# PytorchConnectomics/pytorch_connectomics

Hardware: AMD Instinct MI355X
Metric: voxels/s (train + sliding-window infer), MedNeXt-S 112^3 bf16 (higher is better)
Workload: dtype bf16; 1 GPU; Lucchi++ sliding-window inference (configs[1]): MedNeXt-S k3, 165x1024x768 volume, roi 112^3, overlap 0.5, bump blending, sw_batch_size 8, random-init weights; step = one whole-volume EagerSlidingWindowEngine call (TTA off); value = window-voxels/s; sw_batch_size=8, window_pipeline_streams=3

## Files before the change

include/pytc_hip.h:

```cpp
#ifndef PYTC_HIP_H
#define PYTC_HIP_H

#include <stdint.h>

#ifdef __cplusplus
extern "C" {
#endif

#define PYTC_ABI_VERSION 5

#define PYTC_OK 0
#define PYTC_ERR_INVALID 1
#define PYTC_ERR_HIP 2
#define PYTC_ERR_UNSUPPORTED 3

#define PYTC_F32 0
#define PYTC_BF16 1

#define PYTC_VIEW_FLIP_Z 1
#define PYTC_VIEW_FLIP_Y 2
#define PYTC_VIEW_FLIP_X 4
#define PYTC_VIEW_SWAP_YX 8
#define PYTC_VIEW_SWAP_ZY 16
#define PYTC_VIEW_SWAP_ZX 32

#define PYTC_PAD_CONSTANT 0
#define PYTC_PAD_REFLECT 1
#define PYTC_PAD_REPLICATE 2
#define PYTC_PAD_CIRCULAR 3

#define PYTC_BLEND_PRODUCT 0
#define PYTC_BLEND_MIN 1

#define PYTC_ACT_NONE 0
#define PYTC_ACT_SIGMOID 1
#define PYTC_ACT_TANH 2
#define PYTC_ACT_GELU 3

#define PYTC_RES_NONE 0
#define PYTC_RES_ADD 1
#define PYTC_RES_UPSAMPLE 2
#define PYTC_RES_GELU_BWD 3
#define PYTC_RES_NORM_BWD 4

int pytc_abi_version(void);
const char* pytc_last_error(void);
int pytc_device_info(int device, int* cu_count, int* lds_bytes_per_cu, char* arch, int arch_len);
int pytc_set_tuning(const char* key, int value);


int pytc_gather_windows(const float* vol, int C, int Z, int Y, int X, const int32_t* starts, int B,
                        int rz, int ry, int rx, int view, int pad_mode, float cval, void* out,
                        int out_dtype, void* stream);

int pytc_blend_accumulate(const void* pred, int pred_dtype, int B, const int32_t* starts, int rz,
                          int ry, int rx, int C, int view, const float* wz, const float* wy,
                          const float* wx, int combine, float floor_w, const int32_t* border ,
                          float* value, float* weight, int Z, int Y, int X, void* stream);

int pytc_blend_accumulate_mapped(const void* pred, int pred_dtype, int B, const int32_t* starts, int rz, int ry,
                                 int rx, int C, int view, const float* wz, const float* wy, const float* wx,
                                 int combine, float floor_w, const int32_t* border, const int32_t* chan_src,
                                 const int32_t* chan_shift, float* value, float* weight, int Z, int Y, int X,
                                 void* stream);
int pytc_blend_weight_shifted(int B, const int32_t* starts, int rz, int ry, int rx, const float* wz, const float* wy,
                              const float* wx, int combine, float floor_w, const int32_t* border,
                              const int32_t* shift, float* weight, int Z, int Y, int X, void* stream);
int pytc_normalize_covered(float* value, const float* weight, int64_t n, void* stream);
int pytc_ensemble_update_masked(float* stat, float* count, const float* x, const float* cover, int64_t n, int mode,
                                void* stream);
int pytc_ensemble_finalize_masked(const float* stat, const float* count, float* out, int64_t n, int mode, void* stream);

int pytc_blend_finalize(float* value, const float* weight, int C, int64_t nvox, float clamp,
                        int act, void* stream);

#define PYTC_ACT_SOFTMAX 4
int pytc_channel_activation(float* value, int C, int64_t nvox, int channels_last, int c0, int c1, int act,
                            float scale, void* stream);

int pytc_ensemble_update(float* acc, const float* x, int64_t n, int mode, int count, void* stream);

#define PYTC_ST_U8 0
#define PYTC_ST_I8 1
#define PYTC_ST_U16 2
#define PYTC_ST_I16 3
#define PYTC_ST_I32 4
#define PYTC_ST_F16 5
#define PYTC_ST_F32 6
int pytc_scale_cast(const float* x, void* y, int64_t n, float scale, int target, void* stream);


#define PYTC_RAW_U8 0
// ... 11 lines not shown
#define PYTC_NORM_ZSCORE 1
#define PYTC_NORM_MINMAX 2
#define PYTC_NORM_DIVIDE 3
int64_t pytc_window_normalize_ws_elems(int B, int64_t n);
int pytc_window_normalize(float* x, int B, int64_t n, int mode, int binarize, float threshold, float divide, const float* clip,
                          double* workspace, void* stream);


int pytc_dwconv3d_stat_slots(int N, int D, int H, int W, int C, int K, int stride, int dtype,
                             int transposed);

int pytc_dwconv3d_kernel_variant(int N, int D, int H, int W, int C, int K, int stride, int dtype, int transposed);

int pytc_dwconv3d_fwd(const void* x, void* y, const float* w, const float* bias, float* stats,
                      int N, int D, int H, int W, int C, int K, int stride, int dtype,
                      void* stream);

int pytc_dwconv3d_fwd_wide(const void* x, void* y, const float* w, const float* bias, float* stats, int N, int D, int H,
                           int W, int C, int K, int stride, int dtype, void* stream);

int pytc_dwconv3d_res_supported(int D, int H, int W, int C, int K, int stride, int dtype);

int pytc_dwmix_supported(int D, int H, int W, int C, int C_hid, int C_out, int dtype);
int pytc_dwmix_fwd(const void* x, const float* taps, const float* dw_bias, const void* w2n, const float* b2n, const void* w3_f16,
                   const float* b3, int residual, void* y, const void* head_w, const float* head_b, float* head_y, int n_head, int N,
                   int D, int H, int W, int C, int C_hid, int C_out, int dtype, void* stream);
int pytc_dwconv3d_fwd_res(const void* x, const void* res, void* y, const float* w, const float* bias, int N, int D, int H,
                          int W, int C, int K, int stride, int dtype, void* stream);

int pytc_dwconvT3d_fwd(const void* x, void* y, const float* w, const float* bias, float* stats,
                       int N, int D, int H, int W, int C, int K, int dtype, void* stream);

int pytc_groupnorm_finalize(const float* stats, int slots, float count, const float* gamma,
                            const float* beta, float eps, float* ab, int N, int C, void* stream);


int64_t pytc_pw_packed_elems(int C_out, int C_in, int dtype);
int pytc_pw_pack_weight(const float* w, int C_out, int C_in, int transposed, void* packed,
                        int dtype, void* stream);

typedef struct {
  const void* x;
  const void* w_packed;
  const float* bias;
  const float* ab;
  const void* res;
  void* y;
  int N;
  int64_t rows_per_sample;
  int C_in, C_out;
  int in_dtype, out_dtype, w_dtype;
  int act;
  int res_mode;
  int gather;
  int Di, Hi, Wi;
  const void* res_low;
  const float* res_bias;
  int pre_act;
  int w_paired;
} pytc_pw_args;

int pytc_pw_conv_fwd(const pytc_pw_args* a, void* stream);
int pytc_pw_conv_paired_supported(const pytc_pw_args* a);
int pytc_pw_conv_rowmajor_supported(const pytc_pw_args* a);

typedef struct {
  const void* t;
  const float* ab;
  const void* w2_packed;
  const float* b2;
  const void* w3_packed;
  const float* b3;
  const void* res;
  const void* res_low;
  const float* res_bias;
  void* y;
  int N;
  int64_t rows_per_sample;
  int C_in, C_hid, C_out;
  int res_mode;
  int Di, Hi, Wi;
  int w3_format;
  int per_sample;
} pytc_mlp_args;
#define PYTC_W3_BF16 0
#define PYTC_W3_F16 1

int pytc_pw_gemm_supported(int C_in, int C_out);
int pytc_pw_gemm_fwd(const void* x, const void* w, const float* bias, const float* ab, void* y, int N, int64_t rows_per_sample,
                     int C_in, int C_out, int in_f16, int gelu_out, const void* res, const void* res_low, const float* res_bias,
                     int res_mode, int Di, int Hi, int Wi, void* stream);
int pytc_pw_mlp_supported(int C_in, int C_hid, int C_out);
int pytc_pw_pack_weight_paired(const float* w, int C_out, int C_in, int transposed, void* packed_bf16,
                               void* stream);
int pytc_pack_multi(const int64_t* table_dev, int n_items, int64_t total_elems, void* stream);
int pytc_pw_pack_weight_paired_f16(const float* w, int C_out, int C_in, int transposed, void* packed_f16,
                                   void* stream);
int pytc_pw_mlp_fwd(const pytc_mlp_args* a, void* stream);

int pytc_pw_mlp_lds_supported(int C_in, int C_hid, int C_out);
int pytc_pw_mlp_lds_fwd(const pytc_mlp_args* a, void* stream);
int pytc_pw_mlp_dma_applies(const pytc_mlp_args* a, int ignore_res_mode);
int pytc_pw_mlp_proj_supported(int C_in, int C_hid, int C_out, int C_proj);
int pytc_pw_mlp_proj_fwd(const pytc_mlp_args* a, const void* proj_w, const float* proj_b, void* z, int store_y, void* stream);
int pytc_pw_mlp_chunk_supported(int C_in, int C_hid, int C_out);
int pytc_pw_mlp_chunk_fwd(const pytc_mlp_args* a, void* stream);
int pytc_groupnorm_fold_mlp(const float* stats, int slots, float count, const float* gamma, const float* beta, float eps,
                            const float* w2, const float* b2, void* w2n, float* b2n, float* ab_out, int N, int C, int C_hid,
                            void* stream);
int pytc_pw_mlp_train_fwd(const pytc_mlp_args* a, void* hidden_pre, void* stream);
int pytc_pw_mlp_train_fwd_nostore(const pytc_mlp_args* a, void* stream);
int pytc_pw_mlp_bwd(const pytc_mlp_args* a, const void* hidden_pre, void* d_hidden, void* stream);
int pytc_pw_mlp_up_supported(int C_in, int C_hid, int C_out);
int pytc_pw_mlp_up_fwd(const pytc_mlp_args* a, const float* taps, const float* dw_bias, void* stream);
int pytc_pw_mlp_head_supported(int C_in, int C_hid, int C_out);
int pytc_pw_mlp_stemres_fwd(const pytc_mlp_args* a, const float* stem_x, const float* stem_w, const float* stem_b,
                            void* stream);
int pytc_stem_dwconv3d_stat_slots(int D, int H, int W);
int pytc_stem_dwconv3d_supported(int C_in, int C, int K);
int pytc_stem_dwconv3d_mfma_image_bytes(void);
int pytc_stem_dwconv3d_pack_mfma(const float* wx, const float* wb, const float* cst, void* image, void* stream);
int pytc_stem_dwconv3d_fwd(const float* x, const float* wx, const float* wb, const float* cst, const void* mfma_image, void* y,
                           float* stats, int N, int D, int H, int W, int C, void* stream);
int pytc_pw_mlp_head_fwd(const pytc_mlp_args* a, const void* head_w, const float* head_b, float* head_y, int n_head,
                         int store_y, void* stream);


#define PYTC_ACT_RELU 5
#define PYTC_ACT_LEAKY 6
#define PYTC_ACT_ELU 7

typedef struct {
  const void* x;
  const void* w_packed;
  const float* bias;
  const float* ab;
  const void* res;
  void* y;
  int N, D, H, W, C_in, C_out;
  int kd, kh, kw;
  int act_in;
  float act_param;
  int res_mode;
  int dtype;
} pytc_conv3d_args;

int64_t pytc_conv3d_packed_elems(int C_out, int C_in, int kd, int kh, int kw, int dtype);
int pytc_conv3d_pack_weight(const float* w, int C_out, int C_in, int kd, int kh, int kw, void* packed, int dtype,
                            void* stream);
int pytc_conv3d_fwd(const pytc_conv3d_args* a, void* stream);

int pytc_channel_stats_slots(int64_t rows);
int pytc_channel_stats(const void* x, float* stats, int N, int64_t rows, int C, int dtype, void* stream);
int pytc_norm_finalize_groups(const float* stats, int slots, float count, const float* gamma, const float* beta,
                              float eps, int groups, float* ab, int N, int C, void* stream);
int pytc_affine_act(const void* x, void* y, const float* ab, int N, int64_t rows, int C, int act, float prm,
                    int dtype, void* stream);
int pytc_maxpool3d_fwd(const void* x, void* y, int N, int D, int H, int W, int C, int fz, int fy, int fx, int dtype,
                       void* stream);
int pytc_dwconvT3d_generic_fwd(const void* x, void* y, const float* w, int N, int D, int H, int W, int C,
                               const int32_t* kernel, const int32_t* stride, const int32_t* pad, int dtype,
                               void* stream);


int pytc_groupnorm_finalize_mr(const float* stats, int slots, float count, const float* gamma, const float* beta,
                               float eps, float* ab, float* mean_rstd, int N, int C, void* stream);
int pytc_gelu(const void* x, const void* dy, void* out, int64_t n, int dtype, void* stream);
int pytc_add_inplace(void* y, const void* x, int64_t n, int dtype, void* stream);
int pytc_pw_wgrad_slots(int64_t rows_total);
int pytc_pw_wgrad(const void* x, const float* ab, const void* dy, float* dW, float* db, float* workspace, int N,
                  int64_t rows_per_sample, int C_in, int C_out, int dtype, int x_act , void* stream);
int pytc_dw_wgrad_slots(int N, const int32_t* gdims, const int32_t* xdims, int C, int K, int stride, int dtype);
int pytc_dw_wgrad(const void* g, const void* x, float* dW, float* db, float* workspace, int N, const int32_t* gdims,
                  const int32_t* xdims, int C, int K, int stride, int dtype, void* stream);

int pytc_pw_wgrad_partial(const void* x, const float* ab, const void* dy, float* workspace, int want_db, int N,
                          int64_t rows_per_sample, int C_in, int C_out, int dtype, int x_act, int* slots_out, void* stream);
int pytc_pw_wgrad_dgrad_supported(int C_in, int C_out, int dtype);
int pytc_pw_wgrad_dgrad_partial(const void* x, const void* dy, const void* w_t_paired, void* dx, float* workspace, int want_db, int N,
                                int64_t rows_per_sample, int C_in, int C_out, int dtype, int* slots_out, void* stream);
int pytc_mixer_bwd_rc_supported(int C, int C_hid, int C_out, int dtype);
// ... 175 lines not shown
```

pytorch_connectomics_amd/_native.py:

```python
from __future__ import annotations

import ctypes as C
import os
from pathlib import Path

LIB_PATH = Path(__file__).resolve().parent / "lib" / "libpytc_hip.so"
ABI_VERSION = 5

F32, BF16 = 0, 1
OK = 0

VIEW_FLIP_Z, VIEW_FLIP_Y, VIEW_FLIP_X, VIEW_SWAP_YX, VIEW_SWAP_ZY, VIEW_SWAP_ZX = 1, 2, 4, 8, 16, 32
VIEW_SWAPS = {VIEW_SWAP_YX: (1, 2), VIEW_SWAP_ZY: (0, 1), VIEW_SWAP_ZX: (0, 2)}
PAD_MODES = {"constant": 0, "reflect": 1, "replicate": 2, "circular": 3}
BLEND_PRODUCT, BLEND_MIN = 0, 1
ACT_NONE, ACT_SIGMOID, ACT_TANH, ACT_GELU, ACT_SOFTMAX, ACT_RELU, ACT_LEAKY, ACT_ELU = 0, 1, 2, 3, 4, 5, 6, 7
RES_NONE, RES_ADD, RES_UPSAMPLE, RES_GELU_BWD, RES_NORM_BWD = 0, 1, 2, 3, 4


class PwArgs(C.Structure):
    _fields_ = [
        ("x", C.c_void_p), ("w_packed", C.c_void_p), ("bias", C.c_void_p), ("ab", C.c_void_p),
        ("res", C.c_void_p), ("y", C.c_void_p),
        ("N", C.c_int), ("rows_per_sample", C.c_int64),
        ("C_in", C.c_int), ("C_out", C.c_int),
        ("in_dtype", C.c_int), ("out_dtype", C.c_int), ("w_dtype", C.c_int),
        ("act", C.c_int), ("res_mode", C.c_int), ("gather", C.c_int),
        ("Di", C.c_int), ("Hi", C.c_int), ("Wi", C.c_int),
        ("res_low", C.c_void_p), ("res_bias", C.c_void_p), ("pre_act", C.c_int), ("w_paired", C.c_int),
    ]


class MlpArgs(C.Structure):
    _fields_ = [
        ("t", C.c_void_p), ("ab", C.c_void_p), ("w2_packed", C.c_void_p), ("b2", C.c_void_p),
        ("w3_packed", C.c_void_p), ("b3", C.c_void_p), ("res", C.c_void_p), ("res_low", C.c_void_p),
        ("res_bias", C.c_void_p), ("y", C.c_void_p),
        ("N", C.c_int), ("rows_per_sample", C.c_int64),
        ("C_in", C.c_int), ("C_hid", C.c_int), ("C_out", C.c_int), ("res_mode", C.c_int),
        ("Di", C.c_int), ("Hi", C.c_int), ("Wi", C.c_int), ("w3_format", C.c_int), ("per_sample", C.c_int),
    ]


W3_BF16, W3_F16 = 0, 1
NORM_NONE, NORM_ZSCORE, NORM_MINMAX, NORM_DIVIDE = 0, 1, 2, 3
RAW_DTYPES = {"uint8": 0, "int8": 1, "uint16": 2, "int16": 3, "uint32": 4, "int32": 5, "float32": 6, "float64": 7}


class ReduceItem(C.Structure):
    _fields_ = [("part", C.c_void_p), ("out", C.c_void_p), ("n", C.c_int64), ("slots", C.c_int32), ("out_t", C.c_int32)]


class Conv3dArgs(C.Structure):
    _fields_ = [
        ("x", C.c_void_p), ("w_packed", C.c_void_p), ("bias", C.c_void_p), ("ab", C.c_void_p), ("res", C.c_void_p),
        ("y", C.c_void_p),
        ("N", C.c_int), ("D", C.c_int), ("H", C.c_int), ("W", C.c_int), ("C_in", C.c_int), ("C_out", C.c_int),
        ("kd", C.c_int), ("kh", C.c_int), ("kw", C.c_int),
        ("act_in", C.c_int), ("act_param", C.c_float), ("res_mode", C.c_int), ("dtype", C.c_int),
    ]


_SIGS = {
    "pytc_abi_version": (C.c_int, []),
    "pytc_last_error": (C.c_char_p, []),
    "pytc_device_info": (C.c_int, [C.c_int, C.POINTER(C.c_int), C.POINTER(C.c_int), C.c_char_p, C.c_int]),
    "pytc_set_tuning": (C.c_int, [C.c_char_p, C.c_int]),
    "pytc_gather_windows": (C.c_int, [C.c_void_p, C.c_int, C.c_int, C.c_int, C.c_int, C.POINTER(C.c_int32),
                                      C.c_int, C.c_int, C.c_int, C.c_int, C.c_int, C.c_int, C.c_float,
                                      C.c_void_p, C.c_int, C.c_void_p]),
    "pytc_blend_accumulate": (C.c_int, [C.c_void_p, C.c_int, C.c_int, C.POINTER(C.c_int32), C.c_int, C.c_int,
                                        C.c_int, C.c_int, C.c_int, C.c_void_p, C.c_void_p, C.c_void_p, C.c_int,
                                        C.c_float, C.POINTER(C.c_int32), C.c_void_p, C.c_void_p, C.c_int, C.c_int,
                                        C.c_int, C.c_void_p]),
    "pytc_blend_finalize": (C.c_int, [C.c_void_p, C.c_void_p, C.c_int, C.c_int64, C.c_float, C.c_int, C.c_void_p]),
    "pytc_channel_activation": (C.c_int, [C.c_void_p, C.c_int, C.c_int64, C.c_int, C.c_int, C.c_int, C.c_int,
                                          C.c_float, C.c_void_p]),
    "pytc_ensemble_update": (C.c_int, [C.c_void_p, C.c_void_p, C.c_int64, C.c_int, C.c_int, C.c_void_p]),
    "pytc_dwconv3d_stat_slots": (C.c_int, [C.c_int] * 9),
    "pytc_dwconv3d_kernel_variant": (C.c_int, [C.c_int] * 9),
    "pytc_dwconv3d_fwd": (C.c_int, [C.c_void_p, C.c_void_p, C.c_void_p, C.c_void_p, C.c_void_p] + [C.c_int] * 8
                          + [C.c_void_p]),
    "pytc_dwconv3d_fwd_wide": (C.c_int, [C.c_void_p, C.c_void_p, C.c_void_p, C.c_void_p, C.c_void_p] + [C.c_int] * 8
                               + [C.c_void_p]),
    "pytc_dwconv3d_res_supported": (C.c_int, [C.c_int] * 7),
    "pytc_dwmix_supported": (C.c_int, [C.c_int] * 7),
    "pytc_dwmix_fwd": (C.c_int, [C.c_void_p] * 7 + [C.c_int] + [C.c_void_p] * 4 + [C.c_int] * 9 + [C.c_void_p]),
    "pytc_dwconv3d_fwd_res": (C.c_int, [C.c_void_p, C.c_void_p, C.c_void_p, C.c_void_p, C.c_void_p] + [C.c_int] * 8
                              + [C.c_void_p]),
    "pytc_dwconvT3d_fwd": (C.c_int, [C.c_void_p, C.c_void_p, C.c_void_p, C.c_void_p, C.c_void_p] + [C.c_int] * 7
                           + [C.c_void_p]),
    "pytc_groupnorm_finalize": (C.c_int, [C.c_void_p, C.c_int, C.c_float, C.c_void_p, C.c_void_p, C.c_float,
                                          C.c_void_p, C.c_int, C.c_int, C.c_void_p]),
    "pytc_groupnorm_fold_mlp": (C.c_int, [C.c_void_p, C.c_int, C.c_float, C.c_void_p, C.c_void_p, C.c_float, C.c_void_p,
                                          C.c_void_p, C.c_void_p, C.c_void_p, C.c_void_p, C.c_int, C.c_int, C.c_int, C.c_void_p]),
    "pytc_pw_gemm_supported": (C.c_int, [C.c_int, C.c_int]),
    "pytc_pw_gemm_fwd": (C.c_int, [C.c_void_p, C.c_void_p, C.c_void_p, C.c_void_p, C.c_void_p, C.c_int, C.c_int64, C.c_int, C.c_int,
                                   C.c_int, C.c_int, C.c_void_p, C.c_void_p, C.c_void_p, C.c_int, C.c_int, C.c_int, C.c_int,
                                   C.c_void_p]),
    "pytc_pw_packed_elems": (C.c_int64, [C.c_int, C.c_int, C.c_int]),
    "pytc_pw_pack_weight": (C.c_int, [C.c_void_p, C.c_int, C.c_int, C.c_int, C.c_void_p, C.c_int, C.c_void_p]),
    "pytc_blend_accumulate_mapped": (C.c_int, [C.c_void_p, C.c_int, C.c_int, C.POINTER(C.c_int32), C.c_int, C.c_int, C.c_int,
                                               C.c_int, C.c_int, C.c_void_p, C.c_void_p, C.c_void_p, C.c_int, C.c_float,
                                               C.POINTER(C.c_int32), C.POINTER(C.c_int32), C.POINTER(C.c_int32), C.c_void_p,
                                               C.c_void_p, C.c_int, C.c_int, C.c_int, C.c_void_p]),
    "pytc_blend_weight_shifted": (C.c_int, [C.c_int, C.POINTER(C.c_int32), C.c_int, C.c_int, C.c_int, C.c_void_p, C.c_void_p,
                                            C.c_void_p, C.c_int, C.c_float, C.POINTER(C.c_int32), C.POINTER(C.c_int32),
                                            C.c_void_p, C.c_int, C.c_int, C.c_int, C.c_void_p]),
    "pytc_normalize_covered": (C.c_int, [C.c_void_p, C.c_void_p, C.c_int64, C.c_void_p]),
    "pytc_ensemble_update_masked": (C.c_int, [C.c_void_p, C.c_void_p, C.c_void_p, C.c_void_p, C.c_int64, C.c_int, C.c_void_p]),
    "pytc_ensemble_finalize_masked": (C.c_int, [C.c_void_p, C.c_void_p, C.c_void_p, C.c_int64, C.c_int, C.c_void_p]),
    "pytc_scale_cast": (C.c_int, [C.c_void_p, C.c_void_p, C.c_int64, C.c_float, C.c_int, C.c_void_p]),
    "pytc_resample_region": (C.c_int, [C.c_void_p, C.c_int, C.POINTER(C.c_int64), C.c_int, C.c_void_p, C.c_void_p, C.c_void_p,
                                       C.POINTER(C.c_int32), C.c_void_p, C.c_void_p]),
    "pytc_window_normalize_ws_elems": (C.c_int64, [C.c_int, C.c_int64]),
    "pytc_window_normalize": (C.c_int, [C.c_void_p, C.c_int, C.c_int64, C.c_int, C.c_int, C.c_float, C.c_float, C.c_void_p,
                                        C.c_void_p, C.c_void_p]),
    "pytc_pw_conv_fwd": (C.c_int, [C.POINTER(PwArgs), C.c_void_p]),
    "pytc_pw_conv_paired_supported": (C.c_int, [C.POINTER(PwArgs)]),
    "pytc_pw_conv_rowmajor_supported": (C.c_int, [C.POINTER(PwArgs)]),
    "pytc_conv3d_packed_elems": (C.c_int64, [C.c_int] * 6),
    "pytc_conv3d_pack_weight": (C.c_int, [C.c_void_p, C.c_int, C.c_int, C.c_int, C.c_int, C.c_int, C.c_void_p, C.c_int,
                                          C.c_void_p]),
    "pytc_conv3d_fwd": (C.c_int, [C.POINTER(Conv3dArgs), C.c_void_p]),
    "pytc_channel_stats_slots": (C.c_int, [C.c_int64]),
    "pytc_channel_stats": (C.c_int, [C.c_void_p, C.c_void_p, C.c_int, C.c_int64, C.c_int, C.c_int, C.c_void_p]),
    "pytc_norm_finalize_groups": (C.c_int, [C.c_void_p, C.c_int, C.c_float, C.c_void_p, C.c_void_p, C.c_float, C.c_int,
# ... 33 lines not shown
    "pytc_pw_wgrad_groupnorm_supported": (C.c_int, [C.c_int, C.c_int, C.c_int]),
    "pytc_pw_wgrad_groupnorm_sps": (C.c_int, [C.c_int, C.c_int64, C.c_int, C.c_int]),
    "pytc_pw_wgrad_groupnorm_ws_elems": (C.c_int64, [C.c_int, C.c_int64, C.c_int, C.c_int]),
    "pytc_pw_wgrad_groupnorm": (C.c_int, [C.c_void_p] * 6 + [C.c_float] + [C.c_void_p] * 3 + [C.c_int, C.c_int64, C.c_int, C.c_int, C.c_int,
                                           C.c_void_p]),
    "pytc_norm_bwd_apply": (C.c_int, [C.c_void_p] * 5 + [C.c_int, C.c_void_p, C.c_int, C.c_int64, C.c_int, C.c_float, C.c_int,
                                      C.c_void_p, C.c_void_p]),
    "pytc_norm_bwd_ws_elems": (C.c_int, [C.c_int, C.c_int64, C.c_int]),
    "pytc_norm_bwd": (C.c_int, [C.c_void_p, C.c_void_p, C.c_void_p, C.c_void_p, C.c_void_p, C.c_void_p, C.c_void_p,
                                C.c_int, C.c_int64, C.c_float, C.c_int, C.c_int, C.c_void_p]),
    "pytc_dwconv3d_bwd_data": (C.c_int, [C.c_void_p, C.c_void_p, C.c_void_p, C.c_int, C.POINTER(C.c_int32),
                                         C.POINTER(C.c_int32), C.c_int, C.c_int, C.c_int, C.c_int, C.c_void_p]),
    "pytc_dwconv3d_bwd_data_add": (C.c_int, [C.c_void_p, C.c_void_p, C.c_void_p, C.c_void_p, C.c_int, C.POINTER(C.c_int32),
                                             C.POINTER(C.c_int32), C.c_int, C.c_int, C.c_int, C.c_int, C.c_void_p]),
    "pytc_conv3d_wgrad_ws_elems": (C.c_int64, [C.c_int, C.c_int, C.c_int, C.c_int, C.c_int, C.c_int, C.POINTER(C.c_int32), C.c_int]),
    "pytc_conv3d_wgrad": (C.c_int, [C.c_void_p, C.c_void_p, C.c_void_p, C.c_void_p, C.c_int, C.c_int, C.c_int, C.c_int, C.c_int,
                                    C.c_int, C.POINTER(C.c_int32), C.c_int, C.c_void_p]),
    "pytc_act_bwd": (C.c_int, [C.c_void_p, C.c_void_p, C.c_void_p, C.c_void_p, C.c_void_p, C.c_int, C.c_int64, C.c_int,
                               C.c_int, C.c_float, C.c_int, C.c_void_p]),
    "pytc_norm_finalize_groups_mr": (C.c_int, [C.c_void_p, C.c_int, C.c_float, C.c_void_p, C.c_void_p, C.c_float, C.c_int,
                                               C.c_void_p, C.c_void_p, C.c_int, C.c_int, C.c_void_p]),
    "pytc_norm_bwd_stats": (C.c_int, [C.c_void_p, C.c_void_p, C.c_void_p, C.c_void_p, C.c_void_p, C.c_int, C.c_int64, C.c_int,
                                      C.c_int, C.c_void_p]),
    "pytc_act_norm_bwd_stats": (C.c_int, [C.c_void_p] * 8 + [C.c_int, C.c_int64, C.c_int, C.c_int, C.c_float, C.c_int, C.c_void_p]),
    "pytc_act_norm_bwd_apply": (C.c_int, [C.c_void_p] * 7 + [C.c_int, C.c_int64, C.c_int, C.c_int, C.c_float, C.c_int, C.c_void_p]),
    "pytc_act_norm_bwd_apply_cg": (C.c_int, [C.c_void_p] * 5 + [C.c_int] + [C.c_void_p] * 2 + [C.c_int, C.c_int64, C.c_int, C.c_int, C.c_float, C.c_int, C.c_void_p]),
    "pytc_norm_bwd_apply_general": (C.c_int, [C.c_void_p, C.c_void_p, C.c_void_p, C.c_void_p, C.c_void_p, C.c_void_p, C.c_int,
                                              C.c_int64, C.c_int, C.c_int, C.c_void_p]),
    "pytc_maxpool3d_bwd": (C.c_int, [C.c_void_p, C.c_void_p, C.c_void_p, C.c_int, C.c_int, C.c_int, C.c_int, C.c_int, C.c_int,
                                     C.c_int, C.c_int, C.c_int, C.c_void_p]),
    "pytc_dwconv3d_generic_fwd": (C.c_int, [C.c_void_p, C.c_void_p, C.c_void_p, C.c_int, C.c_int, C.c_int, C.c_int, C.c_int,
                                            C.POINTER(C.c_int32), C.POINTER(C.c_int32), C.POINTER(C.c_int32),
                                            C.POINTER(C.c_int32), C.c_int, C.c_void_p]),
    "pytc_conv3d_direct_packed_elems": (C.c_int64, [C.c_int] * 6),
    "pytc_conv3d_pack_weight_direct": (C.c_int, [C.c_void_p, C.c_int, C.c_int, C.c_int, C.c_int, C.c_int, C.c_int64, C.c_int64,
                                                 C.c_int, C.c_void_p, C.c_int, C.c_void_p]),
    "pytc_conv3d_strided_fwd": (C.c_int, [C.POINTER(Conv3dArgs), C.POINTER(C.c_int32), C.POINTER(C.c_int32),
                                          C.POINTER(C.c_int32), C.c_int, C.c_void_p]),
    "pytc_convT3d_c1_fwd": (C.c_int, [C.c_void_p, C.c_void_p, C.c_void_p, C.c_void_p, C.c_void_p, C.c_int, C.POINTER(C.c_int32), C.c_int,
                                      C.c_int, C.c_void_p]),
    "pytc_convT3d_phase_plan": (C.c_int, [C.c_int, C.c_int, C.c_int, C.c_void_p]),
    "pytc_convT3d_phase_supported": (C.c_int, [C.c_int, C.c_int, C.c_int]),
    "pytc_convT3d_phase_fwd": (C.c_int, [C.POINTER(Conv3dArgs), C.POINTER(C.c_int32), C.c_void_p]),
    "pytc_conv3d_wgrad_strided_ws_elems": (C.c_int64, [C.c_int, C.POINTER(C.c_int32), C.c_int, C.c_int, C.POINTER(C.c_int32)]),
    "pytc_conv3d_wgrad_strided": (C.c_int, [C.c_void_p, C.c_void_p, C.c_void_p, C.c_void_p, C.c_int, C.POINTER(C.c_int32),
                                            C.POINTER(C.c_int32), C.c_int, C.c_int, C.POINTER(C.c_int32), C.POINTER(C.c_int32),
                                            C.POINTER(C.c_int32), C.c_int, C.c_void_p]),
    "pytc_conv3d_pack_plan": (C.c_int, [C.c_int] * 7 + [C.c_void_p]),
    "pytc_conv3d_pack_multi": (C.c_int, [C.c_void_p, C.c_int, C.c_int64, C.c_void_p]),
    "pytc_conv3d_pack_weight_dgrad": (C.c_int, [C.c_void_p, C.c_int, C.c_int, C.c_int, C.c_int, C.c_int, C.c_void_p, C.c_int, C.c_void_p]),
    "pytc_norm_bwd_means": (C.c_int, [C.c_void_p, C.c_void_p, C.c_void_p, C.c_void_p, C.c_void_p, C.c_int, C.c_int, C.c_int,
                                      C.c_float, C.c_void_p]),
    "pytc_norm_bwd_means_cpg": (C.c_int, [C.c_void_p, C.c_void_p, C.c_void_p, C.c_void_p, C.c_void_p, C.c_int, C.c_int, C.c_int,
                                          C.c_int, C.c_float, C.c_void_p]),
    "pytc_norm_finalize_groups_cpg": (C.c_int, [C.c_void_p, C.c_int, C.c_float, C.c_void_p, C.c_void_p, C.c_float, C.c_int, C.c_int,
                                                C.c_void_p, C.c_void_p, C.c_int, C.c_int, C.c_void_p]),
    "pytc_bn_train_finalize": (C.c_int, [C.c_void_p, C.c_int, C.c_float, C.c_void_p, C.c_void_p, C.c_float, C.c_float, C.c_void_p,
                                         C.c_void_p, C.c_void_p, C.c_void_p, C.c_void_p, C.c_int, C.c_int, C.c_void_p]),
    "pytc_bn_train_finalize_cpad": (C.c_int, [C.c_void_p, C.c_int, C.c_float, C.c_void_p, C.c_void_p, C.c_float, C.c_float, C.c_void_p,
                                              C.c_void_p, C.c_void_p, C.c_void_p, C.c_void_p, C.c_int, C.c_int, C.c_int, C.c_void_p]),
    "pytc_bn_update_running": (C.c_int, [C.c_void_p, C.c_void_p, C.c_void_p, C.c_int, C.c_float, C.c_float, C.c_float, C.c_void_p]),
    "pytc_layernorm_rows": (C.c_int, [C.c_void_p, C.c_void_p, C.c_void_p, C.c_void_p, C.c_int64, C.c_int, C.c_float, C.c_int, C.c_void_p]),
    "pytc_layernorm_rows_bwd_slots": (C.c_int, [C.c_int64, C.c_int, C.c_int]),
    "pytc_layernorm_rows_bwd": (C.c_int, [C.c_void_p, C.c_void_p, C.c_void_p, C.c_void_p, C.c_void_p, C.c_int64, C.c_int, C.c_float,
                                          C.c_int, C.c_void_p]),
    "pytc_grn_bwd_apply": (C.c_int, [C.c_void_p, C.c_void_p, C.c_void_p, C.c_void_p, C.c_void_p, C.c_int, C.c_int64, C.c_int, C.c_int,
                                     C.c_void_p]),
    "pytc_bce_dice_ws_elems": (C.c_int64, [C.c_int, C.c_int, C.c_int64]),
    "pytc_bce_dice_fwd": (C.c_int, [C.c_void_p, C.c_void_p, C.c_void_p, C.c_int, C.c_int, C.c_int64, C.POINTER(C.c_int64),
                                    C.POINTER(C.c_int64), C.POINTER(C.c_int64), C.c_float, C.c_float, C.c_float, C.c_float,
                                    C.c_float, C.c_void_p, C.c_void_p, C.c_void_p, C.c_void_p]),
    "pytc_bce_dice_bwd": (C.c_int, [C.c_void_p, C.c_void_p, C.c_void_p, C.c_void_p, C.c_void_p, C.c_void_p, C.c_void_p,
                                    C.c_int, C.c_int, C.c_int64, C.POINTER(C.c_int64), C.POINTER(C.c_int64),
                                    C.POINTER(C.c_int64), C.POINTER(C.c_int64), C.c_float, C.c_float, C.c_float, C.c_float,
                                    C.c_float, C.c_void_p]),
    "pytc_opt_chunk_elems": (C.c_int, []),
    "pytc_grad_norm_multi": (C.c_int, [C.c_void_p, C.c_void_p, C.c_int, C.c_float, C.c_void_p, C.c_void_p, C.c_void_p]),
    "pytc_adamw_multi": (C.c_int, [C.c_void_p, C.c_void_p, C.c_int, C.POINTER(C.c_float), C.c_int, C.c_void_p, C.c_void_p]),
    "pytc_pw_mlp_supported": (C.c_int, [C.c_int, C.c_int, C.c_int]),
    "pytc_pw_pack_weight_paired": (C.c_int, [C.c_void_p, C.c_int, C.c_int, C.c_int, C.c_void_p, C.c_void_p]),
    "pytc_pack_multi": (C.c_int, [C.c_void_p, C.c_int, C.c_int64, C.c_void_p]),
    "pytc_pw_pack_weight_paired_f16": (C.c_int, [C.c_void_p, C.c_int, C.c_int, C.c_int, C.c_void_p, C.c_void_p]),
    "pytc_pw_mlp_fwd": (C.c_int, [C.POINTER(MlpArgs), C.c_void_p]),
    "pytc_pw_mlp_lds_supported": (C.c_int, [C.c_int, C.c_int, C.c_int]),
    "pytc_pw_mlp_lds_fwd": (C.c_int, [C.POINTER(MlpArgs), C.c_void_p]),
    "pytc_pw_mlp_dma_applies": (C.c_int, [C.POINTER(MlpArgs), C.c_int]),
    "pytc_pw_mlp_proj_supported": (C.c_int, [C.c_int, C.c_int, C.c_int, C.c_int]),
    "pytc_pw_mlp_proj_fwd": (C.c_int, [C.POINTER(MlpArgs), C.c_void_p, C.c_void_p, C.c_void_p, C.c_int, C.c_void_p]),
    "pytc_pw_mlp_chunk_supported": (C.c_int, [C.c_int, C.c_int, C.c_int]),
    "pytc_pw_mlp_chunk_fwd": (C.c_int, [C.POINTER(MlpArgs), C.c_void_p]),
    "pytc_pw_mlp_stemres_fwd": (C.c_int, [C.POINTER(MlpArgs), C.c_void_p, C.c_void_p, C.c_void_p, C.c_void_p]),
    "pytc_stem_dwconv3d_stat_slots": (C.c_int, [C.c_int, C.c_int, C.c_int]),
    "pytc_stem_dwconv3d_supported": (C.c_int, [C.c_int, C.c_int, C.c_int]),
    "pytc_convT3d_thin_supported": (C.c_int, [C.c_int, C.c_int]),
    "pytc_convT3d_thin_fwd": (C.c_int, [C.c_void_p, C.c_void_p, C.c_void_p, C.c_void_p, C.c_int, C.POINTER(C.c_int32), C.c_int, C.c_int,
                                        C.c_int, C.c_void_p]),
    "pytc_stem_dwconv3d_mfma_image_bytes": (C.c_int, []),
    "pytc_stem_dwconv3d_pack_mfma": (C.c_int, [C.c_void_p, C.c_void_p, C.c_void_p, C.c_void_p, C.c_void_p]),
    "pytc_stem_dwconv3d_fwd": (C.c_int, [C.c_void_p, C.c_void_p, C.c_void_p, C.c_void_p, C.c_void_p, C.c_void_p, C.c_void_p,
                                         C.c_int, C.c_int, C.c_int, C.c_int, C.c_int, C.c_void_p]),
    "pytc_pw_mlp_train_fwd": (C.c_int, [C.POINTER(MlpArgs), C.c_void_p, C.c_void_p]),
    "pytc_pw_mlp_train_fwd_nostore": (C.c_int, [C.POINTER(MlpArgs), C.c_void_p]),
    "pytc_pw_mlp_bwd": (C.c_int, [C.POINTER(MlpArgs), C.c_void_p, C.c_void_p, C.c_void_p]),
    "pytc_pw_mlp_up_supported": (C.c_int, [C.c_int, C.c_int, C.c_int]),
    "pytc_pw_mlp_up_fwd": (C.c_int, [C.POINTER(MlpArgs), C.c_void_p, C.c_void_p, C.c_void_p]),
    "pytc_pw_mlp_head_supported": (C.c_int, [C.c_int, C.c_int, C.c_int]),
    "pytc_pw_mlp_head_fwd": (C.c_int, [C.POINTER(MlpArgs), C.c_void_p, C.c_void_p, C.c_void_p, C.c_int, C.c_int, C.c_void_p]),
    "pytc_upcat_deconv2_fwd": (C.c_int, [C.c_void_p, C.c_void_p, C.c_void_p, C.c_void_p, C.c_void_p] + [C.c_int] * 11 + [C.c_void_p]),
    "pytc_upcat_deconv2_bwd_data": (C.c_int, [C.c_void_p, C.c_void_p, C.c_void_p, C.c_void_p] + [C.c_int] * 11 + [C.c_void_p]),
    "pytc_upcat_deconv2_wgrad_ws_elems": (C.c_int64, [C.c_int] * 4),
    "pytc_upcat_deconv2_wgrad": (C.c_int, [C.c_void_p] * 5 + [C.c_int] * 11 + [C.c_void_p]),
    "pytc_linear_fwd": (C.c_int, [C.c_void_p] * 4 + [C.c_int] + [C.c_void_p] * 2 + [C.c_int] * 5 + [C.c_void_p]),
    "pytc_linear_bwd_data": (C.c_int, [C.c_void_p] * 4 + [C.c_int] * 4 + [C.c_void_p]),
    "pytc_linear_wgrad": (C.c_int, [C.c_void_p] * 5 + [C.c_int] * 6 + [C.c_void_p]),
    "pytc_layernorm_wide": (C.c_int, [C.c_void_p] * 4 + [C.c_int64, C.c_int, C.c_float, C.c_int, C.c_void_p]),
    "pytc_layernorm_wide_bwd_slots": (C.c_int, [C.c_int64]),
    "pytc_layernorm_wide_bwd": (C.c_int, [C.c_void_p] * 7 + [C.c_int64, C.c_int, C.c_float, C.c_int, C.c_void_p]),
    "pytc_patch_gather16": (C.c_int, [C.c_void_p] * 2 + [C.c_int] * 7 + [C.c_void_p]),
    "pytc_attention_supported": (C.c_int, [C.c_int]),
    "pytc_attention_fwd": (C.c_int, [C.c_void_p] * 3 + [C.c_int] * 4 + [C.c_float, C.c_int, C.c_void_p]),
    "pytc_attention_bwd": (C.c_int, [C.c_void_p] * 6 + [C.c_int] * 4 + [C.c_float, C.c_int, C.c_void_p]),
    "pytc_deconv2_upfirst_fwd": (C.c_int, [C.c_void_p] * 5 + [C.c_int] * 8 + [C.c_void_p]),
    "pytc_deconv2_upfirst_bwd_data": (C.c_int, [C.c_void_p] * 4 + [C.c_int] * 8 + [C.c_void_p]),
    "pytc_deconv2_upfirst_wgrad": (C.c_int, [C.c_void_p] * 5 + [C.c_int] * 8 + [C.c_void_p]),
    "pytc_window_attention_supported": (C.c_int, [C.c_int]),
    "pytc_window_attention_bias_groups": (C.c_int, [C.c_int] * 3),
    "pytc_window_attention_fwd": (C.c_int, [C.c_void_p] * 2 + [C.POINTER(C.c_int32)] + [C.c_void_p] * 2 + [C.c_int] * 4
                                  + [C.c_float, C.c_int, C.c_void_p]),
    "pytc_window_attention_bwd": (C.c_int, [C.c_void_p] * 2 + [C.POINTER(C.c_int32)] + [C.c_void_p] * 7 + [C.c_int] * 4
                                  + [C.c_float, C.c_int, C.c_void_p]),
    "pytc_window_partition": (C.c_int, [C.c_void_p] * 3 + [C.POINTER(C.c_int32)] + [C.c_int] * 4 + [C.c_void_p]),
    "pytc_space_to_depth2": (C.c_int, [C.c_void_p] * 2 + [C.c_int] * 8 + [C.c_void_p]),
    "pytc_layernorm_any": (C.c_int, [C.c_void_p] * 4 + [C.c_int64, C.c_int, C.c_float, C.c_int, C.c_void_p]),
    "pytc_layernorm_any_bwd_slots": (C.c_int, [C.c_int64]),
    "pytc_layernorm_any_bwd": (C.c_int, [C.c_void_p] * 8 + [C.c_int64, C.c_int, C.c_float, C.c_int, C.c_void_p]),
    "pytc_cldice_tiles": (C.c_int, [C.c_int64]),
    "pytc_cldice_erode": (C.c_int, [C.c_void_p] * 2 + [C.c_int] * 5 + [C.c_void_p]),
    "pytc_cldice_skeleton": (C.c_int, [C.c_void_p] * 7 + [C.c_int] * 6 + [C.c_void_p]),
    "pytc_cldice_chain_bwd": (C.c_int, [C.c_void_p] * 7 + [C.c_int] * 6 + [C.c_void_p]),
    "pytc_cldice_sweep_bwd": (C.c_int, [C.c_void_p] * 9 + [C.c_int] * 7 + [C.c_void_p]),
}

_lib = None


def exported_symbols():
    return sorted(_SIGS)


def lib():
    global _lib
    if _lib is not None:
        return _lib
    if not LIB_PATH.exists():
        raise RuntimeError(
            f"pytorch_connectomics_amd: HIP library {LIB_PATH} is missing. Build it with "
            "`python -m pytorch_connectomics_amd.csrc.build` (needs hipcc). There is no CPU fallback.")
    import torch
    handle = C.CDLL(str(LIB_PATH))
    for name, (res, args) in _SIGS.items():
        try:
            fn = getattr(handle, name)
        except AttributeError as e:
            raise RuntimeError(f"{LIB_PATH} does not export {name}; rebuild the library") from e
        fn.restype = res
        fn.argtypes = args
# ... 19 lines not shown
```

pytorch_connectomics_amd/csrc/pw_common.h:

```cpp
#pragma once
#include "pytc_common.h"

namespace pytc {

template <typename TW>
struct Mma;

template <>
struct Mma<bf16_t> {
  static constexpr int EPL = 8;
  static constexpr int KSTEP = 32;
  typedef bf16x8_t frag_t;
  static __device__ __forceinline__ f32x4_t mma(frag_t a, frag_t b, f32x4_t c) {
    return __builtin_amdgcn_mfma_f32_16x16x32_bf16(a, b, c, 0, 0, 0);
  }
  static __device__ __forceinline__ frag_t from_floats(const float (&v)[8]) {
    f32x8_t f;
#pragma unroll
    for (int i = 0; i < 8; ++i) f[i] = v[i];
    return __builtin_convertvector(f, frag_t);
  }
};

template <>
struct Mma<float> {
  static constexpr int EPL = 4;
  static constexpr int KSTEP = 16;
  typedef f32x4_t frag_t;
  static __device__ __forceinline__ f32x4_t mma(frag_t a, frag_t b, f32x4_t c) {
#pragma unroll
    for (int s = 0; s < 4; ++s) c = __builtin_amdgcn_mfma_f32_16x16x4f32(a[s], b[s], c, 0, 0, 0);
    return c;
  }
  static __device__ __forceinline__ frag_t from_floats(const float (&v)[4]) {
    frag_t f;
#pragma unroll
    for (int i = 0; i < 4; ++i) f[i] = v[i];
    return f;
  }
};

__host__ __device__ __forceinline__ int paired_row(int T, int m) {
  return (T >> 1) * 32 + (m >> 2) * 8 + (T & 1) * 4 + (m & 3);
}

struct EpiParams {
  const void* res;
  const void* res_low;
  const float* res_bias;
  void* y;
  long rps_out;
  int C_out;
  int res_mode;
  int Go_d, Go_h, Go_w;
  int Gl_d, Gl_h, Gl_w;
  int nt;
};

typedef unsigned int pytc_u32x4_t __attribute__((ext_vector_type(4)));
template <typename V>
__device__ __forceinline__ V ld_stream(const V* ptr, int nt) {
  static_assert(sizeof(V) == 16, "16-byte row pieces");
  if (nt) return __builtin_bit_cast(V, __builtin_nontemporal_load(reinterpret_cast<const pytc_u32x4_t*>(ptr)));
  return *ptr;
}

static inline int stream_nt_policy(long bytes_largest_tensor) {
  (void)bytes_largest_tensor;
  return tuning_get("stream_nt", 0) > 0 ? 1 : 0;
}

template <typename TO, int NCH, bool GELU_BWD = false, int COUT = 0>
__device__ __forceinline__ void finish_and_store(float (&v)[NCH], const EpiParams& e, int n, long orow, int o0,
                                                 const float* pre = nullptr, const int* pos = nullptr) {
  const int C_out = COUT > 0 ? COUT : e.C_out;
  TO* yn = reinterpret_cast<TO*>(e.y) + (long)n * e.rps_out * C_out;
  const TO* resn = e.res ? reinterpret_cast<const TO*>(e.res) + (long)n * e.rps_out * C_out : nullptr;
  const long off = orow * C_out + o0;
  const bool full = (C_out % NCH) == 0 && (o0 + NCH <= C_out);
  if (e.res_mode == PYTC_RES_ADD) {
    float rv[NCH];
    if (pre) {
#pragma unroll
      for (int i = 0; i < NCH; ++i) rv[i] = pre[i];
    } else if (full) VecIO<TO, NCH>::load(resn + off, rv);
    else {
#pragma unroll
      for (int i = 0; i < NCH; ++i) rv[i] = (o0 + i < C_out) ? to_f32<TO>(resn[off + i]) : 0.f;
    }
#pragma unroll
    for (int i = 0; i < NCH; ++i) v[i] += rv[i];
  } else if (GELU_BWD && e.res_mode == PYTC_RES_GELU_BWD) {
    float rv[NCH];
    if (pre) {
#pragma unroll
      for (int i = 0; i < NCH; ++i) rv[i] = pre[i];
    } else if (full) VecIO<TO, NCH>::load(resn + off, rv);
    else {
#pragma unroll
      for (int i = 0; i < NCH; ++i) rv[i] = (o0 + i < C_out) ? to_f32<TO>(resn[off + i]) : 0.f;
    }
#pragma unroll
    for (int i = 0; i < NCH; ++i) v[i] *= gelu_erf_grad(rv[i]);
  } else if (GELU_BWD && e.res_mode == PYTC_RES_NORM_BWD) {
    float rv[NCH];
    if (pre) {
#pragma unroll
      for (int i = 0; i < NCH; ++i) rv[i] = pre[i];
    } else if (full) VecIO<TO, NCH>::load(resn + off, rv);
    else {
#pragma unroll
      for (int i = 0; i < NCH; ++i) rv[i] = (o0 + i < C_out) ? to_f32<TO>(resn[off + i]) : 0.f;
    }
    const float* cf = e.res_bias + (long)n * 3 * C_out + o0;
#pragma unroll
    for (int i = 0; i < NCH; ++i)
      if (o0 + i < C_out) v[i] = fmaf(cf[i], v[i], fmaf(cf[C_out + i], rv[i], cf[2 * C_out + i]));
    if (e.Go_w > 0) {
      const unsigned ur = (unsigned)orow, gw = (unsigned)e.Go_w, gh = (unsigned)e.Go_h;
      const unsigned tq = ur / gw;
      const int px = (int)(ur - tq * gw), pz = (int)(tq / gh), py = (int)(tq - (unsigned)pz * gh);
      if (px == 0 || py == 0 || pz == 0) return;
      const long crow = ((long)(pz - 1) * (e.Go_h - 1) + (py - 1)) * (e.Go_w - 1) + (px - 1);
      TO* yc = reinterpret_cast<TO*>(e.y) + ((long)n * (e.Go_d - 1) * (e.Go_h - 1) * (e.Go_w - 1) + crow) * C_out + o0;
      if (full) VecIO<TO, NCH>::store(yc, v);
      else {
#pragma unroll
        for (int i = 0; i < NCH; ++i)
          if (o0 + i < C_out) yc[i] = from_f32<TO>(v[i]);
      }
      return;
    }
  } else if (e.res_mode == PYTC_RES_UPSAMPLE) {
    int px, py, pz;
    if (pos) { pz = pos[0]; py = pos[1]; px = pos[2]; }
    else {
      const unsigned ur = (unsigned)orow, gw = (unsigned)e.Go_w, gh = (unsigned)e.Go_h;
      const unsigned t = ur / gw;
      px = (int)(ur - t * gw);
      pz = (int)(t / gh);
      py = (int)(t - (unsigned)pz * gh);
    }
    float sk[NCH];
    if (pre) {
#pragma unroll
      for (int i = 0; i < NCH; ++i) sk[i] = pre[i];
    } else if (full) VecIO<TO, NCH>::load(resn + off, sk);
    else {
#pragma unroll
      for (int i = 0; i < NCH; ++i) sk[i] = (o0 + i < C_out) ? to_f32<TO>(resn[off + i]) : 0.f;
    }
    if (px == 0 || py == 0 || pz == 0) {
#pragma unroll
      for (int i = 0; i < NCH; ++i) v[i] = sk[i];
    } else {
      const int oz = pz - 1, oy = py - 1, ox = px - 1;
      float rl[NCH];
      if (e.res_low && !((oz | oy | ox) & 1)) {
        const TO* rp = reinterpret_cast<const TO*>(e.res_low) +
                       ((((long)n * e.Gl_d + (oz >> 1)) * e.Gl_h + (oy >> 1)) * e.Gl_w + (ox >> 1)) * C_out + o0;
        if (full) VecIO<TO, NCH>::load(rp, rl);
        else {
#pragma unroll
          for (int i = 0; i < NCH; ++i) rl[i] = (o0 + i < C_out) ? to_f32<TO>(rp[i]) : 0.f;
        }
      } else {
#pragma unroll
        for (int i = 0; i < NCH; ++i) rl[i] = (e.res_bias && o0 + i < C_out) ? e.res_bias[o0 + i] : 0.f;
      }
#pragma unroll
      for (int i = 0; i < NCH; ++i) v[i] = v[i] + rl[i] + sk[i];
    }
  }
  if (full) {
    if constexpr (sizeof(TO) == 2 && NCH == 8) {
      if (e.nt) {
        f32x8_t f;
#pragma unroll
        for (int i = 0; i < 8; ++i) f[i] = v[i];
        __builtin_nontemporal_store(__builtin_convertvector(f, bf16x8_t), reinterpret_cast<bf16x8_t*>(yn + off));
        return;
      }
    }
    VecIO<TO, NCH>::store(yn + off, v);
  } else {
#pragma unroll
    for (int i = 0; i < NCH; ++i)
      if (o0 + i < C_out) yn[off + i] = from_f32<TO>(v[i]);
  }
}

template <typename TI, int EPL>
__device__ __forceinline__ void load_row_frag(const TI* __restrict__ row, int k0, int C_in, bool vec_ok,
                                              float (&v)[EPL]) {
  if (vec_ok && k0 + EPL <= C_in) {
    if constexpr (sizeof(TI) == 4 && EPL == 8) {
      float t0[4], t1[4];
      VecIO<float, 4>::load(reinterpret_cast<const float*>(row) + k0, t0);
      VecIO<float, 4>::load(reinterpret_cast<const float*>(row) + k0 + 4, t1);
#pragma unroll
      for (int i = 0; i < 4; ++i) { v[i] = t0[i]; v[4 + i] = t1[i]; }
    } else {
      VecIO<TI, EPL>::load(row + k0, v);
    }
  } else {
#pragma unroll
    for (int j = 0; j < EPL; ++j) v[j] = (k0 + j < C_in) ? to_f32<TI>(row[k0 + j]) : 0.f;
  }
}

template <int PER>
struct WarmRegs { unsigned int r[2 * PER]; };
template <int PER>
__device__ __forceinline__ void warm_l2(const void* base, long bytes, WarmRegs<PER>& w, int first) {
  const long lines = (bytes + 127) >> 7;
  const long lin = (long)blockIdx.z * gridDim.y * gridDim.x + (long)blockIdx.y * gridDim.x + blockIdx.x;
  const long total = (long)gridDim.x * gridDim.y * gridDim.z;
  const long per_xcd = (total + 7) >> 3;
  const long stride = per_xcd * blockDim.x;
  long l = (lin >> 3) * blockDim.x + threadIdx.x;
#pragma unroll
  for (int it = 0; it < PER; ++it, l += stride) {
    const long lc = l < lines ? l : lines - 1;
    const char* ptr = reinterpret_cast<const char*>(base) + (lc << 7);
    asm volatile("global_load_dword %0, %1, off" : "=v"(w.r[first + it]) : "v"(ptr) : "memory");
  }
}
template <int PER>
__device__ __forceinline__ void warm_l2_done(WarmRegs<PER>& w) {
  asm volatile("s_waitcnt vmcnt(0)" : : : "memory");
#pragma unroll
  for (int i = 0; i < 2 * PER; ++i) asm volatile("" : : "v"(w.r[i]) : "memory");
}

__device__ __forceinline__ float apply_act(float t, int act) {
  if (act == PYTC_ACT_GELU) return gelu_erf(t);
  if (act == PYTC_ACT_SIGMOID) return 1.f / (1.f + __expf(-t));
  if (act == PYTC_ACT_TANH) return tanhf(t);
  return t;
}

}
```

pytorch_connectomics_amd/csrc/pw_mlp_chunk_kernels.hip:

```cpp
#include "pw_common.h"

namespace pytc {

struct MlpChunkParams {
  const bf16_t* t;
  const float* ab;
  const bf16x8_t* w2;
  const float* b2;
  const h8_t* w3;
  const float* b3;
  EpiParams e;
  long rps;
  int N, C_in, C_hid, C_out, HC;
  long w2_stride;
};

__device__ __forceinline__ void chunk_glds16(const void* gsrc, unsigned lds_dst) {
  unsigned keep;
  asm volatile("s_mov_b32 %0, m0\n\ts_mov_b32 m0, %2\n\ts_nop 0\n\tglobal_load_lds_dwordx4 %1, off\n\ts_mov_b32 m0, %0"
               : "=&s"(keep) : "v"(gsrc), "s"(lds_dst) : "memory");
}

template <int KS_IN, int MO, int NW, int WPS>
__global__ void __launch_bounds__(NW * 64, WPS)
pw_mlp_chunk_kernel(MlpChunkParams p) {
  constexpr int NT = 2, CIN = KS_IN * 32, COUT = MO * 16;
  constexpr int PIECES = 2 * KS_IN + MO;
  constexpr int MINE = (PIECES + NW - 1) / NW;
  constexpr int NBUF = 3;
  extern __shared__ __attribute__((aligned(16))) unsigned char chunk_lds[];
  uint4* ring = reinterpret_cast<uint4*>(chunk_lds);
  float* lb2 = reinterpret_cast<float*>(chunk_lds + (size_t)NBUF * PIECES * 1024);
  float* lb3 = lb2 + p.C_hid;
  const int tid = threadIdx.x, lane = tid & 63;
  const int wave = __builtin_amdgcn_readfirstlane(tid >> 6);
  const int r = lane & 15, kb = lane >> 4;
  const int n = blockIdx.y;
  const bool folded = p.ab == nullptr;
  const long row0 = ((long)blockIdx.x * NW + wave) * (NT * 16);
  const bool with_res = p.e.res_mode != PYTC_RES_NONE;
  const bool ups = p.e.res_mode == PYTC_RES_UPSAMPLE;

  const unsigned char* w2img = reinterpret_cast<const unsigned char*>(p.w2 + (folded ? (long)n * p.w2_stride : 0L));
  const unsigned char* w3img = reinterpret_cast<const unsigned char*>(p.w3);
  const unsigned lbase = __builtin_amdgcn_readfirstlane((unsigned)(size_t)(__attribute__((address_space(3))) void*)ring);
  int mine = 0;
#pragma unroll
  for (int i = 0; i < MINE; ++i) mine += (wave + i * NW < PIECES) ? 1 : 0;
  auto request = [&](int hc) {
    const unsigned buf = lbase + (unsigned)((hc % NBUF) * PIECES) * 1024u;
#pragma unroll
    for (int i = 0; i < MINE; ++i) {
      const int pc = wave + i * NW;
      if (pc < PIECES) {
        const unsigned char* src = pc < 2 * KS_IN ? w2img + ((long)hc * (2 * KS_IN) + pc) * 1024
                                                  : w3img + ((long)(pc - 2 * KS_IN) * p.HC + hc) * 1024;
        chunk_glds16(src + lane * 16, buf + (unsigned)pc * 1024u);
      }
    }
  };

  long orow[NT];
#pragma unroll
  for (int nt = 0; nt < NT; ++nt) orow[nt] = row0 + nt * 16 + r;
  bf16x8_t bact[KS_IN][NT];
  const bf16_t* tn = p.t + (long)n * p.rps * CIN;
  uint4 raw[KS_IN][NT];
#pragma unroll
  for (int nt = 0; nt < NT; ++nt) {
    const long rr = orow[nt] < p.rps ? orow[nt] : p.rps - 1;
#pragma unroll
    for (int ks = 0; ks < KS_IN; ++ks) raw[ks][nt] = ld_stream(reinterpret_cast<const uint4*>(tn + rr * CIN + ks * 32 + kb * 8), p.e.nt);
  }
  {
    const float* b2 = p.b2 + (folded ? (long)n * p.C_hid : 0L);
    for (int i = tid; i < p.C_hid; i += NW * 64) lb2[i] = b2[i];
    if (tid < COUT) lb3[tid] = p.b3[tid];
  }
  request(0);
  if (p.HC > 1) request(1);
  const float* an = folded ? nullptr : p.ab + (long)n * 2 * CIN;
#pragma unroll
  for (int ks = 0; ks < KS_IN; ++ks) {
    if (folded) {
#pragma unroll
      for (int nt = 0; nt < NT; ++nt) bact[ks][nt] = __builtin_bit_cast(bf16x8_t, raw[ks][nt]);
    } else {
      const int k0 = ks * 32 + kb * 8;
      float av[8], bv[8];
      VecIO<float, 4>::load(an + k0, reinterpret_cast<float(&)[4]>(av[0]));
      VecIO<float, 4>::load(an + k0 + 4, reinterpret_cast<float(&)[4]>(av[4]));
      VecIO<float, 4>::load(an + CIN + k0, reinterpret_cast<float(&)[4]>(bv[0]));
      VecIO<float, 4>::load(an + CIN + k0 + 4, reinterpret_cast<float(&)[4]>(bv[4]));
#pragma unroll
      for (int nt = 0; nt < NT; ++nt) {
        float v[8];
        VecIO<bf16_t, 8>::load(reinterpret_cast<const bf16_t*>(&raw[ks][nt]), v);
#pragma unroll
        for (int j = 0; j < 8; ++j) v[j] = fmaf(v[j], av[j], bv[j]);
        bact[ks][nt] = Mma<bf16_t>::from_floats(v);
      }
    }
  }
#pragma unroll
  for (int ks = 0; ks < KS_IN; ++ks)
#pragma unroll
    for (int nt = 0; nt < NT; ++nt) asm volatile("" : "+v"(bact[ks][nt]));
  __syncthreads();
  f32x4_t acc2[MO][NT];
#pragma unroll
  for (int pr = 0; pr < MO / 2; ++pr) {
    const f32x4_t lo = *reinterpret_cast<const f32x4_t*>(lb3 + pr * 32 + kb * 8), hi = *reinterpret_cast<const f32x4_t*>(lb3 + pr * 32 + kb * 8 + 4);
#pragma unroll
    for (int nt = 0; nt < NT; ++nt) { acc2[2 * pr][nt] = lo; acc2[2 * pr + 1][nt] = hi; }
  }

  for (int hc = 0; hc < p.HC; ++hc) {
    if (hc + 1 < p.HC) {
      if (mine == 2) asm volatile("s_waitcnt vmcnt(2)" ::: "memory");
      else if (mine == 1) asm volatile("s_waitcnt vmcnt(1)" ::: "memory");
      else if (mine == 3) asm volatile("s_waitcnt vmcnt(3)" ::: "memory");
      else asm volatile("s_waitcnt vmcnt(0)" ::: "memory");
    } else {
      asm volatile("s_waitcnt vmcnt(0)" ::: "memory");
    }
    __syncthreads();
    if (hc + 2 < p.HC) request(hc + 2);
    const uint4* cb = ring + (size_t)(hc % NBUF) * PIECES * 64;
    const f32x4_t b2lo = *reinterpret_cast<const f32x4_t*>(lb2 + hc * 32 + kb * 8);
    const f32x4_t b2hi = *reinterpret_cast<const f32x4_t*>(lb2 + hc * 32 + kb * 8 + 4);
    f32x4_t acc1[2][NT];
#pragma unroll
    for (int nt = 0; nt < NT; ++nt) { acc1[0][nt] = b2lo; acc1[1][nt] = b2hi; }
#pragma unroll
    for (int mt = 0; mt < 2; ++mt) {
#pragma unroll
      for (int ks = 0; ks < KS_IN; ++ks) {
        const bf16x8_t a = __builtin_bit_cast(bf16x8_t, cb[(mt * KS_IN + ks) * 64 + lane]);
#pragma unroll
        for (int nt = 0; nt < NT; ++nt) acc1[mt][nt] = Mma<bf16_t>::mma(a, bact[ks][nt], acc1[mt][nt]);
      }
    }
    h8_t bhh[NT];
#pragma unroll
    for (int nt = 0; nt < NT; ++nt) {
      float gg[8];
#pragma unroll
      for (int j = 0; j < 4; ++j) { gg[j] = acc1[0][nt][j]; gg[4 + j] = acc1[1][nt][j]; }
      bhh[nt] = gelu_h8_from_f32(gg);
    }
#pragma unroll
    for (int mo = 0; mo < MO; ++mo) {
      const h8_t a = __builtin_bit_cast(h8_t, cb[(2 * KS_IN + mo) * 64 + lane]);
#pragma unroll
      for (int nt = 0; nt < NT; ++nt) acc2[mo][nt] = __builtin_amdgcn_mfma_f32_16x16x32_f16(a, bhh[nt], acc2[mo][nt], 0, 0, 0);
    }
  }

  if (row0 >= p.rps) return;
  int upos[NT][3];
  if (ups) {
    const unsigned ur = (unsigned)row0, gw = (unsigned)p.e.Go_w, gh = (unsigned)p.e.Go_h;
    const unsigned t0 = ur / gw;
    const int bx = (int)(ur - t0 * gw);
    const int bz = (int)(t0 / gh);
    const int by = (int)(t0 - (unsigned)bz * gh);
#pragma unroll
    for (int nt = 0; nt < NT; ++nt) {
      int px = bx + nt * 16 + r, py = by, pz = bz;
      while (px >= p.e.Go_w) { px -= p.e.Go_w; ++py; }
      while (py >= p.e.Go_h) { py -= p.e.Go_h; ++pz; }
      upos[nt][0] = pz; upos[nt][1] = py; upos[nt][2] = px;
    }
  }
#pragma unroll
  for (int pr = 0; pr < MO / 2; ++pr) {
#pragma unroll
    for (int nt = 0; nt < NT; ++nt) {
      if (orow[nt] >= p.rps) continue;
      float v[8];
#pragma unroll
      for (int j = 0; j < 4; ++j) { v[j] = acc2[2 * pr][nt][j]; v[4 + j] = acc2[2 * pr + 1][nt][j]; }
      finish_and_store<bf16_t, 8, false, COUT>(v, p.e, n, orow[nt], pr * 32 + kb * 8, nullptr, (with_res && ups) ? upos[nt] : nullptr);
    }
  }
}

template <int KS_IN, int MO, int NW, int WPS>
static void launch_mlp_chunk_v(const MlpChunkParams& p, hipStream_t s) {
  auto kern = &pw_mlp_chunk_kernel<KS_IN, MO, NW, WPS>;
  const size_t lds = (size_t)3 * (2 * KS_IN + MO) * 1024 + (size_t)(p.C_hid + MO * 16) * 4;
  if (!ensure_dynamic_lds(reinterpret_cast<const void*>(kern), 160 * 1024, "pw_mlp_chunk")) return;
  const long wg_rows = (long)NW * 32;
  dim3 grid((unsigned)((p.rps + wg_rows - 1) / wg_rows), (unsigned)p.N), block(NW * 64);
  hipLaunchKernelGGL(kern, grid, block, lds, s, p);
}

template <int KS_IN, int MO>
static void launch_mlp_chunk(const MlpChunkParams& p, int variant, hipStream_t s) {
  if (variant == 0) variant = (KS_IN == 8) ? 1 : 3;
  switch (variant) {
    case 2: launch_mlp_chunk_v<KS_IN, MO, 12, 3>(p, s); break;
    case 3: launch_mlp_chunk_v<KS_IN, MO, 8, 4>(p, s); break;
    case 4: launch_mlp_chunk_v<KS_IN, MO, 16, 4>(p, s); break;
    default: launch_mlp_chunk_v<KS_IN, MO, 8, 2>(p, s); break;
  }
}

}

using namespace pytc;

extern "C" int pytc_pw_mlp_chunk_supported(int C_in, int C_hid, int C_out) {
  if (C_in % 32 || C_hid % 32 || C_out % 32) return 0;
  const int ks = C_in / 32, mo = C_out / 16;
  const bool shape = (ks == 2 && (mo == 2 || mo == 4 || mo == 8)) || (ks == 4 && mo == 4) || (ks == 4 && mo == 8) || (ks == 8 && mo == 8);
  return (shape && C_hid >= 64 && C_hid <= 8192) ? 1 : 0;
}

extern "C" int pytc_pw_mlp_chunk_fwd(const pytc_mlp_args* a, void* stream) {
  PYTC_REQUIRE(a && a->t && (a->ab || a->per_sample) && a->w2_packed && a->w3_packed && a->b2 && a->b3 && a->y, "pw_mlp_chunk: null pointer");
  PYTC_REQUIRE(!(a->ab && a->per_sample), "pw_mlp_chunk: per-sample (norm-folded) expand operands come without an affine");
  PYTC_REQUIRE(a->w3_format == PYTC_W3_F16, "pw_mlp_chunk: the projection image must be fp16 (pytc_pw_pack_weight_paired_f16)");
  PYTC_REQUIRE(a->N >= 1 && a->rows_per_sample >= 1, "pw_mlp_chunk: bad shape");
  if (!pytc_pw_mlp_chunk_supported(a->C_in, a->C_hid, a->C_out)) {
    set_error("pw_mlp_chunk: no chunk-streamed kernel for C_in=%d C_hid=%d C_out=%d", a->C_in, a->C_hid, a->C_out);
    return PYTC_ERR_UNSUPPORTED;
  }
  PYTC_REQUIRE(a->res_mode == PYTC_RES_NONE || a->res, "pw_mlp_chunk: residual mode without residual pointer");
  PYTC_REQUIRE(a->res_mode == PYTC_RES_NONE || a->res_mode == PYTC_RES_ADD || a->res_mode == PYTC_RES_UPSAMPLE, "pw_mlp_chunk: residual mode");
  MlpChunkParams p{};
  p.t = (const bf16_t*)a->t; p.ab = a->ab; p.w2 = (const bf16x8_t*)a->w2_packed; p.b2 = a->b2;
  p.w3 = (const h8_t*)a->w3_packed; p.b3 = a->b3;
  p.rps = a->rows_per_sample; p.N = a->N; p.C_in = a->C_in; p.C_hid = a->C_hid; p.C_out = a->C_out; p.HC = a->C_hid / 32;
  p.w2_stride = (long)(a->C_hid / 16) * (a->C_in / 32) * 64;
  p.e.res = a->res; p.e.res_low = a->res_low; p.e.res_bias = a->res_bias; p.e.y = a->y;
  p.e.rps_out = a->rows_per_sample; p.e.C_out = a->C_out; p.e.res_mode = a->res_mode;
  p.e.nt = stream_nt_policy((long)a->N * a->rows_per_sample * (a->C_in > a->C_out ? a->C_in : a->C_out) * 2);
  p.e.Go_d = p.e.Go_h = p.e.Go_w = p.e.Gl_d = p.e.Gl_h = p.e.Gl_w = 0;
  if (a->res_mode == PYTC_RES_UPSAMPLE) {
    PYTC_REQUIRE((long)a->Di * a->Hi * a->Wi == a->rows_per_sample && !(a->Di & 1) && !(a->Hi & 1) && !(a->Wi & 1) &&
                 a->rows_per_sample < (1L << 31), "pw_mlp_chunk: RES_UPSAMPLE needs the (even) output grid");
    p.e.Go_d = a->Di; p.e.Go_h = a->Hi; p.e.Go_w = a->Wi;
    p.e.Gl_d = a->Di / 2; p.e.Gl_h = a->Hi / 2; p.e.Gl_w = a->Wi / 2;
  }
  hipStream_t s = (hipStream_t)stream;
  const int ks = a->C_in / 32, mo = a->C_out / 16;
  const int variant = tuning_get("mlp_chunk_variant", 0);
  if (ks == 2 && mo == 2) launch_mlp_chunk<2, 2>(p, variant, s);
  else if (ks == 2 && mo == 4) launch_mlp_chunk<2, 4>(p, variant, s);
  else if (ks == 2 && mo == 8) launch_mlp_chunk<2, 8>(p, variant, s);
  else if (ks == 4 && mo == 4) launch_mlp_chunk<4, 4>(p, variant, s);
  else if (ks == 4 && mo == 8) launch_mlp_chunk<4, 8>(p, variant, s);
  else launch_mlp_chunk<8, 8>(p, variant, s);
  PYTC_LAUNCH_CHECK("pw_mlp_chunk");
  return PYTC_OK;
}
```

pytorch_connectomics_amd/csrc/pw_mlp_kernels.hip:

```cpp
#include <cmath>
#include "pw_common.h"

namespace pytc {

struct MlpParams {
  const bf16_t* t;
  const float* ab;
  const bf16x8_t* w2;
  const float* b2;
  const bf16x8_t* w3;
  const float* b3;
  EpiParams e;
  long rps;
  int C_in, C_hid, C_out, HC;
  int w3_f16;
  long w2_stride;
  const bf16x8_t* head_w;
  const float* head_b;
  float* head_y;
  int n_head, store_y;
  bf16_t* proj_y;
  const float* stem_x;
  const float* stem_w;
  const float* stem_b;
  bf16_t* hp;
  int round_h;
  const bf16_t* hp_in;
};

constexpr int GELU_LUT_N = 1024;
__device__ float2 g_gelu_lut[GELU_LUT_N];

__device__ __forceinline__ float gelu_lut(const float2* __restrict__ tab, float x) {
  const float t = fminf(fmaxf(fmaf(x, 64.0f, 512.0f), 0.0f), (float)(GELU_LUT_N - 1));
  const float2 ab = tab[(int)t];
  return fmaf(ab.y, x, ab.x);
}

constexpr int mlp_waves_per_simd(int ks, int mo, int nt) {
  if (ks >= 8 && nt == 1) return 1;
  const int regs = ks * nt * 4 + mo * nt * 4 + 2 * nt * 4;
  return regs <= 64 ? 4 : (regs <= 112 ? 3 : (regs <= 200 ? 2 : 1));
}

template <int KS_IN, int MO, int NT, int GELU_MODE, bool HEAD = false, bool STEMRES = false, bool STOREH = false, bool BWD = false>
__global__ void __launch_bounds__(256, mlp_waves_per_simd(KS_IN, MO, NT))
pw_mlp_kernel(MlpParams p) {
  constexpr int CIN = KS_IN * 32, COUT = MO * 16;
  static_assert(MO % 2 == 0, "C_out must be a multiple of 32");
  static_assert(!STEMRES || (MO == 2 && (MO / 2) * NT <= 4), "the stem-recomputing residual covers C_out = 32");
  static_assert(!HEAD || MO == 2, "the fused head covers C_out = 32");
  __shared__ __attribute__((aligned(16))) float2 lut[GELU_MODE == 2 ? GELU_LUT_N : 1];
  if constexpr (GELU_MODE == 2) {
    const uint4* src = reinterpret_cast<const uint4*>(g_gelu_lut);
    uint4* dst = reinterpret_cast<uint4*>(lut);
    dst[threadIdx.x] = src[threadIdx.x];
    dst[threadIdx.x + 256] = src[threadIdx.x + 256];
    __syncthreads();
  }
  constexpr bool PREFETCH_RES = (MO / 2) * NT <= 4;
  const int wave = threadIdx.x >> 6, lane = threadIdx.x & 63;
  const int n = blockIdx.y;
  constexpr bool WARM = KS_IN * MO >= 32;
  constexpr int WPER = KS_IN * MO >= 512 ? 6 : 2;
  WarmRegs<WPER> warm;
  const bool folded = p.ab == nullptr;
  const bf16x8_t* w2 = p.w2 + (folded ? (long)n * p.w2_stride : 0L);
  const float* b2 = p.b2 + (folded ? (long)n * p.C_hid : 0L);
  if (WARM) {
    warm_l2(w2, (long)p.C_hid * CIN * 2, warm, 0);
    warm_l2(p.w3, (long)COUT * p.C_hid * 2, warm, WPER);
  }
  const long row0 = ((long)blockIdx.x * 4 + wave) * (NT * 16);
  if (row0 >= p.rps) {
    if (WARM) asm volatile("s_waitcnt vmcnt(0)" : : : "memory");
    return;
  }
  const int r = lane & 15, kb = lane >> 4;

  long orow[NT];
#pragma unroll
  for (int nt = 0; nt < NT; ++nt) orow[nt] = row0 + nt * 16 + r;

  bf16x8_t bact[KS_IN][NT];
  const bf16_t* tn = p.t + (long)n * p.rps * CIN;
  if (folded) {
#pragma unroll
    for (int ks = 0; ks < KS_IN; ++ks)
#pragma unroll
      for (int nt = 0; nt < NT; ++nt) {
        const long rr = orow[nt] < p.rps ? orow[nt] : p.rps - 1;
        bact[ks][nt] = ld_stream(reinterpret_cast<const bf16x8_t*>(tn + rr * CIN + ks * 32 + kb * 8), p.e.nt);
      }
  }
  const float* an = p.ab + (long)n * 2 * CIN;
#pragma unroll
  for (int ks = 0; ks < KS_IN; ++ks) {
    if (folded) break;
    const int k0 = ks * 32 + kb * 8;
    float av[8], bv[8];
    VecIO<float, 4>::load(an + k0, reinterpret_cast<float(&)[4]>(av[0]));
    VecIO<float, 4>::load(an + k0 + 4, reinterpret_cast<float(&)[4]>(av[4]));
    VecIO<float, 4>::load(an + CIN + k0, reinterpret_cast<float(&)[4]>(bv[0]));
    VecIO<float, 4>::load(an + CIN + k0 + 4, reinterpret_cast<float(&)[4]>(bv[4]));
#pragma unroll
    for (int nt = 0; nt < NT; ++nt) {
      const long rr = orow[nt] < p.rps ? orow[nt] : p.rps - 1;
      float v[8];
      VecIO<bf16_t, 8>::load(tn + rr * CIN + k0, v);
#pragma unroll
      for (int j = 0; j < 8; ++j) v[j] = fmaf(v[j], av[j], bv[j]);
      bact[ks][nt] = Mma<bf16_t>::from_floats(v);
    }
  }

  if (WARM) warm_l2_done(warm);

  uint4 rpre[PREFETCH_RES ? MO / 2 : 1][PREFETCH_RES ? NT : 1];
  const bool use_pre = PREFETCH_RES && p.e.res_mode != PYTC_RES_NONE;
  if constexpr (STEMRES) {
    const float* sx = p.stem_x + (long)n * p.rps;
    float sw[8], sb[8];
    VecIO<float, 4>::load(p.stem_w + kb * 8, reinterpret_cast<float(&)[4]>(sw[0]));
    VecIO<float, 4>::load(p.stem_w + kb * 8 + 4, reinterpret_cast<float(&)[4]>(sw[4]));
    VecIO<float, 4>::load(p.stem_b + kb * 8, reinterpret_cast<float(&)[4]>(sb[0]));
    VecIO<float, 4>::load(p.stem_b + kb * 8 + 4, reinterpret_cast<float(&)[4]>(sb[4]));
#pragma unroll
    for (int nt = 0; nt < NT; ++nt) {
      const float xv = sx[orow[nt] < p.rps ? orow[nt] : p.rps - 1];
      float rv[8];
#pragma unroll
      for (int j = 0; j < 8; ++j) rv[j] = fmaf(sw[j], xv, sb[j]);
      rpre[0][nt] = __builtin_bit_cast(uint4, Mma<bf16_t>::from_floats(rv));
    }
  } else if (use_pre) {
    const bf16_t* resn = reinterpret_cast<const bf16_t*>(p.e.res) + (long)n * p.rps * COUT;
#pragma unroll
    for (int pr = 0; pr < (PREFETCH_RES ? MO / 2 : 1); ++pr)
#pragma unroll
      for (int nt = 0; nt < (PREFETCH_RES ? NT : 1); ++nt) {
        const long rr = orow[nt] < p.rps ? orow[nt] : p.rps - 1;
        rpre[pr][nt] = ld_stream(reinterpret_cast<const uint4*>(resn + rr * COUT + pr * 32 + kb * 8), p.e.nt);
      }
  }

  f32x4_t acc2[MO][NT];
#pragma unroll
  for (int pr = 0; pr < MO / 2; ++pr) {
    float b[8];
    VecIO<float, 4>::load(p.b3 + pr * 32 + kb * 8, reinterpret_cast<float(&)[4]>(b[0]));
    VecIO<float, 4>::load(p.b3 + pr * 32 + kb * 8 + 4, reinterpret_cast<float(&)[4]>(b[4]));
#pragma unroll
    for (int nt = 0; nt < NT; ++nt) {
      acc2[2 * pr][nt] = f32x4_t{b[0], b[1], b[2], b[3]};
      acc2[2 * pr + 1][nt] = f32x4_t{b[4], b[5], b[6], b[7]};
    }
  }

  for (int hc = 0; hc < p.HC; ++hc) {
    float b2v[8];
    VecIO<float, 4>::load(b2 + hc * 32 + kb * 8, reinterpret_cast<float(&)[4]>(b2v[0]));
    VecIO<float, 4>::load(b2 + hc * 32 + kb * 8 + 4, reinterpret_cast<float(&)[4]>(b2v[4]));
    f32x4_t acc1[2][NT];
#pragma unroll
    for (int nt = 0; nt < NT; ++nt) {
      acc1[0][nt] = f32x4_t{b2v[0], b2v[1], b2v[2], b2v[3]};
      acc1[1][nt] = f32x4_t{b2v[4], b2v[5], b2v[6], b2v[7]};
    }
#pragma unroll
    for (int mt = 0; mt < 2; ++mt) {
#pragma unroll
      for (int ks = 0; ks < KS_IN; ++ks) {
        const bf16x8_t a = w2[((long)(hc * 2 + mt) * KS_IN + ks) * 64 + lane];
#pragma unroll
        for (int nt = 0; nt < NT; ++nt) acc1[mt][nt] = Mma<bf16_t>::mma(a, bact[ks][nt], acc1[mt][nt]);
      }
    }
    bf16x8_t bh[NT];
    h8_t bhh[GELU_MODE == 3 ? NT : 1];
#pragma unroll
    for (int nt = 0; nt < NT; ++nt) {
      float g[8];
      if constexpr (BWD) {
        const long rr = orow[nt] < p.rps ? orow[nt] : p.rps - 1;
        float hv[8];
        VecIO<bf16_t, 8>::load(p.hp_in + ((long)n * p.rps + rr) * p.C_hid + hc * 32 + kb * 8, hv);
#pragma unroll
        for (int j = 0; j < 4; ++j) {
          g[j] = acc1[0][nt][j] * gelu_erf_grad(hv[j]);
          g[4 + j] = acc1[1][nt][j] * gelu_erf_grad(hv[4 + j]);
        }
        bh[nt] = Mma<bf16_t>::from_floats(g);
        if (orow[nt] < p.rps)
          *reinterpret_cast<bf16x8_t*>(p.hp + ((long)n * p.rps + orow[nt]) * p.C_hid + hc * 32 + kb * 8) = bh[nt];
        continue;
      }
      if constexpr (STOREH) {
        float pre[8];
#pragma unroll
        for (int j = 0; j < 4; ++j) { pre[j] = acc1[0][nt][j]; pre[4 + j] = acc1[1][nt][j]; }
        const bf16x8_t hb = Mma<bf16_t>::from_floats(pre);
        if (p.hp && orow[nt] < p.rps)
          *reinterpret_cast<bf16x8_t*>(p.hp + ((long)n * p.rps + orow[nt]) * p.C_hid + hc * 32 + kb * 8) = hb;
        const f32x8_t hr = __builtin_convertvector(hb, f32x8_t);
#pragma unroll
        for (int j = 0; j < 4; ++j) { acc1[0][nt][j] = hr[j]; acc1[1][nt][j] = hr[4 + j]; }
      }
      if constexpr (GELU_MODE == 3) {
#pragma unroll
        for (int j = 0; j < 4; ++j) { g[j] = acc1[0][nt][j]; g[4 + j] = acc1[1][nt][j]; }
        bhh[nt] = gelu_h8_from_f32(g);
        continue;
      }
#pragma unroll
      for (int j = 0; j < 4; ++j) {
        g[j] = GELU_MODE == 2 ? gelu_lut(lut, acc1[0][nt][j]) : (GELU_MODE == 1 ? gelu_fast(acc1[0][nt][j]) : gelu_erf(acc1[0][nt][j]));
        g[4 + j] = GELU_MODE == 2 ? gelu_lut(lut, acc1[1][nt][j]) : (GELU_MODE == 1 ? gelu_fast(acc1[1][nt][j]) : gelu_erf(acc1[1][nt][j]));
      }
      bh[nt] = Mma<bf16_t>::from_floats(g);
    }
#pragma unroll
    for (int mo = 0; mo < MO; ++mo) {
      if constexpr (GELU_MODE == 3) {
        const h8_t a = reinterpret_cast<const h8_t*>(p.w3)[((long)mo * p.HC + hc) * 64 + lane];
#pragma unroll
        for (int nt = 0; nt < NT; ++nt) acc2[mo][nt] = __builtin_amdgcn_mfma_f32_16x16x32_f16(a, bhh[nt], acc2[mo][nt], 0, 0, 0);
      } else {
        const bf16x8_t a = p.w3[((long)mo * p.HC + hc) * 64 + lane];
#pragma unroll
        for (int nt = 0; nt < NT; ++nt) acc2[mo][nt] = Mma<bf16_t>::mma(a, bh[nt], acc2[mo][nt]);
      }
    }
  }

  if constexpr (HEAD) {
    bf16_t* yn = reinterpret_cast<bf16_t*>(p.e.y) + (long)n * p.rps * 32;
    const bf16_t* resn = p.e.res ? reinterpret_cast<const bf16_t*>(p.e.res) + (long)n * p.rps * 32 : nullptr;
    float* hy = p.head_y + (long)n * p.rps * p.n_head;
    const bf16x8_t ah = p.head_w[lane];
    float hb[4];
#pragma unroll
    for (int i = 0; i < 4; ++i) hb[i] = (p.head_b && kb * 4 + i < p.n_head) ? p.head_b[kb * 4 + i] : 0.f;
#pragma unroll
    for (int nt = 0; nt < NT; ++nt) {
      float v[8];
#pragma unroll
      for (int j = 0; j < 4; ++j) { v[j] = acc2[0][nt][j]; v[4 + j] = acc2[1][nt][j]; }
      const bool live = orow[nt] < p.rps;
      if (p.e.res_mode == PYTC_RES_ADD) {
        float rv[8];
        if (use_pre) VecIO<bf16_t, 8>::load(reinterpret_cast<const bf16_t*>(&rpre[0][PREFETCH_RES ? nt : 0]), rv);
        else VecIO<bf16_t, 8>::load(resn + (live ? orow[nt] : p.rps - 1) * 32 + kb * 8, rv);
#pragma unroll
        for (int j = 0; j < 8; ++j) v[j] += rv[j];
      }
      const bf16x8_t ob = Mma<bf16_t>::from_floats(v);
      if (p.store_y && live) *reinterpret_cast<bf16x8_t*>(yn + orow[nt] * 32 + kb * 8) = ob;
      const f32x4_t h = Mma<bf16_t>::mma(ah, ob, f32x4_t{0.f, 0.f, 0.f, 0.f});
      if (live) {
#pragma unroll
        for (int i = 0; i < 4; ++i)
          if (kb * 4 + i < p.n_head) hy[orow[nt] * p.n_head + kb * 4 + i] = h[i] + hb[i];
      }
    }
    return;
  }
  int upos[NT][3];
  const bool ups = p.e.res_mode == PYTC_RES_UPSAMPLE;
  if (ups) {
    const unsigned ur = (unsigned)row0, gw = (unsigned)p.e.Go_w, gh = (unsigned)p.e.Go_h;
    const unsigned t0 = ur / gw;
    const int bx = (int)(ur - t0 * gw);
    const int bz = (int)(t0 / gh);
    const int by = (int)(t0 - (unsigned)bz * gh);
#pragma unroll
    for (int nt = 0; nt < NT; ++nt) {
      int px = bx + nt * 16 + r, py = by, pz = bz;
      while (px >= p.e.Go_w) { px -= p.e.Go_w; ++py; }
      while (py >= p.e.Go_h) { py -= p.e.Go_h; ++pz; }
      upos[nt][0] = pz; upos[nt][1] = py; upos[nt][2] = px;
    }
  }
#pragma unroll
  for (int pr = 0; pr < MO / 2; ++pr) {
#pragma unroll
    for (int nt = 0; nt < NT; ++nt) {
      if (orow[nt] >= p.rps) continue;
      float v[8];
#pragma unroll
      for (int j = 0; j < 4; ++j) {
        v[j] = acc2[2 * pr][nt][j];
        v[4 + j] = acc2[2 * pr + 1][nt][j];
      }
      if (use_pre) {
        float pre[8];
        VecIO<bf16_t, 8>::load(reinterpret_cast<const bf16_t*>(&rpre[PREFETCH_RES ? pr : 0][PREFETCH_RES ? nt : 0]), pre);
        finish_and_store<bf16_t, 8, false, COUT>(v, p.e, n, orow[nt], pr * 32 + kb * 8, pre, ups ? upos[nt] : nullptr);
      } else {
        finish_and_store<bf16_t, 8, false, COUT>(v, p.e, n, orow[nt], pr * 32 + kb * 8, nullptr, ups ? upos[nt] : nullptr);
      }
    }
  }
}


__device__ __forceinline__ void glds16(const void* gsrc, unsigned lds_dst) {
  unsigned keep;
  asm volatile("s_mov_b32 %0, m0\n\ts_mov_b32 m0, %2\n\ts_nop 0\n\tglobal_load_lds_dwordx4 %1, off\n\ts_mov_b32 m0, %0"
               : "=&s"(keep) : "v"(gsrc), "s"(lds_dst) : "memory");
}
__device__ __forceinline__ void glds4(const void* gsrc, unsigned lds_dst) {
  unsigned keep;
  asm volatile("s_mov_b32 %0, m0\n\ts_mov_b32 m0, %2\n\ts_nop 0\n\tglobal_load_lds_dword %1, off\n\ts_mov_b32 m0, %0"
               : "=&s"(keep) : "v"(gsrc), "s"(lds_dst) : "memory");
}

template <int HCT, int KIND>
__global__ void __launch_bounds__(256, 3)
pw_mlp_dma_kernel(MlpParams p, int waves_per_sample) {
  constexpr int NT = 4, CIN = 32, COUT = 32;
  constexpr bool STEM = KIND == 1, HEAD = KIND == 2, PROJ = KIND == 3;
  __shared__ __attribute__((aligned(16))) uint4 land[4][2][NT * 64];
  __shared__ __attribute__((aligned(16))) uint4 w2s[HCT * 2 * 64], w3s[2 * HCT * 64];
  __shared__ __attribute__((aligned(16))) float b2s[HCT * 32], b3s[32];
  __shared__ __attribute__((aligned(16))) float auxa[STEM ? 32 : (HEAD ? 256 : (PROJ ? 512 : 4))], auxb[(STEM || PROJ) ? 32 : (HEAD ? 16 : 4)];
  const int wave = threadIdx.x >> 6, lane = threadIdx.x & 63;
  const int n = blockIdx.y;
  const int r = lane & 15, kb = lane >> 4;
  const long tiles = (p.rps + NT * 16 - 1) / (NT * 16);
  const bool with_res = STEM || p.e.res_mode == PYTC_RES_ADD;
  const bf16_t* tn = p.t + (long)n * p.rps * CIN;
  const bf16_t* resn = (!STEM && with_res) ? reinterpret_cast<const bf16_t*>(p.e.res) + (long)n * p.rps * COUT : nullptr;
  const float* sx = STEM ? p.stem_x + (long)n * p.rps : nullptr;
  bf16_t* yn = reinterpret_cast<bf16_t*>(p.e.y) + (long)n * p.rps * COUT;
  float* hy = HEAD ? p.head_y + (long)n * p.rps * p.n_head : nullptr;
  bf16_t* zn = PROJ ? p.proj_y + (long)n * p.rps * 32 : nullptr;
  {
    const uint4* w2 = reinterpret_cast<const uint4*>(p.w2 + (long)n * p.w2_stride);
    const uint4* w3 = reinterpret_cast<const uint4*>(p.w3);
    for (int i = threadIdx.x; i < HCT * 2 * 64; i += 256) { w2s[i] = w2[i]; w3s[i] = w3[i]; }
    if (threadIdx.x < HCT * 32) b2s[threadIdx.x] = p.b2[(long)n * p.C_hid + threadIdx.x];
    if (threadIdx.x < 32) b3s[threadIdx.x] = p.b3[threadIdx.x];
    if constexpr (STEM) {
      if (threadIdx.x < 32) { auxa[threadIdx.x] = p.stem_w[threadIdx.x]; auxb[threadIdx.x] = p.stem_b[threadIdx.x]; }
    }
    if constexpr (HEAD) {
      reinterpret_cast<float*>(auxa)[threadIdx.x] = reinterpret_cast<const float*>(p.head_w)[threadIdx.x];
      if (threadIdx.x < 16) auxb[threadIdx.x] = (p.head_b && (int)threadIdx.x < p.n_head) ? p.head_b[threadIdx.x] : 0.f;
    }
    if constexpr (PROJ) {
      auxa[threadIdx.x] = reinterpret_cast<const float*>(p.head_w)[threadIdx.x];
      auxa[threadIdx.x + 256] = reinterpret_cast<const float*>(p.head_w)[threadIdx.x + 256];
      if (threadIdx.x < 32) auxb[threadIdx.x] = p.head_b ? p.head_b[threadIdx.x] : 0.f;
    }
  }
  __syncthreads();
  asm volatile("s_waitcnt vmcnt(0)" ::: "memory");

  const unsigned lbase = __builtin_amdgcn_readfirstlane((unsigned)(size_t)(__attribute__((address_space(3))) void*)&land[wave][0][0]);
  auto request = [&](long tile) {
#pragma unroll
    for (int nt = 0; nt < NT; ++nt) {
      long row = tile * (NT * 16) + nt * 16 + r;
      row = row < p.rps ? row : p.rps - 1;
      glds16(tn + row * CIN + kb * 8, lbase + (unsigned)(nt * 64) * 16);
      if constexpr (STEM) glds4(sx + row, lbase + (unsigned)(NT * 64) * 16 + (unsigned)(nt * 64) * 4);
      else if (with_res) glds16(resn + row * COUT + kb * 8, lbase + (unsigned)((NT + nt) * 64) * 16);
    }
  };
  bf16x8_t out[NT];
  f32x4_t hout[HEAD ? NT : 1];
  bf16x8_t zout[PROJ ? NT : 1];
  auto store = [&](long tile) {
#pragma unroll
    for (int nt = 0; nt < NT; ++nt) {
      const long row = tile * (NT * 16) + nt * 16 + r;
      if (row >= p.rps) continue;
      if (!(HEAD || PROJ) || p.store_y) *reinterpret_cast<bf16x8_t*>(yn + row * COUT + kb * 8) = out[nt];
      if constexpr (PROJ) *reinterpret_cast<bf16x8_t*>(zn + row * 32 + kb * 8) = zout[nt];
      if constexpr (HEAD) {
#pragma unroll
        for (int i = 0; i < 4; ++i)
          if (kb * 4 + i < p.n_head) hy[row * p.n_head + kb * 4 + i] = hout[nt][i];
      }
    }
// ... 308 lines not shown

static bool ensure_gelu_lut() {
  static int state = 0;
  if (state == 0) {
    static float2 host[GELU_LUT_N];
    auto f = [](double x) { return 0.5 * x * (1.0 + erf(x * 0.70710678118654752440)); };
    for (int i = 0; i < GELU_LUT_N; ++i) {
      const double x0 = -8.0 + i / 64.0, x1 = x0 + 1.0 / 64.0;
      const double b = (f(x1) - f(x0)) * 64.0;
      host[i].x = (float)(f(x0) - b * x0);
      host[i].y = (float)b;
    }
    state = hipMemcpyToSymbol(HIP_SYMBOL(g_gelu_lut), host, sizeof(host)) == hipSuccess ? 1 : -1;
  }
  return state == 1;
}

template <int KS_IN, int MO, int NT>
static void launch_mlp(const MlpParams& p, int N, hipStream_t s) {
  long rows_per_block = 4L * NT * 16;
  dim3 grid((unsigned)((p.rps + rows_per_block - 1) / rows_per_block), (unsigned)N), block(256);
  if (p.hp_in) {
    hipLaunchKernelGGL((pw_mlp_kernel<KS_IN, MO, NT, 1, false, false, false, true>), grid, block, 0, s, p);
    return;
  }
  if (p.hp || p.round_h) {
    if (p.w3_f16) hipLaunchKernelGGL((pw_mlp_kernel<KS_IN, MO, NT, 3, false, false, true>), grid, block, 0, s, p);
    else hipLaunchKernelGGL((pw_mlp_kernel<KS_IN, MO, NT, 1, false, false, true>), grid, block, 0, s, p);
    return;
  }
  if (p.w3_f16) {
    hipLaunchKernelGGL((pw_mlp_kernel<KS_IN, MO, NT, 3>), grid, block, 0, s, p);
    return;
  }
  if (tuning_get("mlp_exact_gelu", 0))
    hipLaunchKernelGGL((pw_mlp_kernel<KS_IN, MO, NT, 0>), grid, block, 0, s, p);
  else if (tuning_get("mlp_gelu_lut", 0) && ensure_gelu_lut())
    hipLaunchKernelGGL((pw_mlp_kernel<KS_IN, MO, NT, 2>), grid, block, 0, s, p);
  else
    hipLaunchKernelGGL((pw_mlp_kernel<KS_IN, MO, NT, 1>), grid, block, 0, s, p);
}

static bool dispatch_mlp(const MlpParams& p, int N, hipStream_t s) {
  const int ks = p.C_in / 32, mo = p.C_out / 16;
  const int variant = tuning_get("mlp_variant", 0);
#define PYTC_MLP_CASE(KS, MOO, NTT) \
  if (ks == KS && mo == MOO) { launch_mlp<KS, MOO, NTT>(p, N, s); return true; }
  if (!(variant & 1)) { PYTC_MLP_CASE(2, 4, 2) }
  if (variant & 2) { PYTC_MLP_CASE(1, 2, 2) PYTC_MLP_CASE(2, 2, 2) }
  if (variant & 4) { PYTC_MLP_CASE(1, 4, 2) }
  PYTC_MLP_CASE(1, 2, 4)
  PYTC_MLP_CASE(1, 4, 4)
  PYTC_MLP_CASE(2, 2, 4)
  PYTC_MLP_CASE(2, 4, 4)
  PYTC_MLP_CASE(2, 8, 2)
  PYTC_MLP_CASE(4, 4, 2)
  PYTC_MLP_CASE(4, 8, 2)
  PYTC_MLP_CASE(4, 16, 1)
  PYTC_MLP_CASE(8, 8, 2)
  PYTC_MLP_CASE(8, 16, 1)
  PYTC_MLP_CASE(8, 32, 1)
  PYTC_MLP_CASE(16, 16, 1)
  PYTC_MLP_CASE(16, 32, 1)
#undef PYTC_MLP_CASE
  return false;
}

static bool mlp_shape_ok(int C_in, int C_hid, int C_out) {
  if (C_in % 32 || C_hid % 32 || C_out % 32 || C_in < 32 || C_out < 32 || C_hid < 32) return false;
  const int ks = C_in / 32, mo = C_out / 16;
  static const int ok[][2] = {{1, 2}, {1, 4}, {2, 2}, {2, 4}, {2, 8}, {4, 4}, {4, 8}, {4, 16}, {8, 8},
                              {8, 16}, {8, 32}, {16, 16}, {16, 32}};
  for (auto& c : ok)
    if (c[0] == ks && c[1] == mo) return true;
  return false;
}

}

using namespace pytc;

extern "C" int pytc_pw_mlp_supported(int C_in, int C_hid, int C_out) { return mlp_shape_ok(C_in, C_hid, C_out) ? 1 : 0; }

extern "C" int pytc_groupnorm_fold_mlp(const float* stats, int slots, float count, const float* gamma, const float* beta,
                                       float eps, const float* w2, const float* b2, void* w2n, float* b2n, float* ab_out, int N,
                                       int C, int C_hid, void* stream) {
  PYTC_REQUIRE(stats && w2 && w2n && b2n && slots >= 1 && count > 0 && N >= 1, "groupnorm_fold_mlp: bad arguments");
  PYTC_REQUIRE(C == 32 || C == 64 || C == 128, "groupnorm_fold_mlp: C=%d (32, 64 or 128)", C);
  PYTC_REQUIRE(C_hid % 32 == 0 && C_hid >= 32 && C_hid <= 512, "groupnorm_fold_mlp: C_hid=%d", C_hid);
  hipLaunchKernelGGL(groupnorm_fold_mlp_kernel, dim3(N), dim3(1024), 0, (hipStream_t)stream, stats, slots, count, gamma, beta,
                     eps, w2, b2, (bf16_t*)w2n, b2n, ab_out, C, C_hid);
  PYTC_LAUNCH_CHECK("groupnorm_fold_mlp");
  return PYTC_OK;
}

extern "C" int pytc_pw_mlp_head_supported(int C_in, int C_hid, int C_out) {
  return (C_out == 32 && (C_in == 32 || C_in == 64) && C_hid % 32 == 0 && C_hid >= 32) ? 1 : 0;
}

extern "C" int pytc_pw_pack_weight_paired(const float* w, int C_out, int C_in, int transposed, void* packed,
                                          void* stream) {
  PYTC_REQUIRE(w && packed && C_out >= 1 && C_in >= 1, "pw_pack_weight_paired: bad arguments");
  PYTC_REQUIRE(C_out % 32 == 0, "pw_pack_weight_paired: C_out=%d must be a multiple of 32", C_out);
  long total = pytc_pw_packed_elems(C_out, C_in, PYTC_BF16);
  int KG = (C_in + 31) / 32;
  hipLaunchKernelGGL(pw_pack_paired_kernel<bf16_t>, dim3(ceil_div(total, 256)), dim3(256), 0, (hipStream_t)stream, w, C_out,
                     C_in, transposed, (bf16_t*)packed, KG, total);
  PYTC_LAUNCH_CHECK("pw_pack_weight_paired");
  return PYTC_OK;
}

extern "C" int pytc_pw_pack_weight_paired_f16(const float* w, int C_out, int C_in, int transposed, void* packed,
                                              void* stream) {
  PYTC_REQUIRE(w && packed && C_out >= 1 && C_in >= 1, "pw_pack_weight_paired_f16: bad arguments");
  PYTC_REQUIRE(C_out % 32 == 0, "pw_pack_weight_paired_f16: C_out=%d must be a multiple of 32", C_out);
  long total = pytc_pw_packed_elems(C_out, C_in, PYTC_BF16);
  int KG = (C_in + 31) / 32;
  hipLaunchKernelGGL(pw_pack_paired_kernel<_Float16>, dim3(ceil_div(total, 256)), dim3(256), 0, (hipStream_t)stream, w,
                     C_out, C_in, transposed, (_Float16*)packed, KG, total);
  PYTC_LAUNCH_CHECK("pw_pack_weight_paired_f16");
  return PYTC_OK;
}

extern "C" int pytc_pack_multi(const int64_t* table_dev, int n_items, int64_t total_elems, void* stream) {
  PYTC_REQUIRE(table_dev && n_items >= 1 && total_elems >= 1, "pack_multi: bad arguments");
  hipLaunchKernelGGL(pack_multi_kernel, dim3(ceil_div(total_elems, 256)), dim3(256), 0, (hipStream_t)stream,
                     reinterpret_cast<const long*>(table_dev), n_items, (long)total_elems);
  PYTC_LAUNCH_CHECK("pack_multi");
  return PYTC_OK;
}

extern "C" int pytc_pw_mlp_head_fwd(const pytc_mlp_args* a, const void* head_w, const float* head_b, float* head_y,
                                    int n_head, int store_y, void* stream) {
  PYTC_REQUIRE(a && a->t && (a->ab || a->per_sample) && a->w2_packed && a->w3_packed && a->b2 && a->b3 && head_w && head_y, "pw_mlp_head: null pointer");
  PYTC_REQUIRE(!(a->ab && a->per_sample), "pw_mlp_head: per-sample (norm-folded) expand operands come without an affine");
  PYTC_REQUIRE(!store_y || a->y, "pw_mlp_head: store_y without an output buffer");
  PYTC_REQUIRE(a->N >= 1 && a->rows_per_sample >= 1 && n_head >= 1 && n_head <= 16, "pw_mlp_head: bad shape");
  if (!pytc_pw_mlp_head_supported(a->C_in, a->C_hid, a->C_out)) {
    set_error("pw_mlp_head: no fused kernel for C_in=%d C_hid=%d C_out=%d", a->C_in, a->C_hid, a->C_out);
    return PYTC_ERR_UNSUPPORTED;
  }
  PYTC_REQUIRE(a->res_mode == PYTC_RES_NONE || (a->res_mode == PYTC_RES_ADD && a->res), "pw_mlp_head: residual add or none");
  MlpParams p;
  p.t = (const bf16_t*)a->t; p.ab = a->ab; p.w2 = (const bf16x8_t*)a->w2_packed; p.b2 = a->b2;
  p.w3 = (const bf16x8_t*)a->w3_packed; p.b3 = a->b3;
  p.rps = a->rows_per_sample; p.C_in = a->C_in; p.C_hid = a->C_hid; p.C_out = a->C_out; p.HC = a->C_hid / 32;
  p.w2_stride = (long)(a->C_hid / 16) * (a->C_in / 32) * 64;
  p.e.res = a->res; p.e.res_low = nullptr; p.e.res_bias = nullptr; p.e.y = a->y;
  p.e.rps_out = a->rows_per_sample; p.e.C_out = a->C_out; p.e.res_mode = a->res_mode;
  p.e.nt = stream_nt_policy((long)a->N * a->rows_per_sample * (a->C_in > a->C_out ? a->C_in : a->C_out) * 2);
  p.e.Go_d = p.e.Go_h = p.e.Go_w = p.e.Gl_d = p.e.Gl_h = p.e.Gl_w = 0;
  p.head_w = (const bf16x8_t*)head_w; p.head_b = head_b; p.head_y = head_y; p.n_head = n_head; p.store_y = store_y;
  p.w3_f16 = a->w3_format == PYTC_W3_F16 ? 1 : 0;
  dim3 grid((unsigned)((p.rps + 4L * 4 * 16 - 1) / (4L * 4 * 16)), (unsigned)a->N), block(256);
  hipStream_t s = (hipStream_t)stream;
  const bool exact = tuning_get("mlp_exact_gelu", 0) != 0;
  if (mlp_dma_applies(a, p)) {
    mlp_dma_launch<2>(a, p, s);
    PYTC_LAUNCH_CHECK("pw_mlp_head_dma");
    return PYTC_OK;
  }
  if (p.w3_f16) {
    if (a->C_in == 32) hipLaunchKernelGGL((pw_mlp_kernel<1, 2, 4, 3, true>), grid, block, 0, s, p);
    else hipLaunchKernelGGL((pw_mlp_kernel<2, 2, 4, 3, true>), grid, block, 0, s, p);
  } else if (a->C_in == 32) {
    if (exact) hipLaunchKernelGGL((pw_mlp_kernel<1, 2, 4, 0, true>), grid, block, 0, s, p);
// ... 28 lines not shown
  p.stem_x = stem_x; p.stem_w = stem_w; p.stem_b = stem_b;
  p.w3_f16 = a->w3_format == PYTC_W3_F16 ? 1 : 0;
  dim3 grid((unsigned)((p.rps + 4L * 4 * 16 - 1) / (4L * 4 * 16)), (unsigned)a->N), block(256);
  hipStream_t s = (hipStream_t)stream;
  pytc_mlp_args shape = *a;
  shape.res_mode = PYTC_RES_NONE;
  if (mlp_dma_applies(&shape, p)) {
    mlp_dma_launch<1>(a, p, s);
    PYTC_LAUNCH_CHECK("pw_mlp_stemres_dma");
    return PYTC_OK;
  }
  if (p.w3_f16) hipLaunchKernelGGL((pw_mlp_kernel<1, 2, 4, 3, false, true>), grid, block, 0, s, p);
  else if (tuning_get("mlp_exact_gelu", 0) != 0) hipLaunchKernelGGL((pw_mlp_kernel<1, 2, 4, 0, false, true>), grid, block, 0, s, p);
  else hipLaunchKernelGGL((pw_mlp_kernel<1, 2, 4, 1, false, true>), grid, block, 0, s, p);
  PYTC_LAUNCH_CHECK("pw_mlp_stemres");
  return PYTC_OK;
}

extern "C" int pytc_pw_mlp_dma_applies(const pytc_mlp_args* a, int ignore_res_mode) {
  if (!a) return 0;
  MlpParams p{};
  p.HC = a->C_hid / 32;
  p.w3_f16 = a->w3_format == PYTC_W3_F16 ? 1 : 0;
  pytc_mlp_args shape = *a;
  if (ignore_res_mode) shape.res_mode = PYTC_RES_NONE;
  return mlp_dma_applies(&shape, p) ? 1 : 0;
}

extern "C" int pytc_pw_mlp_proj_supported(int C_in, int C_hid, int C_out, int C_proj) {
  return (C_in == 32 && C_out == 32 && C_proj == 32 && (C_hid == 64 || C_hid == 96 || C_hid == 128)) ? 1 : 0;
}
extern "C" int pytc_pw_mlp_proj_fwd(const pytc_mlp_args* a, const void* proj_w, const float* proj_b, void* z, int store_y, void* stream) {
  PYTC_REQUIRE(a && a->t && a->w2_packed && a->w3_packed && a->b2 && a->b3 && proj_w && z, "pw_mlp_proj: null pointer");
  PYTC_REQUIRE(a->per_sample && !a->ab, "pw_mlp_proj: takes the per-sample (norm-folded) expand operands");
  PYTC_REQUIRE(a->w3_format == PYTC_W3_F16, "pw_mlp_proj: the mixer's projection image must be fp16 (pytc_pw_pack_weight_paired_f16)");
  PYTC_REQUIRE(!store_y || a->y, "pw_mlp_proj: store_y without an output buffer");
  PYTC_REQUIRE(a->N >= 1 && a->rows_per_sample >= 1, "pw_mlp_proj: bad shape");
  if (!pytc_pw_mlp_proj_supported(a->C_in, a->C_hid, a->C_out, 32)) {
    set_error("pw_mlp_proj: no fused kernel for C_in=%d C_hid=%d C_out=%d", a->C_in, a->C_hid, a->C_out);
    return PYTC_ERR_UNSUPPORTED;
  }
  PYTC_REQUIRE(a->res_mode == PYTC_RES_NONE || (a->res_mode == PYTC_RES_ADD && a->res), "pw_mlp_proj: residual add or none");
  MlpParams p{};
  p.t = (const bf16_t*)a->t; p.ab = nullptr; p.w2 = (const bf16x8_t*)a->w2_packed; p.b2 = a->b2;
  p.w3 = (const bf16x8_t*)a->w3_packed; p.b3 = a->b3;
  p.rps = a->rows_per_sample; p.C_in = a->C_in; p.C_hid = a->C_hid; p.C_out = a->C_out; p.HC = a->C_hid / 32;
  p.w2_stride = (long)(a->C_hid / 16) * (a->C_in / 32) * 64;
  p.e.res = a->res; p.e.y = a->y; p.e.rps_out = a->rows_per_sample; p.e.C_out = a->C_out; p.e.res_mode = a->res_mode;
  p.head_w = (const bf16x8_t*)proj_w; p.head_b = proj_b; p.proj_y = (bf16_t*)z; p.store_y = store_y;
  p.w3_f16 = 1;
  mlp_dma_launch<3>(a, p, (hipStream_t)stream);
  PYTC_LAUNCH_CHECK("pw_mlp_proj");
  return PYTC_OK;
}

static int mlp_fwd_impl(const pytc_mlp_args* a, void* hp, void* stream, const void* hp_in = nullptr, bool round_h = false);

extern "C" int pytc_pw_mlp_bwd(const pytc_mlp_args* a, const void* hidden_pre, void* d_hidden, void* stream) {
  PYTC_REQUIRE(hidden_pre && d_hidden, "pw_mlp_bwd: null hidden buffers");
  PYTC_REQUIRE(a && a->res_mode == PYTC_RES_NONE, "pw_mlp_bwd: no residual in the backward mixer");
  return mlp_fwd_impl(a, d_hidden, stream, hidden_pre);
}

extern "C" int pytc_pw_mlp_train_fwd(const pytc_mlp_args* a, void* hidden_pre, void* stream) {
  PYTC_REQUIRE(hidden_pre, "pw_mlp_train: null hidden buffer");
  return mlp_fwd_impl(a, hidden_pre, stream);
}

extern "C" int pytc_pw_mlp_train_fwd_nostore(const pytc_mlp_args* a, void* stream) {
  return mlp_fwd_impl(a, nullptr, stream, nullptr, true);
}

extern "C" int pytc_pw_mlp_fwd(const pytc_mlp_args* a, void* stream) { return mlp_fwd_impl(a, nullptr, stream); }

static int mlp_fwd_impl(const pytc_mlp_args* a, void* hp, void* stream, const void* hp_in, bool round_h) {
  PYTC_REQUIRE(a && a->t && (a->ab || a->per_sample) && a->w2_packed && a->w3_packed && a->b2 && a->b3 && a->y, "pw_mlp: null pointer");
  PYTC_REQUIRE(!(a->ab && a->per_sample), "pw_mlp: per-sample (norm-folded) expand operands come without an affine");
  PYTC_REQUIRE(!(a->per_sample && (hp || hp_in || round_h)), "pw_mlp: the training kernels take the shared expand image and the affine");
  PYTC_REQUIRE(a->N >= 1 && a->rows_per_sample >= 1, "pw_mlp: bad shape");
  if (!mlp_shape_ok(a->C_in, a->C_hid, a->C_out)) {
    set_error("pw_mlp: no fused kernel for C_in=%d C_hid=%d C_out=%d", a->C_in, a->C_hid, a->C_out);
    return PYTC_ERR_UNSUPPORTED;
  }
  PYTC_REQUIRE(a->res_mode == PYTC_RES_NONE || a->res, "pw_mlp: residual mode without residual pointer");
  PYTC_REQUIRE(a->res_mode == PYTC_RES_NONE || a->res_mode == PYTC_RES_ADD || a->res_mode == PYTC_RES_UPSAMPLE,
               "pw_mlp: unsupported res_mode %d", a->res_mode);
  MlpParams p{};
  p.t = (const bf16_t*)a->t; p.ab = a->ab; p.w2 = (const bf16x8_t*)a->w2_packed; p.b2 = a->b2;
  p.w3 = (const bf16x8_t*)a->w3_packed; p.b3 = a->b3;
  p.rps = a->rows_per_sample; p.C_in = a->C_in; p.C_hid = a->C_hid; p.C_out = a->C_out; p.HC = a->C_hid / 32;
  p.w2_stride = (long)(a->C_hid / 16) * (a->C_in / 32) * 64;
  p.e.res = a->res; p.e.res_low = a->res_low; p.e.res_bias = a->res_bias; p.e.y = a->y;
  p.e.rps_out = a->rows_per_sample; p.e.C_out = a->C_out; p.e.res_mode = a->res_mode;
  p.e.nt = stream_nt_policy((long)a->N * a->rows_per_sample * (a->C_in > a->C_out ? a->C_in : a->C_out) * 2);
  p.e.Go_d = p.e.Go_h = p.e.Go_w = p.e.Gl_d = p.e.Gl_h = p.e.Gl_w = 0;
  p.hp = (bf16_t*)hp;
  p.hp_in = (const bf16_t*)hp_in;
  p.round_h = round_h ? 1 : 0;
  p.w3_f16 = a->w3_format == PYTC_W3_F16 ? 1 : 0;
  PYTC_REQUIRE(!(p.w3_f16 && hp_in), "pw_mlp_bwd: the backward mixer takes bf16 weight images");
  if (a->res_mode == PYTC_RES_UPSAMPLE) {
    PYTC_REQUIRE((long)a->Di * a->Hi * a->Wi == a->rows_per_sample && !(a->Di & 1) && !(a->Hi & 1) && !(a->Wi & 1),
                 "pw_mlp: RES_UPSAMPLE needs the (even) output grid");
    PYTC_REQUIRE(a->rows_per_sample < (1L << 31), "pw_mlp: RES_UPSAMPLE positions are 32-bit (rows per sample < 2^31)");
    p.e.Go_d = a->Di; p.e.Go_h = a->Hi; p.e.Go_w = a->Wi;
    p.e.Gl_d = a->Di / 2; p.e.Gl_h = a->Hi / 2; p.e.Gl_w = a->Wi / 2;
  }
  if (!hp && !hp_in && !round_h && mlp_dma_applies(a, p)) {
    mlp_dma_launch<0>(a, p, (hipStream_t)stream);
    PYTC_LAUNCH_CHECK("pw_mlp_dma");
    return PYTC_OK;
  }
  if (!dispatch_mlp(p, a->N, (hipStream_t)stream)) {
    set_error("pw_mlp: dispatch failed");
    return PYTC_ERR_UNSUPPORTED;
  }
  PYTC_LAUNCH_CHECK("pw_mlp");
  return PYTC_OK;
}
```

pytorch_connectomics_amd/csrc/pw_mlp_lds_kernels.hip:

```cpp
#include <mutex>

#include "pw_common.h"

namespace pytc {

struct MlpLdsParams {
  const bf16_t* t;
  const float* ab;
  const bf16x8_t* w2;
  const float* b2;
  const h8_t* w3;
  const float* b3;
  EpiParams e;
  long rps;
  int N, C_in, C_hid, C_out, HC;
  long w2_stride;
};

template <int KS_IN, int MO, int NT>
struct LdsTile {
  uint4 raw[KS_IN][NT];
  uint4 res[MO / 2][NT];
};

template <int KS_IN, int MO, int NT>
__device__ __forceinline__ void lds_tile_load(LdsTile<KS_IN, MO, NT>& T, const MlpLdsParams& p, int n, long row0, int r, int kb,
                                              bool with_res) {
  const bf16_t* tn = p.t + (long)n * p.rps * (KS_IN * 32);
#pragma unroll
  for (int nt = 0; nt < NT; ++nt) {
    const long o = row0 + nt * 16 + r;
    const long rr = o < p.rps ? o : p.rps - 1;
#pragma unroll
    for (int ks = 0; ks < KS_IN; ++ks) T.raw[ks][nt] = ld_stream(reinterpret_cast<const uint4*>(tn + rr * (KS_IN * 32) + ks * 32 + kb * 8), p.e.nt);
  }
  if (with_res) {
    const bf16_t* resn = reinterpret_cast<const bf16_t*>(p.e.res) + (long)n * p.rps * (MO * 16);
#pragma unroll
    for (int nt = 0; nt < NT; ++nt) {
      const long o = row0 + nt * 16 + r;
      const long rr = o < p.rps ? o : p.rps - 1;
#pragma unroll
      for (int pr = 0; pr < MO / 2; ++pr) T.res[pr][nt] = ld_stream(reinterpret_cast<const uint4*>(resn + rr * (MO * 16) + pr * 32 + kb * 8), p.e.nt);
    }
  }
}

template <int KS_IN, int MO, int NT, int NWAVES, int WPS>
__global__ void __launch_bounds__(NWAVES * 64, WPS)
pw_mlp_lds_kernel(MlpLdsParams p) {
  constexpr int CIN = KS_IN * 32, COUT = MO * 16;
  extern __shared__ __attribute__((aligned(16))) unsigned char lds_raw[];
  bf16x8_t* lw2 = reinterpret_cast<bf16x8_t*>(lds_raw);
  h8_t* lw3 = reinterpret_cast<h8_t*>(lds_raw + (size_t)p.C_hid * CIN * 2);
  float* lb2 = reinterpret_cast<float*>(lds_raw + (size_t)p.C_hid * (CIN + COUT) * 2);
  const int tid = threadIdx.x, wave = tid >> 6, lane = tid & 63;
  const int r = lane & 15, kb = lane >> 4;
  const bool folded = p.ab == nullptr;
  const int n_w2 = p.C_hid * CIN / 8, n_w3 = COUT * p.C_hid / 8;
  for (int i = tid; i < n_w3; i += NWAVES * 64) lw3[i] = p.w3[i];
  const long Ts = (p.rps + NT * 16 - 1) / (NT * 16);
  const long G = Ts * p.N;
  const long g_end = G * (blockIdx.x + 1) / gridDim.x;
  long g = G * blockIdx.x / gridDim.x;
  const bool with_res = p.e.res_mode != PYTC_RES_NONE;
  const bool ups = p.e.res_mode == PYTC_RES_UPSAMPLE;
  int staged = -1;

  while (g < g_end) {
    const int n = (int)(g / Ts);
    const long seg_end = min(g_end, (long)(n + 1) * Ts);
    if (staged < 0 || folded) {
      __syncthreads();
      const bf16x8_t* src = p.w2 + (folded ? (long)n * p.w2_stride : 0L);
      for (int i = tid; i < n_w2; i += NWAVES * 64) lw2[i] = src[i];
      const float* b2 = p.b2 + (folded ? (long)n * p.C_hid : 0L);
      for (int i = tid; i < p.C_hid; i += NWAVES * 64) lb2[i] = b2[i];
      staged = n;
      __syncthreads();
    }
    const float* an = folded ? nullptr : p.ab + (long)n * 2 * CIN;
    const long t_base = (long)n * Ts;

    for (long gt = g + wave; gt < seg_end; gt += NWAVES) {
      const long row0 = (gt - t_base) * (NT * 16);
      LdsTile<KS_IN, MO, NT> cur;
      lds_tile_load(cur, p, n, row0, r, kb, with_res);
      long orow[NT];
#pragma unroll
      for (int nt = 0; nt < NT; ++nt) orow[nt] = row0 + nt * 16 + r;

      bf16x8_t bact[KS_IN][NT];
#pragma unroll
      for (int ks = 0; ks < KS_IN; ++ks) {
        if (folded) {
#pragma unroll
          for (int nt = 0; nt < NT; ++nt) bact[ks][nt] = __builtin_bit_cast(bf16x8_t, cur.raw[ks][nt]);
        } else {
          const int k0 = ks * 32 + kb * 8;
          float av[8], bv[8];
          VecIO<float, 4>::load(an + k0, reinterpret_cast<float(&)[4]>(av[0]));
          VecIO<float, 4>::load(an + k0 + 4, reinterpret_cast<float(&)[4]>(av[4]));
          VecIO<float, 4>::load(an + CIN + k0, reinterpret_cast<float(&)[4]>(bv[0]));
          VecIO<float, 4>::load(an + CIN + k0 + 4, reinterpret_cast<float(&)[4]>(bv[4]));
#pragma unroll
          for (int nt = 0; nt < NT; ++nt) {
            float v[8];
            VecIO<bf16_t, 8>::load(reinterpret_cast<const bf16_t*>(&cur.raw[ks][nt]), v);
#pragma unroll
            for (int j = 0; j < 8; ++j) v[j] = fmaf(v[j], av[j], bv[j]);
            bact[ks][nt] = Mma<bf16_t>::from_floats(v);
          }
        }
      }
      f32x4_t acc2[MO][NT];
#pragma unroll
      for (int pr = 0; pr < MO / 2; ++pr) {
        float b[8];
        VecIO<float, 4>::load(p.b3 + pr * 32 + kb * 8, reinterpret_cast<float(&)[4]>(b[0]));
        VecIO<float, 4>::load(p.b3 + pr * 32 + kb * 8 + 4, reinterpret_cast<float(&)[4]>(b[4]));
#pragma unroll
        for (int nt = 0; nt < NT; ++nt) {
          acc2[2 * pr][nt] = f32x4_t{b[0], b[1], b[2], b[3]};
          acc2[2 * pr + 1][nt] = f32x4_t{b[4], b[5], b[6], b[7]};
        }
      }
      for (int hc = 0; hc < p.HC; ++hc) {
        const f32x4_t b2lo = *reinterpret_cast<const f32x4_t*>(lb2 + hc * 32 + kb * 8);
        const f32x4_t b2hi = *reinterpret_cast<const f32x4_t*>(lb2 + hc * 32 + kb * 8 + 4);
        f32x4_t acc1[2][NT];
#pragma unroll
        for (int nt = 0; nt < NT; ++nt) { acc1[0][nt] = b2lo; acc1[1][nt] = b2hi; }
#pragma unroll
        for (int mt = 0; mt < 2; ++mt) {
#pragma unroll
          for (int ks = 0; ks < KS_IN; ++ks) {
            const bf16x8_t a = lw2[((hc * 2 + mt) * KS_IN + ks) * 64 + lane];
#pragma unroll
            for (int nt = 0; nt < NT; ++nt) acc1[mt][nt] = Mma<bf16_t>::mma(a, bact[ks][nt], acc1[mt][nt]);
          }
        }
        h8_t bhh[NT];
#pragma unroll
        for (int nt = 0; nt < NT; ++nt) {
          float gg[8];
#pragma unroll
          for (int j = 0; j < 4; ++j) { gg[j] = acc1[0][nt][j]; gg[4 + j] = acc1[1][nt][j]; }
          bhh[nt] = gelu_h8_from_f32(gg);
        }
#pragma unroll
        for (int mo = 0; mo < MO; ++mo) {
          const h8_t a = lw3[(mo * p.HC + hc) * 64 + lane];
#pragma unroll
          for (int nt = 0; nt < NT; ++nt) acc2[mo][nt] = __builtin_amdgcn_mfma_f32_16x16x32_f16(a, bhh[nt], acc2[mo][nt], 0, 0, 0);
        }
      }
      int upos[NT][3];
      if (ups) {
        const unsigned ur = (unsigned)row0, gw = (unsigned)p.e.Go_w, gh = (unsigned)p.e.Go_h;
        const unsigned t0 = ur / gw;
        const int bx = (int)(ur - t0 * gw);
        const int bz = (int)(t0 / gh);
        const int by = (int)(t0 - (unsigned)bz * gh);
#pragma unroll
        for (int nt = 0; nt < NT; ++nt) {
          int px = bx + nt * 16 + r, py = by, pz = bz;
          while (px >= p.e.Go_w) { px -= p.e.Go_w; ++py; }
          while (py >= p.e.Go_h) { py -= p.e.Go_h; ++pz; }
          upos[nt][0] = pz; upos[nt][1] = py; upos[nt][2] = px;
        }
      }
#pragma unroll
      for (int pr = 0; pr < MO / 2; ++pr) {
#pragma unroll
        for (int nt = 0; nt < NT; ++nt) {
          if (orow[nt] >= p.rps) continue;
          float v[8];
#pragma unroll
          for (int j = 0; j < 4; ++j) { v[j] = acc2[2 * pr][nt][j]; v[4 + j] = acc2[2 * pr + 1][nt][j]; }
          if (with_res) {
            float pre[8];
            VecIO<bf16_t, 8>::load(reinterpret_cast<const bf16_t*>(&cur.res[pr][nt]), pre);
            finish_and_store<bf16_t, 8, false, COUT>(v, p.e, n, orow[nt], pr * 32 + kb * 8, pre, ups ? upos[nt] : nullptr);
          } else {
            finish_and_store<bf16_t, 8, false, COUT>(v, p.e, n, orow[nt], pr * 32 + kb * 8, nullptr, nullptr);
          }
        }
      }
    }
    g = seg_end;
  }
}

template <int KS_IN, int MO, int NT, int NWAVES, int WPS>
static void launch_mlp_lds_v(const MlpLdsParams& p, size_t lds, hipStream_t s) {
  auto kern = &pw_mlp_lds_kernel<KS_IN, MO, NT, NWAVES, WPS>;
  if (!ensure_dynamic_lds(reinterpret_cast<const void*>(kern), 160 * 1024, "pw_mlp_lds")) return;
  const long tiles = ((p.rps + NT * 16 - 1) / (NT * 16)) * p.N;
  const int by_lds = (int)((160 * 1024) / lds), by_waves = WPS * 4 / NWAVES;
  const int per_cu = by_lds < by_waves ? (by_lds < 1 ? 1 : by_lds) : by_waves;
  long blocks = 256L * per_cu;
  const long need = (tiles + NWAVES - 1) / NWAVES;
  if (blocks > need) blocks = need;
  hipLaunchKernelGGL(kern, dim3((unsigned)blocks), dim3(NWAVES * 64), lds, s, p);
}

template <int KS_IN, int MO, int NT>
static void launch_mlp_lds(const MlpLdsParams& p, int variant, hipStream_t s) {
  const size_t lds = (size_t)p.C_hid * (p.C_in + p.C_out) * 2 + (size_t)p.C_hid * 4;
  if (variant == 0) variant = (KS_IN == 4 && MO == 8) ? 3 : (MO == 2 ? 2 : 4);
  switch (variant) {
    case 1: launch_mlp_lds_v<KS_IN, MO, NT, 8, 4>(p, lds, s); break;
    case 2: launch_mlp_lds_v<KS_IN, MO, NT, 16, 4>(p, lds, s); break;
    case 3: launch_mlp_lds_v<KS_IN, MO, NT, 8, 2>(p, lds, s); break;
    default: launch_mlp_lds_v<KS_IN, MO, NT, 12, 3>(p, lds, s); break;
  }
}

}

using namespace pytc;

extern "C" int pytc_pw_mlp_lds_supported(int C_in, int C_hid, int C_out) {
  if (C_in % 32 || C_hid % 32 || C_out % 32) return 0;
  const int ks = C_in / 32, mo = C_out / 16;
  const bool shape = (ks == 2 && mo == 2) || (ks == 2 && mo == 4) || (ks == 4 && mo == 4) || (ks == 4 && mo == 8);
  const size_t lds = (size_t)C_hid * (C_in + C_out) * 2 + (size_t)C_hid * 4;
  return (shape && lds <= 160 * 1024) ? 1 : 0;
}

extern "C" int pytc_pw_mlp_lds_fwd(const pytc_mlp_args* a, void* stream) {
  PYTC_REQUIRE(a && a->t && (a->ab || a->per_sample) && a->w2_packed && a->w3_packed && a->b2 && a->b3 && a->y, "pw_mlp_lds: null pointer");
  PYTC_REQUIRE(!(a->ab && a->per_sample), "pw_mlp_lds: per-sample (norm-folded) expand operands come without an affine");
  PYTC_REQUIRE(a->w3_format == PYTC_W3_F16, "pw_mlp_lds: the projection image must be fp16 (pytc_pw_pack_weight_paired_f16)");
  PYTC_REQUIRE(a->N >= 1 && a->rows_per_sample >= 1, "pw_mlp_lds: bad shape");
  if (!pytc_pw_mlp_lds_supported(a->C_in, a->C_hid, a->C_out)) {
    set_error("pw_mlp_lds: no LDS-resident kernel for C_in=%d C_hid=%d C_out=%d", a->C_in, a->C_hid, a->C_out);
    return PYTC_ERR_UNSUPPORTED;
  }
  PYTC_REQUIRE(a->res_mode == PYTC_RES_NONE || a->res, "pw_mlp_lds: residual mode without residual pointer");
  MlpLdsParams p{};
  p.t = (const bf16_t*)a->t; p.ab = a->ab; p.w2 = (const bf16x8_t*)a->w2_packed; p.b2 = a->b2;
  p.w3 = (const h8_t*)a->w3_packed; p.b3 = a->b3;
  p.rps = a->rows_per_sample; p.N = a->N; p.C_in = a->C_in; p.C_hid = a->C_hid; p.C_out = a->C_out; p.HC = a->C_hid / 32;
  p.w2_stride = (long)(a->C_hid / 16) * (a->C_in / 32) * 64;
  p.e.res = a->res; p.e.res_low = a->res_low; p.e.res_bias = a->res_bias; p.e.y = a->y;
  p.e.rps_out = a->rows_per_sample; p.e.C_out = a->C_out; p.e.res_mode = a->res_mode;
  p.e.nt = stream_nt_policy((long)a->N * a->rows_per_sample * (a->C_in > a->C_out ? a->C_in : a->C_out) * 2);
  p.e.Go_d = p.e.Go_h = p.e.Go_w = p.e.Gl_d = p.e.Gl_h = p.e.Gl_w = 0;
  if (a->res_mode == PYTC_RES_UPSAMPLE) {
    PYTC_REQUIRE((long)a->Di * a->Hi * a->Wi == a->rows_per_sample && !(a->Di & 1) && !(a->Hi & 1) && !(a->Wi & 1) &&
                 a->rows_per_sample < (1L << 31), "pw_mlp_lds: RES_UPSAMPLE needs the (even) output grid");
    p.e.Go_d = a->Di; p.e.Go_h = a->Hi; p.e.Go_w = a->Wi;
    p.e.Gl_d = a->Di / 2; p.e.Gl_h = a->Hi / 2; p.e.Gl_w = a->Wi / 2;
  }
  hipStream_t s = (hipStream_t)stream;
  const int ks = a->C_in / 32, mo = a->C_out / 16;
  const int variant = tuning_get("mlp_lds_variant", 0);
  if (ks == 2 && mo == 2) launch_mlp_lds<2, 2, 2>(p, variant, s);
  else if (ks == 2 && mo == 4) launch_mlp_lds<2, 4, 2>(p, variant, s);
  else if (ks == 4 && mo == 4) launch_mlp_lds<4, 4, 2>(p, variant, s);
  else launch_mlp_lds<4, 8, 2>(p, variant, s);
  PYTC_LAUNCH_CHECK("pw_mlp_lds");
  return PYTC_OK;
}
```

pytorch_connectomics_amd/hip_ops.py:

```python
from __future__ import annotations

import ctypes as C
from typing import Optional, Sequence

import torch

from . import _native as nat

_DT = {torch.float32: nat.F32, torch.bfloat16: nat.BF16}


def dtype_code(dt: torch.dtype) -> int:
    try:
        return _DT[dt]
    except KeyError:
        raise TypeError(f"pytorch_connectomics_amd kernels support float32/bfloat16, got {dt}") from None


def require_device(device, what: str = "this inference path") -> None:
    if torch.device(device).type != "cuda":
        raise RuntimeError(f"{what} (pytorch_connectomics_amd) needs a CUDA(HIP) device: there is no CPU path")


def _dev(t: torch.Tensor, name: str) -> torch.Tensor:
# ... 477 lines not shown
        _run("pack_multi", self.total * 6, nat.lib().pytc_pack_multi, _p(self.table), len(self.rows), self.total, _stream())
        for r in self.rows:
            r[7] = r[0]._version


def packed_paired(w_mat: torch.Tensor, *, transposed: bool = False, f16: bool = False, packs: Optional[StepPacks] = None):
    if packs is None:
        return pw_pack_weight_paired(w_mat, transposed=transposed, f16=f16)
    kind = (PACK_PAIRED_F16 if f16 else PACK_PAIRED) + (1 if transposed else 0)
    hit = packs.lookup(w_mat, kind)
    if hit is not None:
        return hit
    out = pw_pack_weight_paired(w_mat, transposed=transposed, f16=f16)
    c_out, c_in = (w_mat.shape[1], w_mat.shape[0]) if transposed else (w_mat.shape[0], w_mat.shape[1])
    packs.register(w_mat, kind, out, c_out, c_in, (c_in + 31) // 32)
    return out


def packed_rowmajor(w_mat: torch.Tensor, *, transposed: bool = False, packs: Optional[StepPacks] = None) -> torch.Tensor:
    kind = PACK_ROWMAJOR_T if transposed else PACK_ROWMAJOR
    if packs is not None:
        hit = packs.lookup(w_mat, kind)
        if hit is not None:
            return hit
    out = (w_mat.t() if transposed else w_mat).to(torch.bfloat16).contiguous()
    if packs is not None:
        c_out, c_in = (w_mat.shape[1], w_mat.shape[0]) if transposed else (w_mat.shape[0], w_mat.shape[1])
        packs.register(w_mat, kind, out, c_out, c_in, 0)
    return out


def pw_conv_rowmajor_supported(*, c_in: int, c_out: int, in_dtype: torch.dtype, out_dtype: torch.dtype, act: int = nat.ACT_NONE,
                               gather: int = 0) -> bool:
    a = nat.PwArgs()
    a.C_in, a.C_out, a.act, a.gather = int(c_in), int(c_out), int(act), int(gather)
    try:
        a.in_dtype, a.out_dtype, a.w_dtype = dtype_code(in_dtype), dtype_code(out_dtype), dtype_code(torch.bfloat16)
    except Exception:
        return False
    return bool(nat.lib().pytc_pw_conv_rowmajor_supported(C.byref(a)))


def packed_taps(w: torch.Tensor, *, flipped: bool = False, packs: Optional[StepPacks] = None) -> torch.Tensor:
    c, k3 = w.shape[0], w.shape[-1] ** 3
    src = w.detach()
    kind = PACK_TAPS_FLIPPED if flipped else PACK_TAPS
    if packs is not None and src.dtype == torch.float32 and src.is_contiguous():
        hit = packs.lookup(src, kind)
        if hit is not None:
            return hit
    out = src.float().reshape(c, k3).t().contiguous()
    if flipped:
        out = torch.flip(out, dims=[0]).contiguous()
    if packs is not None and src.dtype == torch.float32 and src.is_contiguous():
        packs.register(src, kind, out, c, 1, k3)
    return out


def _check_out(y: torch.Tensor, numel: int, dtype: torch.dtype, what: str) -> None:
    _dev(y, "y")
    if y.dtype != dtype or y.numel() != numel or not y.is_contiguous():
        raise ValueError(f"{what}: output buffer must be a contiguous {dtype} tensor of {numel} elements, got "
                         f"{tuple(y.shape)} {y.dtype} contiguous={y.is_contiguous()}")


def _w3_format(w3p: torch.Tensor) -> int:
    return nat.W3_F16 if w3p.dtype == torch.float16 else nat.W3_BF16


def _folded_operands(ab, w2p: torch.Tensor, b2: torch.Tensor, N: int, c_in: int, c_hid: int) -> int:
    if ab is not None:
        return 0
    if tuple(w2p.shape) != (N, c_hid * c_in) or tuple(b2.shape) != (N, c_hid) or w2p.dtype != torch.bfloat16:
        raise ValueError(f"norm-folded mixer operands must be w2n (N, C_hid*C_in) bf16 and b2n (N, C_hid); got {tuple(w2p.shape)} "
                         f"{w2p.dtype} / {tuple(b2.shape)}")
    return 1


def pw_mlp(t: torch.Tensor, ab: Optional[torch.Tensor], w2p: torch.Tensor, b2: torch.Tensor, w3p: torch.Tensor,
           b3: torch.Tensor, *, N: int, rows_per_sample: int, c_in: int, c_hid: int, c_out: int,
           res: Optional[torch.Tensor] = None, res_mode: int = nat.RES_NONE, grid: Sequence[int] = (0, 0, 0),
           res_low: Optional[torch.Tensor] = None, res_bias: Optional[torch.Tensor] = None,
           y: Optional[torch.Tensor] = None, hidden_pre: Optional[torch.Tensor] = None, lds: bool = False,
           chunked: bool = False, train_nostore: bool = False) -> torch.Tensor:
    _dev(t, "t")
    if t.dtype != torch.bfloat16:
        raise TypeError("pw_mlp runs on bfloat16 activations")
    if y is None:
        y = torch.empty((N, rows_per_sample, c_out), dtype=torch.bfloat16, device=t.device)
    else:
        _check_out(y, N * rows_per_sample * c_out, torch.bfloat16, "pw_mlp")
    a = nat.MlpArgs()
    a.t, a.ab, a.w2_packed, a.b2, a.w3_packed, a.b3 = (t.data_ptr(), None if ab is None else ab.data_ptr(), w2p.data_ptr(),
                                                       b2.data_ptr(), w3p.data_ptr(), b3.data_ptr())
    a.per_sample = _folded_operands(ab, w2p, b2, N, c_in, c_hid)
    a.w3_format = _w3_format(w3p)
    a.res = res.data_ptr() if res is not None else None
    a.res_low = res_low.data_ptr() if res_low is not None else None
    a.res_bias = res_bias.data_ptr() if res_bias is not None else None
    a.y = y.data_ptr()
    a.N, a.rows_per_sample, a.C_in, a.C_hid, a.C_out, a.res_mode = N, rows_per_sample, c_in, c_hid, c_out, res_mode
    a.Di, a.Hi, a.Wi = (int(v) for v in grid)
    nb = N * rows_per_sample * 2 * (c_in + c_out + (c_out if res is not None else 0))
    if hidden_pre is not None:
        _dev(hidden_pre, "hidden_pre")
        _run(f"pw_mlp_train_fwd[{c_in}->{c_hid}->{c_out}]", nb + N * rows_per_sample * 2 * c_hid, nat.lib().pytc_pw_mlp_train_fwd,
             C.byref(a), _p(hidden_pre), _stream())
        return y
    if train_nostore:
        _run(f"pw_mlp_train_fwd_nostore[{c_in}->{c_hid}->{c_out}]", nb, nat.lib().pytc_pw_mlp_train_fwd_nostore, C.byref(a), _stream(),
             symbol=f"pw_mlp_kernel<{c_in // 32}, {c_out // 16}>")
        return y
    if lds:
        _run(f"pw_mlp_fwd[{c_in}->{c_hid}->{c_out}]", nb, nat.lib().pytc_pw_mlp_lds_fwd, C.byref(a), _stream(),
             symbol=f"pw_mlp_lds_kernel<{c_in // 32}, {c_out // 16}>")
        return y
    if chunked:
        _run(f"pw_mlp_fwd[{c_in}->{c_hid}->{c_out}]", nb, nat.lib().pytc_pw_mlp_chunk_fwd, C.byref(a), _stream(),
             symbol=f"pw_mlp_chunk_kernel<{c_in // 32}, {c_out // 16}>")
        return y
    _run(f"pw_mlp_fwd[{c_in}->{c_hid}->{c_out}]", nb, nat.lib().pytc_pw_mlp_fwd, C.byref(a), _stream(),
         symbol=_mlp_symbol(a, f"pw_mlp_kernel<{c_in // 32}, {c_out // 16}>", 0))
    return y


def pw_mlp_lds_supported(c_in: int, c_hid: int, c_out: int) -> bool:
    return bool(nat.lib().pytc_pw_mlp_lds_supported(int(c_in), int(c_hid), int(c_out)))


def pw_mlp_chunk_supported(c_in: int, c_hid: int, c_out: int) -> bool:
    return bool(nat.lib().pytc_pw_mlp_chunk_supported(int(c_in), int(c_hid), int(c_out)))


def pw_gemm_supported(c_in: int, c_out: int) -> bool:
    return bool(nat.lib().pytc_pw_gemm_supported(int(c_in), int(c_out)))


def pw_gemm(x: torch.Tensor, w: torch.Tensor, bias: torch.Tensor, *, N: int, rows_per_sample: int, ab: Optional[torch.Tensor] = None,
            gelu: bool = False, res: Optional[torch.Tensor] = None, res_mode: int = nat.RES_NONE, grid: Sequence[int] = (0, 0, 0),
            res_low: Optional[torch.Tensor] = None, res_bias: Optional[torch.Tensor] = None,
            y: Optional[torch.Tensor] = None) -> torch.Tensor:
    _dev(x, "x"); _dev(w, "w")
    c_out, c_in = int(w.shape[0]), int(w.shape[1])
    if x.dtype not in (torch.bfloat16, torch.float16) or w.dtype != x.dtype or not w.is_contiguous() or int(x.shape[-1]) != c_in:
        raise TypeError(f"pw_gemm: x {tuple(x.shape)} {x.dtype} / w {tuple(w.shape)} {w.dtype}: same 16-bit type, w (C_out, C_in) contiguous")
    out_dt = torch.float16 if gelu else torch.bfloat16
    if y is None:
        y = torch.empty((N, rows_per_sample, c_out), dtype=out_dt, device=x.device)
    else:
        _check_out(y, N * rows_per_sample * c_out, out_dt, "pw_gemm")
    nb = N * rows_per_sample * 2 * (c_in + c_out + (c_out if res is not None else 0)) + 2 * c_in * c_out
    _run(f"pw_gemm[{c_in}->{c_out}]", nb, nat.lib().pytc_pw_gemm_fwd, _p(x), _p(w), _p(bias), _p(ab), _p(y), N, rows_per_sample, c_in,
         c_out, int(x.dtype == torch.float16), int(gelu), _p(res), _p(res_low), _p(res_bias), int(res_mode), *(int(v) for v in grid),
         _stream(), flops=2 * N * rows_per_sample * c_in * c_out, symbol="pw_gemm_lds_kernel")
    return y


def pw_mlp_up_supported(c_in: int, c_hid: int, c_out: int) -> bool:
    return bool(nat.lib().pytc_pw_mlp_up_supported(int(c_in), int(c_hid), int(c_out)))


def pw_mlp_up(x_low: torch.Tensor, taps: torch.Tensor, dw_bias: Optional[torch.Tensor], ab: torch.Tensor, w2p: torch.Tensor,
              b2: torch.Tensor, w3p: torch.Tensor, b3: torch.Tensor, skip: torch.Tensor, *, c_hid: int, c_out: int,
              res_low: Optional[torch.Tensor] = None, res_bias: Optional[torch.Tensor] = None) -> torch.Tensor:
    _dev(x_low, "x_low"); _dev(skip, "skip"); _dev(taps, "taps")
    if x_low.dtype != torch.bfloat16 or skip.dtype != torch.bfloat16:
        raise TypeError("pw_mlp_up runs on bfloat16 activations")
    N, D, H, W, c_in = x_low.shape
    if tuple(skip.shape) != (N, 2 * D, 2 * H, 2 * W, c_out):
        raise ValueError(f"pw_mlp_up: skip shape {tuple(skip.shape)} does not match the up-sampled grid")
    y = torch.empty((N, 2 * D, 2 * H, 2 * W, c_out), dtype=torch.bfloat16, device=x_low.device)
    a = nat.MlpArgs()
    a.t, a.ab, a.w2_packed, a.b2, a.w3_packed, a.b3 = (x_low.data_ptr(), ab.data_ptr(), w2p.data_ptr(), b2.data_ptr(),
                                                       w3p.data_ptr(), b3.data_ptr())
    if w3p.dtype != torch.bfloat16:
        raise TypeError("pw_mlp_up takes the bf16 image of the projection weights")
    a.res = skip.data_ptr()
    if dw_bias is None:
        dw_bias = torch.zeros((c_in,), dtype=torch.float32, device=x_low.device)
    if res_bias is None:
        res_bias = torch.zeros((c_out,), dtype=torch.float32, device=x_low.device)
    a.res_low = res_low.data_ptr() if res_low is not None else None
    a.res_bias = res_bias.data_ptr()
    a.y = y.data_ptr()
    a.N, a.rows_per_sample, a.C_in, a.C_hid, a.C_out, a.res_mode = N, 8 * D * H * W, c_in, c_hid, c_out, nat.RES_UPSAMPLE
    a.Di, a.Hi, a.Wi = D, H, W
    nb = _nbytes(x_low, skip, y) + (_nbytes(res_low) if res_low is not None else 0)
    _run(f"pw_mlp_up_fwd[{c_in}->{c_hid}->{c_out}]", nb, nat.lib().pytc_pw_mlp_up_fwd, C.byref(a), _p(taps), _p(dw_bias),
         _stream())
    return y


def stem_dwconv3d_supported(c_in: int, c: int, K: int) -> bool:
    return bool(nat.lib().pytc_stem_dwconv3d_supported(int(c_in), int(c), int(K)))


def stem_dwconv3d_pack(stem_w: torch.Tensor, stem_b: torch.Tensor, w_taps: torch.Tensor, bias: Optional[torch.Tensor]):
    wx = (w_taps * stem_w.view(1, -1)).contiguous()
    wb = (w_taps * stem_b.view(1, -1)).contiguous()
    cst = (wb.sum(0) + (bias if bias is not None else 0.0)).contiguous()
    image = torch.empty((nat.lib().pytc_stem_dwconv3d_mfma_image_bytes(),), dtype=torch.uint8, device=wx.device)
    _run("stem_dwconv3d_pack_mfma", 0, nat.lib().pytc_stem_dwconv3d_pack_mfma, _p(wx), _p(wb), _p(cst), _p(image), _stream())
    return wx, wb, cst, image


def stem_dwconv3d(x: torch.Tensor, packed):
# ... 1387 lines not shown
```

pytorch_connectomics_amd/models/architectures/mednext.py:

```python
from __future__ import annotations

import os
from typing import Dict, List, Optional, Sequence, Union

import torch
import torch.nn as nn

from ... import _native as nat
from ... import hip_ops as ops

SMALL_ROWS_TWO_GEMMS = int(os.environ.get("PYTC_MIXER_TWO_GEMM_ROWS", "0"))

L0_SUBBATCH = int(os.environ.get("PYTC_L0_SUBBATCH", "0"))


def _conv_nd(dim: str):
    if dim == "3d":
        return nn.Conv3d, nn.ConvTranspose3d
    if dim == "2d":
        return nn.Conv2d, nn.ConvTranspose2d
    raise ValueError(f"dim must be '2d' or '3d', got {dim!r}")


class _ChannelLayerNorm(nn.Module):
# ... 31 lines not shown
            self.grn_gamma = nn.Parameter(torch.zeros(shape))
        self.kind = "block"

    def forward(self, x, dummy_tensor=None):
        raise RuntimeError("MedNeXt blocks execute through MedNeXt.forward (HIP engine); they are parameter "
                           "holders and cannot be called directly")


class MedNeXtDownBlock(MedNeXtBlock):
    def __init__(self, in_channels, out_channels, exp_r=4, kernel_size=7, do_res=False, norm_type="group",
                 dim="3d", grn=False):
        super().__init__(in_channels, out_channels, exp_r, kernel_size, do_res=False, norm_type=norm_type,
                         dim=dim, grn=grn)
        conv, _ = _conv_nd(dim)
        self.resample_do_res = do_res
        if do_res:
            self.res_conv = conv(in_channels, out_channels, kernel_size=1, stride=2)
        self.conv1 = conv(in_channels, in_channels, kernel_size=kernel_size, stride=2,
                          padding=kernel_size // 2, groups=in_channels)
        self.kind = "down"


class MedNeXtUpBlock(MedNeXtBlock):
    def __init__(self, in_channels, out_channels, exp_r=4, kernel_size=7, do_res=False, norm_type="group",
                 dim="3d", grn=False):
        super().__init__(in_channels, out_channels, exp_r, kernel_size, do_res=False, norm_type=norm_type,
                         dim=dim, grn=grn)
        _, convt = _conv_nd(dim)
        self.resample_do_res = do_res
        if do_res:
            self.res_conv = convt(in_channels, out_channels, kernel_size=1, stride=2)
        self.conv1 = convt(in_channels, in_channels, kernel_size=kernel_size, stride=2,
                           padding=kernel_size // 2, groups=in_channels)
        self.kind = "up"


class OutBlock(nn.Module):
    def __init__(self, in_channels: int, n_classes: int, dim: str = "3d"):
        super().__init__()
        _, convt = _conv_nd(dim)
        self.conv_out = convt(in_channels, n_classes, kernel_size=1)

    def forward(self, x, dummy_tensor=None):
        raise RuntimeError("OutBlock executes through MedNeXt.forward (HIP engine)")


class _WeightCache:

    def __init__(self):
        self._store: Dict = {}

    def get(self, key, params: Sequence[torch.Tensor], make):
        sig = tuple((p.data_ptr(), p._version) for p in params)
        hit = self._store.get(key)
        if hit is not None and hit[0] == sig:
            return hit[1]
        with torch.no_grad():
            val = make()
        self._store[key] = (sig, val)
        return val

    def clear(self):
        self._store.clear()


def _f32(p: Optional[torch.Tensor]) -> Optional[torch.Tensor]:
    return None if p is None else p.detach().float().contiguous()


class HipBlockOps:

    def __init__(self):
        self.cache = _WeightCache()
        self.fused = True
        self.fuse_up = os.environ.get("PYTC_FUSE_UP", "0") == "1"
        self.fuse_up_cin = (64, 128)
        self.fold_norm = os.environ.get("PYTC_FOLD_NORM", "1") != "0"
        self.deep_gemm_rows = int(os.environ.get("PYTC_DEEP_GEMM_ROWS", "8192"))
        self.deep_gemm_cin = int(os.environ.get("PYTC_DEEP_GEMM_CIN", "0"))
        self.lds_mixer_rows = int(os.environ.get("PYTC_LDS_MIXER_ROWS", "131072"))
        self.chunk_mixer_rows = int(os.environ.get("PYTC_CHUNK_MIXER_ROWS", "16384"))
        self.chunk_mixer_hid = int(os.environ.get("PYTC_CHUNK_MIXER_HID", "512"))
        self.fuse_block = int(os.environ.get("PYTC_FUSE_BLOCK", "0"))

    def _taps(self, conv: nn.Module):
        w = conv.weight
        def make():
            c = w.shape[0]
            k = w.shape[-1]
            w3 = embed_stencil_2d(w.detach().float()) if w.dim() == 4 else w.detach().float()
            return w3.reshape(c, k ** 3).t().contiguous(), k
        return self.cache.get(("taps", id(conv)), [w], make)

    def _pw(self, conv: nn.Module, dt: torch.dtype, transposed: bool = False):
        w = conv.weight
        def make():
            w2 = w.detach().float().reshape(w.shape[0], w.shape[1]).contiguous()
            return ops.pw_pack_weight(w2, dt, transposed=transposed)
        return self.cache.get(("pw", id(conv), dt, transposed), [w], make)

    def _pw_paired(self, conv: nn.Module, transposed: bool = False, project: bool = False):
        w = conv.weight
        f16 = bool(project and ops.MLP_F16_PROJECT)
        def make():
            w2 = w.detach().float().reshape(w.shape[0], w.shape[1]).contiguous()
            return ops.pw_pack_weight_paired(w2, transposed=transposed, f16=f16)
        return self.cache.get(("pwp", id(conv), transposed, f16), [w], make)

    def _w2_matrix(self, conv: nn.Module):
        w = conv.weight
        return self.cache.get(("w2mat", id(conv)), [w], lambda: w.detach().float().reshape(w.shape[0], w.shape[1]).contiguous())

    def _fold(self, m, st, count, C: int, c_hid: int):
        gamma, beta = self._vec(m.norm, "weight", m.norm.weight), self._vec(m.norm, "bias", m.norm.bias)
        if self.fold_norm and ops.groupnorm_fold_mlp_supported(C, c_hid):
            w2n, b2n = ops.groupnorm_fold_mlp(st, count, gamma, beta, m.norm.eps, self._w2_matrix(m.conv2),
                                              self._vec(m.conv2, "bias", m.conv2.bias))
            return None, w2n, b2n
        return (ops.groupnorm_finalize(st, count, gamma, beta, m.norm.eps), self._pw_paired(m.conv2),
                self._vec(m.conv2, "bias", m.conv2.bias))

    def _head_w(self, conv: nn.Module):
        w = conv.weight
        def make():
            return ops.pack_head_fragment(w.detach().float().reshape(w.shape[0], w.shape[1]).t().contiguous())
        return self.cache.get(("headw", id(conv)), [w], make)

    def _grn(self, m, h: torch.Tensor, N: int, grid, c_hid: int, kind: str) -> torch.Tensor:
        Do, Ho, Wo = grid
        hv = h.view(N, Do, Ho, Wo, c_hid)
        core = hv[:, 1:, 1:, 1:].contiguous() if kind == "up" else hv
        sumsq = ops.channel_stats(core)[:, :, 1].sum(1)
        gx = sumsq.clamp_min(0).sqrt()
        nx = gx / (gx.mean(1, keepdim=True) + 1e-6)
        g = self._vec(m, "grn_gamma", m.grn_gamma).view(1, c_hid)
        b = self._vec(m, "grn_beta", m.grn_beta).view(1, c_hid)
        ab = torch.stack([g * nx + 1.0, b.expand(N, c_hid)], 1).contiguous()
        return ops.affine_act(hv, ab, nat.ACT_NONE, 0.0).view(N, Do * Ho * Wo, c_hid)

    def _vec(self, owner, name: str, p: Optional[torch.Tensor]):
        if p is None:
            return None
        return self.cache.get(("vec", id(owner), name), [p], lambda: _f32(p).reshape(-1))

    def pointwise(self, x: torch.Tensor, conv: nn.Module, *, out_dtype=None, transposed=False, act=nat.ACT_NONE):
        N = x.shape[0]
        spatial = tuple(x.shape[1:-1])
        rows = 1
        for s in spatial:
            rows *= s
        c_in = x.shape[-1]
        c_out = conv.weight.shape[1] if transposed else conv.weight.shape[0]
        dt = x.dtype if x.dtype == torch.bfloat16 else torch.float32
        wdt = torch.bfloat16 if (dt == torch.bfloat16 or (out_dtype == torch.bfloat16)) else torch.float32
        wp = self._pw(conv, wdt, transposed)
        y = ops.pw_conv(x, wp, self._vec(conv, "bias", conv.bias), N=N, rows_per_sample=rows, c_in=c_in,
                        c_out=c_out, out_dtype=out_dtype or x.dtype, act=act)
        return y.view(N, *spatial, c_out)

    def block(self, m: MedNeXtBlock, x: torch.Tensor, skip: Optional[torch.Tensor] = None, head: Optional[nn.Module] = None,
              out: Optional[torch.Tensor] = None, proj: Optional[nn.Module] = None):
        if m.dim == "2d":
            if x.shape[1] != 1:
                raise ValueError(f"dim='2d' MedNeXt blocks take depth-1 volumes (N, 1, H, W, C), got {tuple(x.shape)}")
            if m.kind == "up":
                sk3 = None
# ... 104 lines not shown
                            res=res, res_mode=nat.RES_ADD if res is not None else nat.RES_NONE, **G)
        else:
            if skip is None:
                skip = torch.zeros((N, Do, Ho, Wo, c_out), dtype=dt, device=x.device)
            res_low = res_bias = None
            if m.resample_do_res:
                res_bias = self._vec(m.res_conv, "bias", m.res_conv.bias)
                res_low = ops.pw_conv(x, self._pw(m.res_conv, dt, transposed=True), res_bias, N=N,
                                      rows_per_sample=D * H * W, c_in=C, c_out=c_out, out_dtype=dt)
            y = ops.pw_conv(h, w3, b3, N=N, rows_per_sample=rows, c_in=c_hid, c_out=c_out, out_dtype=dt,
                            res=skip, res_mode=nat.RES_UPSAMPLE, grid=(Do, Ho, Wo), res_low=res_low,
                            res_bias=res_bias, **G)
        return y.view(N, Do, Ho, Wo, c_out)


def _block_dwmix(self, m, x, taps, b1, c_hid, c_out, head=None, out=None):
    N, D, H, W, C = x.shape
    _, st = ops.dwconv3d(x, taps, b1, K=3, store=False)
    w2n, b2n = ops.groupnorm_fold_mlp(st, float(D * H * W), self._vec(m.norm, "weight", m.norm.weight), self._vec(m.norm, "bias", m.norm.bias),
                                      m.norm.eps, self._w2_matrix(m.conv2), self._vec(m.conv2, "bias", m.conv2.bias))
    w3, b3 = self._pw_paired(m.conv3, project=True), self._vec(m.conv3, "bias", m.conv3.bias)
    if head is not None:
        _, logits = ops.dwmix(x, taps, b1, w2n, b2n, w3, b3, c_hid=c_hid, c_out=c_out, residual=bool(m.do_res),
                              head_w=self._head_w(head), head_b=self._vec(head, "bias", head.bias), store_y=False)
        return None, logits
    if out is not None and tuple(out.shape) != (N, D, H, W, c_out):
        raise ValueError(f"block output buffer {tuple(out.shape)} != {(N, D, H, W, c_out)}")
    return ops.dwmix(x, taps, b1, w2n, b2n, w3, b3, c_hid=c_hid, c_out=c_out, residual=bool(m.do_res), y=out)


HipBlockOps._block_dwmix = None


def _stem_block_fused(self, stem: nn.Module, m, x_cl: torch.Tensor, out: Optional[torch.Tensor] = None) -> Optional[torch.Tensor]:
    N, D, H, W, cin = x_cl.shape
    C = stem.weight.shape[0]
    K = m.conv1.weight.shape[-1]
    if (cin != 1 or x_cl.dtype != torch.float32 or stem.bias is None or m.kind != "block" or not m.do_res or m.grn
            or not isinstance(m.norm, nn.GroupNorm) or m.dim != "3d" or m.conv2.bias is None or m.conv3.bias is None
            or m.conv1.weight.shape[0] != C or W % 4 != 0 or not ops.stem_dwconv3d_supported(cin, C, K)):
        return None
    c_hid, c_out = m.conv2.weight.shape[0], m.conv3.weight.shape[0]
    if c_out != C or not ops.pw_mlp_supported(C, c_hid, c_out):
        return None
    sw = self.cache.get(("stemw", id(stem)), [stem.weight], lambda: stem.weight.detach().float().reshape(-1).bfloat16().float().contiguous())
    sb = self._vec(stem, "bias", stem.bias)
    taps, _ = self._taps(m.conv1)
    packed = self.cache.get(("stemdw", id(stem), id(m.conv1)), [stem.weight, stem.bias, m.conv1.weight, m.conv1.bias],
                            lambda: ops.stem_dwconv3d_pack(sw, sb, taps, self._vec(m.conv1, "bias", m.conv1.bias)))
    t, st = ops.stem_dwconv3d(x_cl, packed)
    rows = D * H * W
    ab, w2x, b2x = self._fold(m, st, float(rows), C, c_hid)
    y = ops.pw_mlp_stemres(t, ab, w2x, b2x,
                           self._pw_paired(m.conv3, project=True), self._vec(m.conv3, "bias", m.conv3.bias), x_cl.reshape(N, rows), sw, sb,
                           N=N, rows_per_sample=rows, c_in=C, c_hid=c_hid, c_out=c_out,
                           y=None if out is None else out.view(N, rows, c_out))
    return y.view(N, D, H, W, c_out)


HipBlockOps._stem_block_fused = None


def _block_fused(self, m, x, t, ab, skip, ishape, oshape, c_hid, c_out, out=None, w2=None, b2=None):
    N, D, H, W, C = ishape
    Do, Ho, Wo = oshape
    rows = Do * Ho * Wo
    dt = torch.bfloat16
    if w2 is None:
        w2, b2 = self._pw_paired(m.conv2), self._vec(m.conv2, "bias", m.conv2.bias)
    w3, b3 = self._pw_paired(m.conv3, project=True), self._vec(m.conv3, "bias", m.conv3.bias)
    kw = dict(N=N, rows_per_sample=rows, c_in=C, c_hid=c_hid, c_out=c_out)
    if (self.lds_mixer_rows and N * rows >= self.lds_mixer_rows and w3.dtype == torch.float16
            and ops.pw_mlp_lds_supported(C, c_hid, c_out)):
        kw["lds"] = True
    chunk_ok = (self.chunk_mixer_rows and N * rows >= self.chunk_mixer_rows and w3.dtype == torch.float16
                and ops.pw_mlp_chunk_supported(C, c_hid, c_out))
    if chunk_ok and (c_hid >= self.chunk_mixer_hid or (C, c_out) == (128, 64)):
        kw.pop("lds", None)
        kw["chunked"] = True
    if out is not None:
        if tuple(out.shape) != (N, Do, Ho, Wo, c_out):
            raise ValueError(f"block output buffer {tuple(out.shape)} != {(N, Do, Ho, Wo, c_out)}")
        kw["y"] = out.view(N, rows, c_out)
    if m.kind == "block":
        y = ops.pw_mlp(t, ab, w2, b2, w3, b3, res=x if m.do_res else None,
                       res_mode=nat.RES_ADD if m.do_res else nat.RES_NONE, **kw)
    elif m.kind == "down":
        res = None
        if m.resample_do_res:
            paired = ops.pw_conv_paired_supported(c_in=C, c_out=c_out, in_dtype=dt, out_dtype=dt, gather=2)
            wres = self._pw_paired(m.res_conv) if paired else self._pw(m.res_conv, dt)
            res = ops.pw_conv(x, wres, self._vec(m.res_conv, "bias", m.res_conv.bias), N=N, rows_per_sample=rows,
                              c_in=C, c_out=c_out, out_dtype=dt, gather=2, grid=(D, H, W), w_paired=paired)
        y = ops.pw_mlp(t, ab, w2, b2, w3, b3, res=res, res_mode=nat.RES_ADD if res is not None else nat.RES_NONE, **kw)
    else:
        if skip is None:
            skip = torch.zeros((N, Do, Ho, Wo, c_out), dtype=dt, device=x.device)
        res_low = res_bias = None
        if m.resample_do_res:
            res_bias = self._vec(m.res_conv, "bias", m.res_conv.bias)
            paired = ops.pw_conv_paired_supported(c_in=C, c_out=c_out, in_dtype=dt, out_dtype=dt)
            wres = self._pw_paired(m.res_conv, transposed=True) if paired else self._pw(m.res_conv, dt, transposed=True)
            res_low = ops.pw_conv(x, wres, res_bias, N=N, rows_per_sample=D * H * W, c_in=C, c_out=c_out,
                                  out_dtype=dt, w_paired=paired)
        y = ops.pw_mlp(t, ab, w2, b2, w3, b3, res=skip, res_mode=nat.RES_UPSAMPLE, grid=(Do, Ho, Wo),
                       res_low=res_low, res_bias=res_bias, **kw)
    return y.view(N, Do, Ho, Wo, c_out)


def _block_deep_gemm(self, m, x, t, ab, skip, ishape, oshape, c_hid, c_out, out=None):
    N, D, H, W, C = ishape
    Do, Ho, Wo = oshape
    rows = Do * Ho * Wo
    dt = torch.bfloat16
    w2 = self.cache.get(("gw2", id(m.conv2)), [m.conv2.weight],
                        lambda: m.conv2.weight.detach().float().reshape(c_hid, C).to(torch.bfloat16).contiguous())
    w3 = self.cache.get(("gw3", id(m.conv3)), [m.conv3.weight],
                        lambda: m.conv3.weight.detach().float().reshape(c_out, c_hid).to(torch.float16).contiguous())
    b2, b3 = self._vec(m.conv2, "bias", m.conv2.bias), self._vec(m.conv3, "bias", m.conv3.bias)
    h = ops.pw_gemm(t.view(N, rows, C), w2, b2, N=N, rows_per_sample=rows, ab=ab, gelu=True)
    kw = dict(N=N, rows_per_sample=rows)
    if out is not None:
        kw["y"] = out.view(N, rows, c_out)
    if m.kind == "block":
        y = ops.pw_gemm(h, w3, b3, res=x if m.do_res else None, res_mode=nat.RES_ADD if m.do_res else nat.RES_NONE, **kw)
    elif m.kind == "down":
        res = None
        if m.resample_do_res:
            paired = ops.pw_conv_paired_supported(c_in=C, c_out=c_out, in_dtype=dt, out_dtype=dt, gather=2)
            wres = self._pw_paired(m.res_conv) if paired else self._pw(m.res_conv, dt)
            res = ops.pw_conv(x, wres, self._vec(m.res_conv, "bias", m.res_conv.bias), N=N, rows_per_sample=rows,
                              c_in=C, c_out=c_out, out_dtype=dt, gather=2, grid=(D, H, W), w_paired=paired)
        y = ops.pw_gemm(h, w3, b3, res=res, res_mode=nat.RES_ADD if res is not None else nat.RES_NONE, **kw)
    else:
        if skip is None:
            skip = torch.zeros((N, Do, Ho, Wo, c_out), dtype=dt, device=x.device)
        res_low = res_bias = None
        if m.resample_do_res:
            res_bias = self._vec(m.res_conv, "bias", m.res_conv.bias)
            paired = ops.pw_conv_paired_supported(c_in=C, c_out=c_out, in_dtype=dt, out_dtype=dt)
            wres = self._pw_paired(m.res_conv, transposed=True) if paired else self._pw(m.res_conv, dt, transposed=True)
            res_low = ops.pw_conv(x, wres, res_bias, N=N, rows_per_sample=D * H * W, c_in=C, c_out=c_out, out_dtype=dt, w_paired=paired)
        y = ops.pw_gemm(h, w3, b3, res=skip, res_mode=nat.RES_UPSAMPLE, grid=(Do, Ho, Wo), res_low=res_low, res_bias=res_bias, **kw)
    return y.view(N, Do, Ho, Wo, c_out)


def _up_block_fused(self, m, x, skip, taps, b1, c_hid, c_out):
    N, D, H, W, C = x.shape
    dt = torch.bfloat16
    _, st = ops.dwconv3d(x, taps, b1, K=3, transposed=True, stats=True, store=False)
    ab = ops.groupnorm_finalize(st, float((2 * D - 1) * (2 * H - 1) * (2 * W - 1)), self._vec(m.norm, "weight", m.norm.weight),
                                self._vec(m.norm, "bias", m.norm.bias), m.norm.eps)
    res_low = res_bias = None
    if m.resample_do_res:
        res_bias = self._vec(m.res_conv, "bias", m.res_conv.bias)
        paired = ops.pw_conv_paired_supported(c_in=C, c_out=c_out, in_dtype=dt, out_dtype=dt)
        wres = self._pw_paired(m.res_conv, transposed=True) if paired else self._pw(m.res_conv, dt, transposed=True)
        res_low = ops.pw_conv(x, wres, res_bias, N=N, rows_per_sample=D * H * W, c_in=C, c_out=c_out, out_dtype=dt,
                              w_paired=paired)
    return ops.pw_mlp_up(x, taps, b1, ab, self._pw_paired(m.conv2), self._vec(m.conv2, "bias", m.conv2.bias),
                         self._pw_paired(m.conv3), self._vec(m.conv3, "bias", m.conv3.bias), skip.contiguous(),
                         c_hid=c_hid, c_out=c_out, res_low=res_low, res_bias=res_bias)


HipBlockOps._up_block_fused = _up_block_fused
HipBlockOps._block_deep_gemm = _block_deep_gemm
HipBlockOps._block_fused = _block_fused
HipBlockOps._stem_block_fused = _stem_block_fused
HipBlockOps._block_dwmix = _block_dwmix


def resolve_compute_dtype(module_pref: Optional[torch.dtype]) -> torch.dtype:
    if module_pref is not None:
        return module_pref
    if torch.is_autocast_enabled("cuda"):
        adt = torch.get_autocast_dtype("cuda")
        if adt == torch.bfloat16:
            return torch.bfloat16
        if adt == torch.float16:
            raise RuntimeError("fp16 autocast is not supported by the MI355X engine; use bf16-mixed")
    return torch.float32


def embed_stencil_2d(w: torch.Tensor) -> torch.Tensor:
    k = w.shape[-1]
# ... 239 lines not shown
```

Measured before the change: 1.795 billion voxels/s.

## Fold resampling residual 1x1 conv into the MLP mixer kernel for down/up blocks

In the MedNeXt down and up blocks, the 1x1x1 residual conv (strided gather for down, transposed low-res for up) is now computed inside the pointwise MLP mixer kernel rather than by a separate pw_conv launch. The mixer reads the low-res or strided input directly and runs extra MFMA work in its epilogue, using ds_bpermute to redistribute fragments in the chunk and LDS paths. This drops a kernel launch and the round trip of the intermediate residual tensor through memory. In exchange it raises register pressure, and in the up block some work is recomputed or redistributed per tile. The fold is on by default and gated by supported shapes.

```diff
diff --git a/include/pytc_hip.h b/include/pytc_hip.h
--- a/include/pytc_hip.h
+++ b/include/pytc_hip.h
@@ -7,7 +7,7 @@
 extern "C" {
 #endif
 
-#define PYTC_ABI_VERSION 5
+#define PYTC_ABI_VERSION 6
 
 #define PYTC_OK 0
 #define PYTC_ERR_INVALID 1
@@ -185,9 +185,18 @@
   int Di, Hi, Wi;
   int w3_format;
   int per_sample;
+  int res_fold;
+  const void* res_x;
+  const void* res_w;
 } pytc_mlp_args;
 #define PYTC_W3_BF16 0
 #define PYTC_W3_F16 1
+#define PYTC_RES_FOLD_NONE 0
+#define PYTC_RES_FOLD_DOWN 1
+#define PYTC_RES_FOLD_UP 2
+#define PYTC_MLP_ENTRY_FWD 0
+#define PYTC_MLP_ENTRY_LDS 1
+#define PYTC_MLP_ENTRY_CHUNK 2
 
 int pytc_pw_gemm_supported(int C_in, int C_out);
 int pytc_pw_gemm_fwd(const void* x, const void* w, const float* bias, const float* ab, void* y, int N, int64_t rows_per_sample,
@@ -200,6 +209,7 @@
 int pytc_pw_pack_weight_paired_f16(const float* w, int C_out, int C_in, int transposed, void* packed_f16,
                                    void* stream);
 int pytc_pw_mlp_fwd(const pytc_mlp_args* a, void* stream);
+int pytc_pw_mlp_res_fold_supported(int C_in, int C_hid, int C_out, int kind, int entry);
 
 int pytc_pw_mlp_lds_supported(int C_in, int C_hid, int C_out);
 int pytc_pw_mlp_lds_fwd(const pytc_mlp_args* a, void* stream);
diff --git a/pytorch_connectomics_amd/_native.py b/pytorch_connectomics_amd/_native.py
--- a/pytorch_connectomics_amd/_native.py
+++ b/pytorch_connectomics_amd/_native.py
@@ -5,7 +5,7 @@
 from pathlib import Path
 
 LIB_PATH = Path(__file__).resolve().parent / "lib" / "libpytc_hip.so"
-ABI_VERSION = 5
+ABI_VERSION = 6
 
 F32, BF16 = 0, 1
 OK = 0
@@ -39,10 +39,13 @@
         ("N", C.c_int), ("rows_per_sample", C.c_int64),
         ("C_in", C.c_int), ("C_hid", C.c_int), ("C_out", C.c_int), ("res_mode", C.c_int),
         ("Di", C.c_int), ("Hi", C.c_int), ("Wi", C.c_int), ("w3_format", C.c_int), ("per_sample", C.c_int),
+        ("res_fold", C.c_int), ("res_x", C.c_void_p), ("res_w", C.c_void_p),
     ]
 
 
 W3_BF16, W3_F16 = 0, 1
+RES_FOLD_NONE, RES_FOLD_DOWN, RES_FOLD_UP = 0, 1, 2
+MLP_ENTRY_FWD, MLP_ENTRY_LDS, MLP_ENTRY_CHUNK = 0, 1, 2
 NORM_NONE, NORM_ZSCORE, NORM_MINMAX, NORM_DIVIDE = 0, 1, 2, 3
 RAW_DTYPES = {"uint8": 0, "int8": 1, "uint16": 2, "int16": 3, "uint32": 4, "int32": 5, "float32": 6, "float64": 7}
 
@@ -242,6 +245,7 @@
     "pytc_pack_multi": (C.c_int, [C.c_void_p, C.c_int, C.c_int64, C.c_void_p]),
     "pytc_pw_pack_weight_paired_f16": (C.c_int, [C.c_void_p, C.c_int, C.c_int, C.c_int, C.c_void_p, C.c_void_p]),
     "pytc_pw_mlp_fwd": (C.c_int, [C.POINTER(MlpArgs), C.c_void_p]),
+    "pytc_pw_mlp_res_fold_supported": (C.c_int, [C.c_int, C.c_int, C.c_int, C.c_int, C.c_int]),
     "pytc_pw_mlp_lds_supported": (C.c_int, [C.c_int, C.c_int, C.c_int]),
     "pytc_pw_mlp_lds_fwd": (C.c_int, [C.POINTER(MlpArgs), C.c_void_p]),
     "pytc_pw_mlp_dma_applies": (C.c_int, [C.POINTER(MlpArgs), C.c_int]),
diff --git a/pytorch_connectomics_amd/csrc/pw_common.h b/pytorch_connectomics_amd/csrc/pw_common.h
--- a/pytorch_connectomics_amd/csrc/pw_common.h
+++ b/pytorch_connectomics_amd/csrc/pw_common.h
@@ -57,6 +57,14 @@
   int nt;
 };
 
+struct ResFoldParams {
+  const bf16_t* x;
+  const bf16x8_t* w;
+  const float* bias;
+  long rps_in;
+  int Hi, Wi, Ho, Wo;
+};
+
 typedef unsigned int pytc_u32x4_t __attribute__((ext_vector_type(4)));
 template <typename V>
 __device__ __forceinline__ V ld_stream(const V* ptr, int nt) {
@@ -72,7 +80,8 @@
 
 template <typename TO, int NCH, bool GELU_BWD = false, int COUT = 0>
 __device__ __forceinline__ void finish_and_store(float (&v)[NCH], const EpiParams& e, int n, long orow, int o0,
-                                                 const float* pre = nullptr, const int* pos = nullptr) {
+                                                 const float* pre = nullptr, const int* pos = nullptr,
+                                                 const float* rl_pre = nullptr) {
   const int C_out = COUT > 0 ? COUT : e.C_out;
   TO* yn = reinterpret_cast<TO*>(e.y) + (long)n * e.rps_out * C_out;
   const TO* resn = e.res ? reinterpret_cast<const TO*>(e.res) + (long)n * e.rps_out * C_out : nullptr;
@@ -156,7 +165,10 @@
     } else {
       const int oz = pz - 1, oy = py - 1, ox = px - 1;
       float rl[NCH];
-      if (e.res_low && !((oz | oy | ox) & 1)) {
+      if (rl_pre && !((oz | oy | ox) & 1)) {
+#pragma unroll
+        for (int i = 0; i < NCH; ++i) rl[i] = rl_pre[i];
+      } else if (e.res_low && !((oz | oy | ox) & 1)) {
         const TO* rp = reinterpret_cast<const TO*>(e.res_low) +
                        ((((long)n * e.Gl_d + (oz >> 1)) * e.Gl_h + (oy >> 1)) * e.Gl_w + (ox >> 1)) * C_out + o0;
         if (full) VecIO<TO, NCH>::load(rp, rl);
@@ -187,6 +199,82 @@
 #pragma unroll
     for (int i = 0; i < NCH; ++i)
       if (o0 + i < C_out) yn[off + i] = from_f32<TO>(v[i]);
+  }
+}
+
+template <int KS, int MO, int NT>
+__device__ __forceinline__ void res_low_fold(const ResFoldParams& f, const EpiParams& e, int n, long row0, long rps, int bx, int by, int bz,
+                                             int lane, uint4 (&rl)[MO / 2][NT]) {
+  static_assert(NT % 2 == 0, "two 16-row tiles share one packed fragment");
+  const int j = lane & 15, kb = lane >> 4;
+  bool hit[NT / 2];
+  uint4 xr[NT / 2][KS];
+  bool any = false;
+#pragma unroll
+  for (int fr = 0; fr < NT / 2; ++fr) {
+    int px = bx + fr * 32 + 2 * j + 1, py = by, pz = bz;
+    while (px >= e.Go_w) { px -= e.Go_w; ++py; }
+    while (py >= e.Go_h) { py -= e.Go_h; ++pz; }
+    hit[fr] = (px & py & pz & 1) && row0 + fr * 32 + 2 * j + 1 < rps;
+    any = any || hit[fr];
+  }
+  if (!__any(any)) {
+#pragma unroll
+    for (int pr = 0; pr < MO / 2; ++pr)
+#pragma unroll
+      for (int nt = 0; nt < NT; ++nt) rl[pr][nt] = uint4{0u, 0u, 0u, 0u};
+    return;
+  }
+#pragma unroll
+  for (int fr = 0; fr < NT / 2; ++fr) {
+    int px = bx + fr * 32 + 2 * j + 1, py = by, pz = bz;
+    while (px >= e.Go_w) { px -= e.Go_w; ++py; }
+    while (py >= e.Go_h) { py -= e.Go_h; ++pz; }
+    const long lrow = hit[fr] ? ((long)((pz - 1) >> 1) * e.Gl_h + ((py - 1) >> 1)) * e.Gl_w + ((px - 1) >> 1) : 0L;
+    const bf16_t* xp = f.x + ((long)n * f.rps_in + lrow) * (KS * 32) + kb * 8;
+#pragma unroll
+    for (int ks = 0; ks < KS; ++ks) xr[fr][ks] = *reinterpret_cast<const uint4*>(xp + ks * 32);
+  }
+#pragma unroll
+  for (int pr = 0; pr < MO / 2; ++pr) {
+    float b[8];
+#pragma unroll
+    for (int i = 0; i < 8; ++i) b[i] = 0.f;
+    if (f.bias) {
+      VecIO<float, 4>::load(f.bias + pr * 32 + kb * 8, reinterpret_cast<float(&)[4]>(b[0]));
+      VecIO<float, 4>::load(f.bias + pr * 32 + kb * 8 + 4, reinterpret_cast<float(&)[4]>(b[4]));
+    }
+    f32x4_t acc[2][NT / 2];
+#pragma unroll
+    for (int fr = 0; fr < NT / 2; ++fr) {
+      acc[0][fr] = f32x4_t{b[0], b[1], b[2], b[3]};
+      acc[1][fr] = f32x4_t{b[4], b[5], b[6], b[7]};
+    }
+#pragma unroll
+    for (int mt = 0; mt < 2; ++mt)
+#pragma unroll
+      for (int ks = 0; ks < KS; ++ks) {
+        const bf16x8_t a = f.w[((long)(pr * 2 + mt) * KS + ks) * 64 + lane];
+#pragma unroll
+        for (int fr = 0; fr < NT / 2; ++fr) acc[mt][fr] = Mma<bf16_t>::mma(a, __builtin_bit_cast(bf16x8_t, xr[fr][ks]), acc[mt][fr]);
+      }
+#pragma unroll
+    for (int fr = 0; fr < NT / 2; ++fr) {
+      float v[8];
+#pragma unroll
+      for (int i = 0; i < 4; ++i) { v[i] = acc[0][fr][i]; v[4 + i] = acc[1][fr][i]; }
+      const uint4 rounded = __builtin_bit_cast(uint4, Mma<bf16_t>::from_floats(v));
+#pragma unroll
+      for (int half = 0; half < 2; ++half) {
+        const int src = (kb * 16 + half * 8 + (j >> 1)) * 4;
+        uint4 got;
+        got.x = (unsigned)__builtin_amdgcn_ds_bpermute(src, (int)rounded.x);
+        got.y = (unsigned)__builtin_amdgcn_ds_bpermute(src, (int)rounded.y);
+        got.z = (unsigned)__builtin_amdgcn_ds_bpermute(src, (int)rounded.z);
+        got.w = (unsigned)__builtin_amdgcn_ds_bpermute(src, (int)rounded.w);
+        rl[pr][2 * fr + half] = got;
+      }
+    }
   }
 }
 
diff --git a/pytorch_connectomics_amd/csrc/pw_mlp_chunk_kernels.hip b/pytorch_connectomics_amd/csrc/pw_mlp_chunk_kernels.hip
--- a/pytorch_connectomics_amd/csrc/pw_mlp_chunk_kernels.hip
+++ b/pytorch_connectomics_amd/csrc/pw_mlp_chunk_kernels.hip
@@ -13,6 +13,7 @@
   long rps;
   int N, C_in, C_hid, C_out, HC;
   long w2_stride;
+  ResFoldParams rf;
 };
 
 __device__ __forceinline__ void chunk_glds16(const void* gsrc, unsigned lds_dst) {
@@ -21,7 +22,7 @@
                : "=&s"(keep) : "v"(gsrc), "s"(lds_dst) : "memory");
 }
 
-template <int KS_IN, int MO, int NW, int WPS>
+template <int KS_IN, int MO, int NW, int WPS, bool RESFOLD = false>
 __global__ void __launch_bounds__(NW * 64, WPS)
 pw_mlp_chunk_kernel(MlpChunkParams p) {
   constexpr int NT = 2, CIN = KS_IN * 32, COUT = MO * 16;
@@ -159,12 +160,14 @@
 
   if (row0 >= p.rps) return;
   int upos[NT][3];
+  uint4 rlow[RESFOLD ? MO / 2 : 1][RESFOLD ? NT : 1];
   if (ups) {
     const unsigned ur = (unsigned)row0, gw = (unsigned)p.e.Go_w, gh = (unsigned)p.e.Go_h;
     const unsigned t0 = ur / gw;
     const int bx = (int)(ur - t0 * gw);
     const int bz = (int)(t0 / gh);
     const int by = (int)(t0 - (unsigned)bz * gh);
+    if constexpr (RESFOLD) res_low_fold<KS_IN, MO, NT>(p.rf, p.e, n, row0, p.rps, bx, by, bz, lane, rlow);
 #pragma unroll
     for (int nt = 0; nt < NT; ++nt) {
       int px = bx + nt * 16 + r, py = by, pz = bz;
@@ -181,14 +184,21 @@
       float v[8];
 #pragma unroll
       for (int j = 0; j < 4; ++j) { v[j] = acc2[2 * pr][nt][j]; v[4 + j] = acc2[2 * pr + 1][nt][j]; }
-      finish_and_store<bf16_t, 8, false, COUT>(v, p.e, n, orow[nt], pr * 32 + kb * 8, nullptr, (with_res && ups) ? upos[nt] : nullptr);
-    }
-  }
-}
-
-template <int KS_IN, int MO, int NW, int WPS>
+      if constexpr (RESFOLD) {
+        float rl[8];
+        VecIO<bf16_t, 8>::load(reinterpret_cast<const bf16_t*>(&rlow[pr][nt]), rl);
+        finish_and_store<bf16_t, 8, false, COUT>(v, p.e, n, orow[nt], pr * 32 + kb * 8, nullptr, (with_res && ups) ? upos[nt] : nullptr,
+                                                 rl);
+      } else {
+        finish_and_store<bf16_t, 8, false, COUT>(v, p.e, n, orow[nt], pr * 32 + kb * 8, nullptr, (with_res && ups) ? upos[nt] : nullptr);
+      }
+    }
+  }
+}
+
+template <int KS_IN, int MO, int NW, int WPS, bool RESFOLD>
 static void launch_mlp_chunk_v(const MlpChunkParams& p, hipStream_t s) {
-  auto kern = &pw_mlp_chunk_kernel<KS_IN, MO, NW, WPS>;
+  auto kern = &pw_mlp_chunk_kernel<KS_IN, MO, NW, WPS, RESFOLD>;
   const size_t lds = (size_t)3 * (2 * KS_IN + MO) * 1024 + (size_t)(p.C_hid + MO * 16) * 4;
   if (!ensure_dynamic_lds(reinterpret_cast<const void*>(kern), 160 * 1024, "pw_mlp_chunk")) return;
   const long wg_rows = (long)NW * 32;
@@ -196,14 +206,14 @@
   hipLaunchKernelGGL(kern, grid, block, lds, s, p);
 }
 
-template <int KS_IN, int MO>
+template <int KS_IN, int MO, bool RESFOLD = false>
 static void launch_mlp_chunk(const MlpChunkParams& p, int variant, hipStream_t s) {
   if (variant == 0) variant = (KS_IN == 8) ? 1 : 3;
   switch (variant) {
-    case 2: launch_mlp_chunk_v<KS_IN, MO, 12, 3>(p, s); break;
-    case 3: launch_mlp_chunk_v<KS_IN, MO, 8, 4>(p, s); break;
-    case 4: launch_mlp_chunk_v<KS_IN, MO, 16, 4>(p, s); break;
-    default: launch_mlp_chunk_v<KS_IN, MO, 8, 2>(p, s); break;
+    case 2: launch_mlp_chunk_v<KS_IN, MO, 12, 3, RESFOLD>(p, s); break;
+    case 3: launch_mlp_chunk_v<KS_IN, MO, 8, 4, RESFOLD>(p, s); break;
+    case 4: launch_mlp_chunk_v<KS_IN, MO, 16, 4, RESFOLD>(p, s); break;
+    default: launch_mlp_chunk_v<KS_IN, MO, 8, 2, RESFOLD>(p, s); break;
   }
 }
 
@@ -229,6 +239,15 @@
   }
   PYTC_REQUIRE(a->res_mode == PYTC_RES_NONE || a->res, "pw_mlp_chunk: residual mode without residual pointer");
   PYTC_REQUIRE(a->res_mode == PYTC_RES_NONE || a->res_mode == PYTC_RES_ADD || a->res_mode == PYTC_RES_UPSAMPLE, "pw_mlp_chunk: residual mode");
+  PYTC_REQUIRE(a->res_fold == PYTC_RES_FOLD_NONE || a->res_fold == PYTC_RES_FOLD_UP, "pw_mlp_chunk: res_fold %d", a->res_fold);
+  if (a->res_fold == PYTC_RES_FOLD_UP) {
+    PYTC_REQUIRE(a->res_mode == PYTC_RES_UPSAMPLE && a->res_x && a->res_w && !a->res_low,
+                 "pw_mlp_chunk: the folded residual conv takes res_x / res_w with RES_UPSAMPLE and no res_low");
+    if (!pytc_pw_mlp_res_fold_supported(a->C_in, a->C_hid, a->C_out, PYTC_RES_FOLD_UP, PYTC_MLP_ENTRY_CHUNK)) {
+      set_error("pw_mlp_chunk: no kernel with the residual conv folded in for C_in=%d C_hid=%d C_out=%d", a->C_in, a->C_hid, a->C_out);
+      return PYTC_ERR_UNSUPPORTED;
+    }
+  }
   MlpChunkParams p{};
   p.t = (const bf16_t*)a->t; p.ab = a->ab; p.w2 = (const bf16x8_t*)a->w2_packed; p.b2 = a->b2;
   p.w3 = (const h8_t*)a->w3_packed; p.b3 = a->b3;
@@ -247,6 +266,13 @@
   hipStream_t s = (hipStream_t)stream;
   const int ks = a->C_in / 32, mo = a->C_out / 16;
   const int variant = tuning_get("mlp_chunk_variant", 0);
+  if (a->res_fold == PYTC_RES_FOLD_UP) {
+    p.rf.x = (const bf16_t*)a->res_x; p.rf.w = (const bf16x8_t*)a->res_w; p.rf.bias = a->res_bias;
+    p.rf.rps_in = (long)p.e.Gl_d * p.e.Gl_h * p.e.Gl_w;
+    launch_mlp_chunk<4, 4, true>(p, variant, s);
+    PYTC_LAUNCH_CHECK("pw_mlp_chunk");
+    return PYTC_OK;
+  }
   if (ks == 2 && mo == 2) launch_mlp_chunk<2, 2>(p, variant, s);
   else if (ks == 2 && mo == 4) launch_mlp_chunk<2, 4>(p, variant, s);
   else if (ks == 2 && mo == 8) launch_mlp_chunk<2, 8>(p, variant, s);
diff --git a/pytorch_connectomics_amd/csrc/pw_mlp_kernels.hip b/pytorch_connectomics_amd/csrc/pw_mlp_kernels.hip
--- a/pytorch_connectomics_amd/csrc/pw_mlp_kernels.hip
+++ b/pytorch_connectomics_amd/csrc/pw_mlp_kernels.hip
@@ -26,6 +26,7 @@
   bf16_t* hp;
   int round_h;
   const bf16_t* hp_in;
+  ResFoldParams rf;
 };
 
 constexpr int GELU_LUT_N = 1024;
@@ -43,13 +44,13 @@
   return regs <= 64 ? 4 : (regs <= 112 ? 3 : (regs <= 200 ? 2 : 1));
 }
 
-template <int KS_IN, int MO, int NT, int GELU_MODE, bool HEAD = false, bool STEMRES = false, bool STOREH = false, bool BWD = false>
-__global__ void __launch_bounds__(256, mlp_waves_per_simd(KS_IN, MO, NT))
-pw_mlp_kernel(MlpParams p) {
+template <int KS_IN, int MO, int NT, int GELU_MODE, bool HEAD, bool STEMRES, bool STOREH, bool BWD, bool RESCONV>
+__device__ __forceinline__ void pw_mlp_body(const MlpParams& p) {
   constexpr int CIN = KS_IN * 32, COUT = MO * 16;
   static_assert(MO % 2 == 0, "C_out must be a multiple of 32");
   static_assert(!STEMRES || (MO == 2 && (MO / 2) * NT <= 4), "the stem-recomputing residual covers C_out = 32");
   static_assert(!HEAD || MO == 2, "the fused head covers C_out = 32");
+  static_assert(!RESCONV || !(HEAD || STEMRES || STOREH || BWD), "the folded residual conv is a mode of the plain inference mixer");
   __shared__ __attribute__((aligned(16))) float2 lut[GELU_MODE == 2 ? GELU_LUT_N : 1];
   if constexpr (GELU_MODE == 2) {
     const uint4* src = reinterpret_cast<const uint4*>(g_gelu_lut);
@@ -58,7 +59,7 @@
     dst[threadIdx.x + 256] = src[threadIdx.x + 256];
     __syncthreads();
   }
-  constexpr bool PREFETCH_RES = (MO / 2) * NT <= 4;
+  constexpr bool PREFETCH_RES = !RESCONV && (MO / 2) * NT <= 4;
   const int wave = threadIdx.x >> 6, lane = threadIdx.x & 63;
   const int n = blockIdx.y;
   constexpr bool WARM = KS_IN * MO >= 32;
@@ -144,6 +145,23 @@
       }
   }
 
+  constexpr bool XRES_EARLY = MO <= 4;
+  bf16x8_t xres[RESCONV ? KS_IN : 1][RESCONV ? NT : 1];
+  auto load_xres = [&]() {
+    const bf16_t* xn = p.rf.x + (long)n * p.rf.rps_in * CIN;
+#pragma unroll
+    for (int nt = 0; nt < NT; ++nt) {
+      long rr = orow[nt] < p.rps ? orow[nt] : p.rps - 1;
+      const int ox = (int)(rr % p.rf.Wo);
+      const long tq = rr / p.rf.Wo;
+      const int oy = (int)(tq % p.rf.Ho), oz = (int)(tq / p.rf.Ho);
+      rr = ((long)(2 * oz) * p.rf.Hi + 2 * oy) * p.rf.Wi + 2 * ox;
+#pragma unroll
+      for (int ks = 0; ks < KS_IN; ++ks) xres[RESCONV ? ks : 0][RESCONV ? nt : 0] = *reinterpret_cast<const bf16x8_t*>(xn + rr * CIN + ks * 32 + kb * 8);
+    }
+  };
+  if constexpr (RESCONV && XRES_EARLY) load_xres();
+
   f32x4_t acc2[MO][NT];
 #pragma unroll
   for (int pr = 0; pr < MO / 2; ++pr) {
@@ -265,6 +283,7 @@
     }
     return;
   }
+  if constexpr (RESCONV && !XRES_EARLY) load_xres();
   int upos[NT][3];
   const bool ups = p.e.res_mode == PYTC_RES_UPSAMPLE;
   if (ups) {
@@ -283,6 +302,29 @@
   }
 #pragma unroll
   for (int pr = 0; pr < MO / 2; ++pr) {
+    f32x4_t racc[RESCONV ? 2 : 1][RESCONV ? NT : 1];
+    if constexpr (RESCONV) {
+      float b[8];
+#pragma unroll
+      for (int j = 0; j < 8; ++j) b[j] = 0.f;
+      if (p.rf.bias) {
+        VecIO<float, 4>::load(p.rf.bias + pr * 32 + kb * 8, reinterpret_cast<float(&)[4]>(b[0]));
+        VecIO<float, 4>::load(p.rf.bias + pr * 32 + kb * 8 + 4, reinterpret_cast<float(&)[4]>(b[4]));
+      }
+#pragma unroll
+      for (int nt = 0; nt < NT; ++nt) {
+        racc[0][nt] = f32x4_t{b[0], b[1], b[2], b[3]};
+        racc[1][nt] = f32x4_t{b[4], b[5], b[6], b[7]};
+      }
+#pragma unroll
+      for (int mt = 0; mt < 2; ++mt)
+#pragma unroll
+        for (int ks = 0; ks < KS_IN; ++ks) {
+          const bf16x8_t a = p.rf.w[((long)(pr * 2 + mt) * KS_IN + ks) * 64 + lane];
+#pragma unroll
+          for (int nt = 0; nt < NT; ++nt) racc[mt][nt] = Mma<bf16_t>::mma(a, xres[ks][nt], racc[mt][nt]);
+        }
+    }
 #pragma unroll
     for (int nt = 0; nt < NT; ++nt) {
       if (orow[nt] >= p.rps) continue;
@@ -292,7 +334,14 @@
         v[j] = acc2[2 * pr][nt][j];
         v[4 + j] = acc2[2 * pr + 1][nt][j];
       }
-      if (use_pre) {
+      if constexpr (RESCONV) {
+        float rv[8], pre[8];
+#pragma unroll
+        for (int j = 0; j < 4; ++j) { rv[j] = racc[0][nt][j]; rv[4 + j] = racc[1][nt][j]; }
+        const bf16x8_t rb = Mma<bf16_t>::from_floats(rv);
+        VecIO<bf16_t, 8>::load(reinterpret_cast<const bf16_t*>(&rb), pre);
+        finish_and_store<bf16_t, 8, false, COUT>(v, p.e, n, orow[nt], pr * 32 + kb * 8, pre, nullptr);
+      } else if (use_pre) {
         float pre[8];
         VecIO<bf16_t, 8>::load(reinterpret_cast<const bf16_t*>(&rpre[PREFETCH_RES ? pr : 0][PREFETCH_RES ? nt : 0]), pre);
         finish_and_store<bf16_t, 8, false, COUT>(v, p.e, n, orow[nt], pr * 32 + kb * 8, pre, ups ? upos[nt] : nullptr);
@@ -301,6 +350,18 @@
       }
     }
   }
+}
+
+template <int KS_IN, int MO, int NT, int GELU_MODE, bool HEAD = false, bool STEMRES = false, bool STOREH = false, bool BWD = false>
+__global__ void __launch_bounds__(256, mlp_waves_per_simd(KS_IN, MO, NT))
+pw_mlp_kernel(MlpParams p) {
+  pw_mlp_body<KS_IN, MO, NT, GELU_MODE, HEAD, STEMRES, STOREH, BWD, false>(p);
+}
+
+template <int KS_IN, int MO, int NT, int GELU_MODE>
+__global__ void __launch_bounds__(256, mlp_waves_per_simd(KS_IN, MO, NT))
+pw_mlp_resconv_kernel(MlpParams p) {
+  pw_mlp_body<KS_IN, MO, NT, GELU_MODE, false, false, false, false, true>(p);
 }
 
 
@@ -775,6 +836,16 @@
 
 extern "C" int pytc_pw_mlp_supported(int C_in, int C_hid, int C_out) { return mlp_shape_ok(C_in, C_hid, C_out) ? 1 : 0; }
 
+extern "C" int pytc_pw_mlp_res_fold_supported(int C_in, int C_hid, int C_out, int kind, int entry) {
+  if (kind == PYTC_RES_FOLD_DOWN && entry == PYTC_MLP_ENTRY_FWD)
+    return (mlp_shape_ok(C_in, C_hid, C_out) && ((C_in == 32 && C_out == 64) || (C_in == 64 && C_out == 128))) ? 1 : 0;
+  if (kind == PYTC_RES_FOLD_UP && entry == PYTC_MLP_ENTRY_LDS)
+    return (C_in == 64 && C_out == 32 && pytc_pw_mlp_lds_supported(C_in, C_hid, C_out)) ? 1 : 0;
+  if (kind == PYTC_RES_FOLD_UP && entry == PYTC_MLP_ENTRY_CHUNK)
+    return (C_in == 128 && C_out == 64 && pytc_pw_mlp_chunk_supported(C_in, C_hid, C_out)) ? 1 : 0;
+  return 0;
+}
+
 extern "C" int pytc_groupnorm_fold_mlp(const float* stats, int slots, float count, const float* gamma, const float* beta,
                                        float eps, const float* w2, const float* b2, void* w2n, float* b2n, float* ab_out, int N,
                                        int C, int C_hid, void* stream) {
@@ -969,7 +1040,7 @@
     set_error("pw_mlp: no fused kernel for C_in=%d C_hid=%d C_out=%d", a->C_in, a->C_hid, a->C_out);
     return PYTC_ERR_UNSUPPORTED;
   }
-  PYTC_REQUIRE(a->res_mode == PYTC_RES_NONE || a->res, "pw_mlp: residual mode without residual pointer");
+  PYTC_REQUIRE(a->res_mode == PYTC_RES_NONE || a->res || a->res_fold == PYTC_RES_FOLD_DOWN, "pw_mlp: residual mode without residual pointer");
   PYTC_REQUIRE(a->res_mode == PYTC_RES_NONE || a->res_mode == PYTC_RES_ADD || a->res_mode == PYTC_RES_UPSAMPLE,
                "pw_mlp: unsupported res_mode %d", a->res_mode);
   MlpParams p{};
@@ -986,6 +1057,28 @@
   p.round_h = round_h ? 1 : 0;
   p.w3_f16 = a->w3_format == PYTC_W3_F16 ? 1 : 0;
   PYTC_REQUIRE(!(p.w3_f16 && hp_in), "pw_mlp_bwd: the backward mixer takes bf16 weight images");
+  PYTC_REQUIRE(a->res_fold == PYTC_RES_FOLD_NONE || a->res_fold == PYTC_RES_FOLD_DOWN, "pw_mlp: res_fold %d", a->res_fold);
+  if (a->res_fold == PYTC_RES_FOLD_DOWN) {
+    PYTC_REQUIRE(!hp && !hp_in && !round_h && p.w3_f16, "pw_mlp: the folded residual conv is an inference mode with the fp16 projection image");
+    PYTC_REQUIRE(a->res_mode == PYTC_RES_ADD && a->res_x && a->res_w, "pw_mlp: the folded residual conv takes res_x / res_w with RES_ADD");
+    if (!pytc_pw_mlp_res_fold_supported(a->C_in, a->C_hid, a->C_out, PYTC_RES_FOLD_DOWN, PYTC_MLP_ENTRY_FWD)) {
+      set_error("pw_mlp: no kernel with the residual conv folded in for C_in=%d C_hid=%d C_out=%d", a->C_in, a->C_hid, a->C_out);
+      return PYTC_ERR_UNSUPPORTED;
+    }
+    const int Do = (a->Di - 1) / 2 + 1, Ho = (a->Hi - 1) / 2 + 1, Wo = (a->Wi - 1) / 2 + 1;
+    PYTC_REQUIRE(a->Di >= 1 && a->Hi >= 1 && a->Wi >= 1 && (long)Do * Ho * Wo == a->rows_per_sample,
+                 "pw_mlp: the folded residual conv needs the block input's grid (Di, Hi, Wi); rows_per_sample is its stride-2 grid");
+    p.rf.x = (const bf16_t*)a->res_x; p.rf.w = (const bf16x8_t*)a->res_w; p.rf.bias = a->res_bias;
+    p.rf.rps_in = (long)a->Di * a->Hi * a->Wi; p.rf.Hi = a->Hi; p.rf.Wi = a->Wi; p.rf.Ho = Ho; p.rf.Wo = Wo;
+    p.e.res = a->y;
+    p.e.res_low = nullptr; p.e.res_bias = nullptr;
+    const long rows_per_block = 4L * (a->C_in == 32 ? 4 : 2) * 16;
+    dim3 grid((unsigned)((p.rps + rows_per_block - 1) / rows_per_block), (unsigned)a->N), block(256);
+    if (a->C_in == 32) hipLaunchKernelGGL((pw_mlp_resconv_kernel<1, 4, 4, 3>), grid, block, 0, (hipStream_t)stream, p);
+    else hipLaunchKernelGGL((pw_mlp_resconv_kernel<2, 8, 2, 3>), grid, block, 0, (hipStream_t)stream, p);
+    PYTC_LAUNCH_CHECK("pw_mlp_resconv");
+    return PYTC_OK;
+  }
   if (a->res_mode == PYTC_RES_UPSAMPLE) {
     PYTC_REQUIRE((long)a->Di * a->Hi * a->Wi == a->rows_per_sample && !(a->Di & 1) && !(a->Hi & 1) && !(a->Wi & 1),
                  "pw_mlp: RES_UPSAMPLE needs the (even) output grid");
diff --git a/pytorch_connectomics_amd/csrc/pw_mlp_lds_kernels.hip b/pytorch_connectomics_amd/csrc/pw_mlp_lds_kernels.hip
--- a/pytorch_connectomics_amd/csrc/pw_mlp_lds_kernels.hip
+++ b/pytorch_connectomics_amd/csrc/pw_mlp_lds_kernels.hip
@@ -15,6 +15,7 @@
   long rps;
   int N, C_in, C_hid, C_out, HC;
   long w2_stride;
+  ResFoldParams rf;
 };
 
 template <int KS_IN, int MO, int NT>
@@ -46,7 +47,7 @@
   }
 }
 
-template <int KS_IN, int MO, int NT, int NWAVES, int WPS>
+template <int KS_IN, int MO, int NT, int NWAVES, int WPS, bool RESFOLD = false>
 __global__ void __launch_bounds__(NWAVES * 64, WPS)
 pw_mlp_lds_kernel(MlpLdsParams p) {
   constexpr int CIN = KS_IN * 32, COUT = MO * 16;
@@ -156,12 +157,14 @@
         }
       }
       int upos[NT][3];
+      uint4 rlow[RESFOLD ? MO / 2 : 1][RESFOLD ? NT : 1];
       if (ups) {
         const unsigned ur = (unsigned)row0, gw = (unsigned)p.e.Go_w, gh = (unsigned)p.e.Go_h;
         const unsigned t0 = ur / gw;
         const int bx = (int)(ur - t0 * gw);
         const int bz = (int)(t0 / gh);
         const int by = (int)(t0 - (unsigned)bz * gh);
+        if constexpr (RESFOLD) res_low_fold<KS_IN, MO, NT>(p.rf, p.e, n, row0, p.rps, bx, by, bz, lane, rlow);
 #pragma unroll
         for (int nt = 0; nt < NT; ++nt) {
           int px = bx + nt * 16 + r, py = by, pz = bz;
@@ -181,7 +184,14 @@
           if (with_res) {
             float pre[8];
             VecIO<bf16_t, 8>::load(reinterpret_cast<const bf16_t*>(&cur.res[pr][nt]), pre);
-            finish_and_store<bf16_t, 8, false, COUT>(v, p.e, n, orow[nt], pr * 32 + kb * 8, pre, ups ? upos[nt] : nullptr);
+            if constexpr (RESFOLD) {
+              float rl[8];
+              VecIO<bf16_t, 8>::load(reinterpret_cast<const bf16_t*>(&rlow[pr][nt]), rl);
+              finish_and_store<bf16_t, 8, false, COUT>(v, p.e, n, orow[nt], pr * 32 + kb * 8, pre, ups ? upos[nt] : nullptr,
+                                                       rl);
+            } else {
+              finish_and_store<bf16_t, 8, false, COUT>(v, p.e, n, orow[nt], pr * 32 + kb * 8, pre, ups ? upos[nt] : nullptr);
+            }
           } else {
             finish_and_store<bf16_t, 8, false, COUT>(v, p.e, n, orow[nt], pr * 32 + kb * 8, nullptr, nullptr);
           }
@@ -192,9 +202,9 @@
   }
 }
 
-template <int KS_IN, int MO, int NT, int NWAVES, int WPS>
+template <int KS_IN, int MO, int NT, int NWAVES, int WPS, bool RESFOLD>
 static void launch_mlp_lds_v(const MlpLdsParams& p, size_t lds, hipStream_t s) {
-  auto kern = &pw_mlp_lds_kernel<KS_IN, MO, NT, NWAVES, WPS>;
+  auto kern = &pw_mlp_lds_kernel<KS_IN, MO, NT, NWAVES, WPS, RESFOLD>;
   if (!ensure_dynamic_lds(reinterpret_cast<const void*>(kern), 160 * 1024, "pw_mlp_lds")) return;
   const long tiles = ((p.rps + NT * 16 - 1) / (NT * 16)) * p.N;
   const int by_lds = (int)((160 * 1024) / lds), by_waves = WPS * 4 / NWAVES;
@@ -205,15 +215,15 @@
   hipLaunchKernelGGL(kern, dim3((unsigned)blocks), dim3(NWAVES * 64), lds, s, p);
 }
 
-template <int KS_IN, int MO, int NT>
+template <int KS_IN, int MO, int NT, bool RESFOLD = false>
 static void launch_mlp_lds(const MlpLdsParams& p, int variant, hipStream_t s) {
   const size_t lds = (size_t)p.C_hid * (p.C_in + p.C_out) * 2 + (size_t)p.C_hid * 4;
   if (variant == 0) variant = (KS_IN == 4 && MO == 8) ? 3 : (MO == 2 ? 2 : 4);
   switch (variant) {
-    case 1: launch_mlp_lds_v<KS_IN, MO, NT, 8, 4>(p, lds, s); break;
-    case 2: launch_mlp_lds_v<KS_IN, MO, NT, 16, 4>(p, lds, s); break;
-    case 3: launch_mlp_lds_v<KS_IN, MO, NT, 8, 2>(p, lds, s); break;
-    default: launch_mlp_lds_v<KS_IN, MO, NT, 12, 3>(p, lds, s); break;
+    case 1: launch_mlp_lds_v<KS_IN, MO, NT, 8, 4, RESFOLD>(p, lds, s); break;
+    case 2: launch_mlp_lds_v<KS_IN, MO, NT, 16, 4, RESFOLD>(p, lds, s); break;
+    case 3: launch_mlp_lds_v<KS_IN, MO, NT, 8, 2, RESFOLD>(p, lds, s); break;
+    default: launch_mlp_lds_v<KS_IN, MO, NT, 12, 3, RESFOLD>(p, lds, s); break;
   }
 }
 
@@ -239,6 +249,15 @@
     return PYTC_ERR_UNSUPPORTED;
   }
   PYTC_REQUIRE(a->res_mode == PYTC_RES_NONE || a->res, "pw_mlp_lds: residual mode without residual pointer");
+  PYTC_REQUIRE(a->res_fold == PYTC_RES_FOLD_NONE || a->res_fold == PYTC_RES_FOLD_UP, "pw_mlp_lds: res_fold %d", a->res_fold);
+  if (a->res_fold == PYTC_RES_FOLD_UP) {
+    PYTC_REQUIRE(a->res_mode == PYTC_RES_UPSAMPLE && a->res_x && a->res_w && !a->res_low,
+                 "pw_mlp_lds: the folded residual conv takes res_x / res_w with RES_UPSAMPLE and no res_low");
+    if (!pytc_pw_mlp_res_fold_supported(a->C_in, a->C_hid, a->C_out, PYTC_RES_FOLD_UP, PYTC_MLP_ENTRY_LDS)) {
+      set_error("pw_mlp_lds: no kernel with the residual conv folded in for C_in=%d C_hid=%d C_out=%d", a->C_in, a->C_hid, a->C_out);
+      return PYTC_ERR_UNSUPPORTED;
+    }
+  }
   MlpLdsParams p{};
   p.t = (const bf16_t*)a->t; p.ab = a->ab; p.w2 = (const bf16x8_t*)a->w2_packed; p.b2 = a->b2;
   p.w3 = (const h8_t*)a->w3_packed; p.b3 = a->b3;
@@ -257,6 +276,13 @@
   hipStream_t s = (hipStream_t)stream;
   const int ks = a->C_in / 32, mo = a->C_out / 16;
   const int variant = tuning_get("mlp_lds_variant", 0);
+  if (a->res_fold == PYTC_RES_FOLD_UP) {
+    p.rf.x = (const bf16_t*)a->res_x; p.rf.w = (const bf16x8_t*)a->res_w; p.rf.bias = a->res_bias;
+    p.rf.rps_in = (long)p.e.Gl_d * p.e.Gl_h * p.e.Gl_w;
+    launch_mlp_lds<2, 2, 2, true>(p, variant, s);
+    PYTC_LAUNCH_CHECK("pw_mlp_lds");
+    return PYTC_OK;
+  }
   if (ks == 2 && mo == 2) launch_mlp_lds<2, 2, 2>(p, variant, s);
   else if (ks == 2 && mo == 4) launch_mlp_lds<2, 4, 2>(p, variant, s);
   else if (ks == 4 && mo == 4) launch_mlp_lds<4, 4, 2>(p, variant, s);
diff --git a/pytorch_connectomics_amd/hip_ops.py b/pytorch_connectomics_amd/hip_ops.py
--- a/pytorch_connectomics_amd/hip_ops.py
+++ b/pytorch_connectomics_amd/hip_ops.py
@@ -583,7 +583,8 @@
            res: Optional[torch.Tensor] = None, res_mode: int = nat.RES_NONE, grid: Sequence[int] = (0, 0, 0),
            res_low: Optional[torch.Tensor] = None, res_bias: Optional[torch.Tensor] = None,
            y: Optional[torch.Tensor] = None, hidden_pre: Optional[torch.Tensor] = None, lds: bool = False,
-           chunked: bool = False, train_nostore: bool = False) -> torch.Tensor:
+           chunked: bool = False, train_nostore: bool = False, res_x: Optional[torch.Tensor] = None,
+           res_w: Optional[torch.Tensor] = None) -> torch.Tensor:
     _dev(t, "t")
     if t.dtype != torch.bfloat16:
         raise TypeError("pw_mlp runs on bfloat16 activations")
@@ -603,6 +604,28 @@
     a.N, a.rows_per_sample, a.C_in, a.C_hid, a.C_out, a.res_mode = N, rows_per_sample, c_in, c_hid, c_out, res_mode
     a.Di, a.Hi, a.Wi = (int(v) for v in grid)
     nb = N * rows_per_sample * 2 * (c_in + c_out + (c_out if res is not None else 0))
+    fold = False
+    if res_x is not None or res_w is not None:
+        if res_x is None or res_w is None or hidden_pre is not None or train_nostore:
+            raise ValueError("pw_mlp: the folded residual conv takes res_x and res_w together, on the inference entries")
+        _dev(res_x, "res_x"); _dev(res_w, "res_w")
+        if res_x.dtype != torch.bfloat16 or res_w.dtype != torch.bfloat16 or not res_x.is_contiguous() or int(res_x.shape[-1]) != c_in:
+            raise TypeError(f"pw_mlp: res_x must be a contiguous bf16 (N, D, H, W, {c_in}) tensor and res_w a paired bf16 image")
+        if res_mode == nat.RES_ADD and res is None and res_low is None:
+            a.res_fold = nat.RES_FOLD_DOWN
+            want = (N,) + tuple(int(v) for v in grid)
+        elif res_mode == nat.RES_UPSAMPLE and res is not None and res_low is None and res_bias is not None:
+            a.res_fold = nat.RES_FOLD_UP
+            want = (N,) + tuple(int(v) // 2 for v in grid)
+        else:
+            raise ValueError("pw_mlp: res_x / res_w go with RES_ADD and no res (down block) or RES_UPSAMPLE, a skip and res_bias (up block)")
+        entry = nat.MLP_ENTRY_LDS if lds else (nat.MLP_ENTRY_CHUNK if chunked else nat.MLP_ENTRY_FWD)
+        if tuple(res_x.shape[:-1]) != want or a.w3_format != nat.W3_F16 or not pw_mlp_res_fold_supported(c_in, c_hid, c_out, a.res_fold, entry):
+            raise ValueError(f"pw_mlp: no folded residual conv for res_x {tuple(res_x.shape)} (expected {want + (c_in,)}), "
+                             f"{c_in}->{c_hid}->{c_out}, lds={lds}, chunked={chunked}, w3 {w3p.dtype}")
+        a.res_x, a.res_w = res_x.data_ptr(), res_w.data_ptr()
+        nb += int(want[1] * want[2] * want[3]) * N * 2 * c_in if a.res_fold == nat.RES_FOLD_UP else N * rows_per_sample * 2 * c_in
+        fold = True
     if hidden_pre is not None:
         _dev(hidden_pre, "hidden_pre")
         _run(f"pw_mlp_train_fwd[{c_in}->{c_hid}->{c_out}]", nb + N * rows_per_sample * 2 * c_hid, nat.lib().pytc_pw_mlp_train_fwd,
@@ -620,9 +643,17 @@
         _run(f"pw_mlp_fwd[{c_in}->{c_hid}->{c_out}]", nb, nat.lib().pytc_pw_mlp_chunk_fwd, C.byref(a), _stream(),
              symbol=f"pw_mlp_chunk_kernel<{c_in // 32}, {c_out // 16}>")
         return y
+    if fold:
+        _run(f"pw_mlp_fwd[{c_in}->{c_hid}->{c_out}]", nb, nat.lib().pytc_pw_mlp_fwd, C.byref(a), _stream(),
+             symbol=f"pw_mlp_resconv_kernel<{c_in // 32}, {c_out // 16}>")
+        return y
     _run(f"pw_mlp_fwd[{c_in}->{c_hid}->{c_out}]", nb, nat.lib().pytc_pw_mlp_fwd, C.byref(a), _stream(),
          symbol=_mlp_symbol(a, f"pw_mlp_kernel<{c_in // 32}, {c_out // 16}>", 0))
     return y
+
+
+def pw_mlp_res_fold_supported(c_in: int, c_hid: int, c_out: int, kind: int, entry: int) -> bool:
+    return bool(nat.lib().pytc_pw_mlp_res_fold_supported(int(c_in), int(c_hid), int(c_out), int(kind), int(entry)))
 
 
 def pw_mlp_lds_supported(c_in: int, c_hid: int, c_out: int) -> bool:
diff --git a/pytorch_connectomics_amd/models/architectures/mednext.py b/pytorch_connectomics_amd/models/architectures/mednext.py
--- a/pytorch_connectomics_amd/models/architectures/mednext.py
+++ b/pytorch_connectomics_amd/models/architectures/mednext.py
@@ -137,6 +137,7 @@
         self.chunk_mixer_rows = int(os.environ.get("PYTC_CHUNK_MIXER_ROWS", "16384"))
         self.chunk_mixer_hid = int(os.environ.get("PYTC_CHUNK_MIXER_HID", "512"))
         self.fuse_block = int(os.environ.get("PYTC_FUSE_BLOCK", "0"))
+        self.fold_res_conv = os.environ.get("PYTC_FOLD_RES_CONV", "1") != "0"
 
     def _taps(self, conv: nn.Module):
         w = conv.weight
@@ -407,6 +408,9 @@
         if tuple(out.shape) != (N, Do, Ho, Wo, c_out):
             raise ValueError(f"block output buffer {tuple(out.shape)} != {(N, Do, Ho, Wo, c_out)}")
         kw["y"] = out.view(N, rows, c_out)
+    entry = nat.MLP_ENTRY_LDS if kw.get("lds") else (nat.MLP_ENTRY_CHUNK if kw.get("chunked") else nat.MLP_ENTRY_FWD)
+    fold_ok = (self.fold_res_conv and m.kind != "block" and m.resample_do_res and m.dim == "3d" and m.conv1.weight.shape[-1] == 3 and w3.dtype == torch.float16
+               and x.dtype == dt and x.is_contiguous())
     if m.kind == "block":
         y = ops.pw_mlp(t, ab, w2, b2, w3, b3, res=x if m.do_res else None,
                        res_mode=nat.RES_ADD if m.do_res else nat.RES_NONE, **kw)
@@ -415,6 +419,10 @@
         if m.resample_do_res:
             paired = ops.pw_conv_paired_supported(c_in=C, c_out=c_out, in_dtype=dt, out_dtype=dt, gather=2)
             wres = self._pw_paired(m.res_conv) if paired else self._pw(m.res_conv, dt)
+            if fold_ok and paired and ops.pw_mlp_res_fold_supported(C, c_hid, c_out, nat.RES_FOLD_DOWN, entry):
+                y = ops.pw_mlp(t, ab, w2, b2, w3, b3, res_mode=nat.RES_ADD, grid=(D, H, W), res_x=x, res_w=wres,
+                               res_bias=self._vec(m.res_conv, "bias", m.res_conv.bias), **kw)
+                return y.view(N, Do, Ho, Wo, c_out)
             res = ops.pw_conv(x, wres, self._vec(m.res_conv, "bias", m.res_conv.bias), N=N, rows_per_sample=rows,
                               c_in=C, c_out=c_out, out_dtype=dt, gather=2, grid=(D, H, W), w_paired=paired)
         y = ops.pw_mlp(t, ab, w2, b2, w3, b3, res=res, res_mode=nat.RES_ADD if res is not None else nat.RES_NONE, **kw)
@@ -426,6 +434,11 @@
             res_bias = self._vec(m.res_conv, "bias", m.res_conv.bias)
             paired = ops.pw_conv_paired_supported(c_in=C, c_out=c_out, in_dtype=dt, out_dtype=dt)
             wres = self._pw_paired(m.res_conv, transposed=True) if paired else self._pw(m.res_conv, dt, transposed=True)
+            if (fold_ok and paired and res_bias is not None and (Do, Ho, Wo) == (2 * D, 2 * H, 2 * W)
+                    and ops.pw_mlp_res_fold_supported(C, c_hid, c_out, nat.RES_FOLD_UP, entry)):
+                y = ops.pw_mlp(t, ab, w2, b2, w3, b3, res=skip, res_mode=nat.RES_UPSAMPLE, grid=(Do, Ho, Wo), res_x=x, res_w=wres,
+                               res_bias=res_bias, **kw)
+                return y.view(N, Do, Ho, Wo, c_out)
             res_low = ops.pw_conv(x, wres, res_bias, N=N, rows_per_sample=D * H * W, c_in=C, c_out=c_out,
                                   out_dtype=dt, w_paired=paired)
         y = ops.pw_mlp(t, ab, w2, b2, w3, b3, res=skip, res_mode=nat.RES_UPSAMPLE, grid=(Do, Ho, Wo),
```

Measured after the change: 1.833 billion voxels/s, median of 6. 2.1% higher.
